# Aakash1312/Fluid-Simulation

Hardware: AMD Instinct MI355X
Metric: simulated substeps/sec (higher is better)
Workload: dtype f64

## Files before the change

fluid-simulation_amd/csrc/common.h:

```cpp
#pragma once
#include <hip/hip_runtime.h>
#include <stdint.h>

namespace fl {

constexpr uint8_t F_SOLID = 1;
constexpr uint8_t F_FLUID = 2;
constexpr int F_CNT_SHIFT = 2;

struct Grid {
    int N;
    int lo;
    int hi;
    int nx, ny, nz;
    int ox, oy, oz;
    __host__ __device__ inline size_t idx(int ix, int iy, int iz) const
    {
        return ((size_t)ix * ny + (size_t)iy) * nz + (size_t)iz;
    }
    __host__ __device__ inline size_t cells() const { return (size_t)nx * ny * nz; }
    __host__ __device__ inline long sx() const { return (long)ny * nz; }
    __host__ __device__ inline int cx0() const { return lo + ox; }
    __host__ __device__ inline int cy0() const { return lo + oy; }
    __host__ __device__ inline int cz0() const { return lo + oz; }
    __host__ __device__ inline int cx1() const { return lo + ox + nx - 1; }
    __host__ __device__ inline int cy1() const { return lo + oy + ny - 1; }
    __host__ __device__ inline int cz1() const { return lo + oz + nz - 1; }
};

struct Box {
    int x0, y0, z0, x1, y1, z1;
    __host__ __device__ inline int nx() const { return x1 - x0 + 1; }
    __host__ __device__ inline int ny() const { return y1 - y0 + 1; }
    __host__ __device__ inline int nz() const { return z1 - z0 + 1; }
    __host__ __device__ inline long long cells() const { return (long long)nx() * ny() * nz(); }
};

template <typename T>
struct Coef {
    T diag[7];
    T inv[7];
    T off;
};

constexpr int LBOX_K0 = 16;
struct LBox {
    int x0, y0, z0, nx, ny, nz, Lx, Ly, Lz;
    __host__ __device__ inline size_t cells() const { return (size_t)Lx * Ly * Lz; }
};

struct MLevel {
    int dx, dy, dz;
    long sx, sy;
    int ox, oy, oz;
    size_t cells;
    __host__ __device__ inline size_t at(int i, int j, int k) const
    {
        return (size_t)((long)(i + ox) * sx + (long)(j + oy) * sy + (k + oz));
    }
};
template <typename T>
struct MgCoef {
    T diag[7];
    T inv[7];
    T off;
};

struct PcgState {
    double bb;
    double thr;
    double rr;
    int done;
    int iters;
    int breakdown;
    int pad;
};

struct StepState {
    int bbox_min[3];
    int bbox_max[3];
    int num_active;
    int n_out;
    int max_cell;
    int n_drop;
    int n_tl_mg, n_tl_sq;
    int n_rows, n_l1_old;
    int n_tl_int, n_tl_bnd;
    int n_l1_gal, n_drop_fail;
    unsigned long long max_speed_bits;
    double dt;
    double err_num;
    double err_den;
};

constexpr size_t STATE_PS_OFF = 256;
constexpr int MAX_PARTIALS = 8192;

__device__ __forceinline__ double spline(double x)
{
    if (x < 0) x *= -1.0;
    if (x < 0.5) return 1.5 * (4.0 * x * x * x - 4.0 * x * x + 2.0 / 3.0);
    if (x < 1.0) return 1.5 * ((-8.0 * (x * x * x) / 6.0) + 4.0 * x * x - 4.0 * x + 4.0 / 3.0);
    return 0;
}

__device__ __forceinline__ double spline_at(double p, int c, int d)
{
    double x = p - (double)c;
    if (d == 1) return spline(x);
    if (x < 0) x *= -1.0;
    if (x < 1.0) return 1.5 * ((-8.0 * (x * x * x) / 6.0) + 4.0 * x * x - 4.0 * x + 4.0 / 3.0);
    return 0;
}

template <typename T>
__device__ __forceinline__ T wave_sum(T v)
{
#pragma unroll
    for (int o = 32; o > 0; o >>= 1) v += __shfl_down(v, o, 64);
    return v;
}
template <typename T>
__device__ __forceinline__ T wave_max(T v)
{
#pragma unroll
    for (int o = 32; o > 0; o >>= 1) {
        T w = __shfl_down(v, o, 64);
        v = w > v ? w : v;
    }
    return v;
}
template <typename T, int NW>
__device__ __forceinline__ T block_sum(T v, T* sm)
{
    v = wave_sum(v);
    const int lane = threadIdx.x & 63, w = threadIdx.x >> 6;
    __syncthreads();
    if (lane == 0) sm[w] = v;
    __syncthreads();
    T r = 0;
    if (threadIdx.x == 0) {
#pragma unroll
        for (int i = 0; i < NW; ++i) r += sm[i];
    }
    return r;
}
template <int NW>
__device__ __forceinline__ double block_sum_array(const double* __restrict__ a, int n, double* sm)
{
    double v = 0;
    for (int i = threadIdx.x; i < n; i += NW * 64) v += a[i];
    v = wave_sum(v);
    const int lane = threadIdx.x & 63, w = threadIdx.x >> 6;
    __syncthreads();
    if (lane == 0) sm[w] = v;
    __syncthreads();
    if (threadIdx.x == 0) {
        double r = 0;
#pragma unroll
        for (int i = 0; i < NW; ++i) r += sm[i];
        sm[NW] = r;
    }
    __syncthreads();
    return sm[NW];
}

__device__ __forceinline__ int xcd_remap(int b, int nb)
{
    const int q = nb >> 3, r = nb & 7, xcd = b & 7;
    return (xcd < r ? xcd * (q + 1) : r * (q + 1) + (xcd - r) * q) + (b >> 3);
}

__device__ __forceinline__ void block_sum3(const double* __restrict__ a, int na, const double* __restrict__ b, int nb,
                                           const double* __restrict__ c, int nc, double* sm, double& ra, double& rb, double& rc)
{
    double va = 0, vb = 0, vc = 0;
    for (int i = threadIdx.x; i < na; i += 256) va += a[i];
    for (int i = threadIdx.x; i < nb; i += 256) vb += b[i];
    for (int i = threadIdx.x; i < nc; i += 256) vc += c[i];
    va = wave_sum(va); vb = wave_sum(vb); vc = wave_sum(vc);
    const int lane = threadIdx.x & 63, w = threadIdx.x >> 6;
    if (lane == 0) { sm[w] = va; sm[4 + w] = vb; sm[8 + w] = vc; }
    __syncthreads();
    ra = ((sm[0] + sm[1]) + sm[2]) + sm[3];
    rb = ((sm[4] + sm[5]) + sm[6]) + sm[7];
    rc = ((sm[8] + sm[9]) + sm[10]) + sm[11];
}

struct Particles {
    double *px, *py, *pz, *vx, *vy, *vz;
    uint32_t* pid;
    __host__ __device__ inline Particles shifted(long o) const
    {
        Particles q = *this;
        q.px += o; q.py += o; q.pz += o; q.vx += o; q.vy += o; q.vz += o; q.pid += o;
        return q;
    }
};
constexpr uint32_t PID_DEAD = 0xFFFFFFFFu;

void launch_bin_count(hipStream_t st, Grid g, long n, Particles p, int* key, int* slot, int* cell_count, int* part, StepState* ss);
void launch_bin_scatter(hipStream_t st, long n, const int* key, const int* slot, const int* cell_start, const uint32_t* pid, int* order,
                         uint32_t* spid);
void launch_bin_rank(hipStream_t st, long n_pos, long pos0, const int* key, const int* cell_start, const int* order, const uint32_t* spid,
                     int* order2);
void launch_reorder(hipStream_t st, long n, const int* order, Particles src, Particles dst, double* w = nullptr, long wstride = 0);
void launch_weights(hipStream_t st, long n, Particles p, double* w, long stride);
void launch_axpby_box(hipStream_t st, Grid g, Box box, double a, const double* x, double b, const double* y, double* out, const PcgState* gate = nullptr);
long p2g_max_items(Box box);
size_t p2g_part_doubles(Box box);
constexpr int P2G_PILED = 256;
void launch_p2g(hipStream_t st, Grid g, Box box, Particles p, const double* pw, long wstride, const int* cell_start, const uint8_t* flags,
                double* part, int* items, float* container, double* u, double* v, double* w, double* ub, double* vb, double* wb, int2* crowd_list = nullptr,
                Particles park = Particles{});
void launch_p2g_tiles(hipStream_t st, Grid g, Box box, Particles p, const double* pw, long wstride, const int* cell_start, const uint8_t* flags,
                      float* container, double* u, double* v, double* w, double* ub, double* vb, double* wb);
void launch_g2p_tiled(hipStream_t st, Grid g, Box pb, Particles p, const int* cell_start, const double* dcx, const double* dcy, const double* dcz,
                      const double* pcx, const double* pcy, const double* pcz, double blend, StepState* ss);
void launch_g2p(hipStream_t st, Grid g, long n, Particles p, const double* dcx, const double* dcy, const double* dcz, const double* pcx,
                const double* pcy, const double* pcz, double blend, StepState* ss);
void launch_advect(hipStream_t st, Grid g, long n, Particles p, const uint8_t* flags, double max_dt, double dx, StepState* ss);
void launch_advect_bin(hipStream_t st, Grid g, long n, Particles p, const uint8_t* flags, double max_dt, double dx, StepState* ss, int* key,
                       int* slot, int* cell_count, int* part);
void launch_pack_particles(hipStream_t st, long n, Particles p, double* pos_aos, double* vel_aos);
void launch_unpack_records(hipStream_t st, long n, const double* rec, Particles p, long off);
void launch_pack_records(hipStream_t st, long n, Particles p, long off, double* rec);
void launch_unpack_ids(hipStream_t st, long n, const double* pos, const double* vel, const uint32_t* ids, Particles p);
void launch_pack_ids(hipStream_t st, long n, Particles p, long off, double* pos, double* vel, uint32_t* ids);
void launch_unpack_particles(hipStream_t st, long n, const double* pos_aos, const double* vel_aos, Particles p);

void launch_out_mark(hipStream_t st, const float* f, int N, int off, int nl, int* flags);
void launch_out_pack(hipStream_t st, const float* f, int N, int lo, int off, int nl, const int* flags, const int* slot, float* values,
                     int* origin);
struct OutWin {
    int ny, nz;
    int ox, oy, oz;
    int olo[3], ohi[3];
    int lo, off;
    int l0[3], nl[3];
    __host__ __device__ inline long leaves() const { return (long)nl[0] * nl[1] * nl[2]; }
};
void launch_out_mark_win(hipStream_t st, const float* f, const OutWin& w, int* flags);
void launch_out_pack_win(hipStream_t st, const float* f, const OutWin& w, const int* flags, const int* slot, float* values, int* origin);
void launch_exclusive_scan(hipStream_t st, const int* in, int* out, long n, int* block_sums, int* total);
void launch_sort_tail(hipStream_t st, const int* cell_count, int* cell_start, long c1, long ncell);
void launch_index_scan(hipStream_t st, Grid g, const uint8_t* flags, int* indices, int* block_sums, int* total);
void launch_index_scan_flat(hipStream_t st, const uint8_t* flags, int* indices, long n, int* block_sums, int* total);
void launch_flags(hipStream_t st, Grid g, const uint8_t* solid, const float* container, uint8_t* flags, int x0, int x1);
void launch_index_scan_range(hipStream_t st, Grid g, const uint8_t* flags, int* indices, int* block_sums, int* total, int x0, int x1);
void launch_rhs_div(hipStream_t st, Grid g, Box box, const uint8_t* flags, const double* u, const double* v, const double* w,
                    float* rhs, float* diver, double dx, double gdt0, double gdt1, double gdt2, bool rows = false, const PcgState* gate = nullptr);
void launch_vel_update(hipStream_t st, Grid g, Box box, const uint8_t* flags, const double* p, double* u, double* v, double* w,
                       double k, double g0, double g1, double g2, bool rows = false, const PcgState* gate = nullptr);
void launch_flip_delta(hipStream_t st, Grid g, Box box, const double* u, const double* v, const double* w,
                       const double* ub, const double* vb, const double* wb, double* dcx, double* dcy, double* dcz, double* pcx, double* pcy, double* pcz);
void launch_err_norm(hipStream_t st, Grid g, Box box, const uint8_t* flags, const float* b, const float* b2, double* part, StepState* ss,
                     const PcgState* gate = nullptr);
void launch_zero_step_state(hipStream_t st, StepState* ss, int N);
struct ZeroList { float* f4[4]; double* f8[7]; };
void launch_zero_fields(hipStream_t st, const ZeroList& z, Grid g, Box box, bool rows = false);
void launch_unpack_box(hipStream_t st, Grid g, Box box, const double* buf, float* container, double* u, double* v, double* w, double* ub, double* vb,
                       double* wb);

void launch_extrap_init(hipStream_t st, Grid g, const uint8_t* solid, const float* container, int* layer);
void launch_extrap_layer(hipStream_t st, Grid g, int pass, int* layer, double* u, double* v, double* w, int* n_new);
void launch_resample(hipStream_t st, Grid g, long n, Particles p, const int* cell_start, int per_cell, int xlim, double far_, int* n_parked);

struct SinkSet { int n; Box box[8]; };
void launch_src_count(hipStream_t st, Grid g, long n, Particles p, Box box, int* hist);
void launch_src_plan(hipStream_t st, Grid g, Box box, uint64_t h0, int per_cell, bool fill, const uint8_t* solid, const int* hist, int* cnt);
void launch_src_emit(hipStream_t st, Grid g, Box box, uint64_t h0, int per_cell, bool fill, const uint8_t* solid, const int* hist, const int* off,
                     Particles p, uint32_t pid0, const double vel[3]);
void launch_src_append(hipStream_t st, long n, const double* pos, const double* vel, Particles p, uint32_t pid0);
void launch_interp_from_grid(hipStream_t st, Grid g, long n, Particles p, const double* u, const double* v, const double* w);
void launch_sink_mark(hipStream_t st, Grid g, long n, Particles p, const SinkSet& sk, int* keep_dev, int* keep_pid, int* removed);
void launch_sink_compact(hipStream_t st, long n, Particles a, Particles b, const int* keep_dev, const int* dev_off, const int* pid_new);

void launch_spline_eval(hipStream_t st, int which, long n, const double* x, double* w);
void launch_dot(hipStream_t st, long n, const double* a, const double* b, double* part, int nb, double* out);

LBox make_lbox(const Box& b);
size_t lbox_max_cells(int N);
int pcg_sq_blocks(const LBox& L);
int pcg_xr_blocks(const LBox& L);
void launch_cnt_local(hipStream_t st, Grid g, LBox L, const uint8_t* flags, uint8_t* cnt);
template <typename T>
void launch_pcg_init(hipStream_t st, Grid g, LBox L, const uint8_t* cnt, const float* b, T* x, T* r, Coef<T> cf, double* part_bb,
                     double* part_rz0, PcgState* ps);
template <typename T>
void launch_pcg_sq(hipStream_t st, LBox L, const uint8_t* cnt, const T* r, const T* s_in, T* s_out, T* q, Coef<T> cf,
                   const double* part_rr, const double* part_rz_new, const double* part_rz_old, double* part_pq, PcgState* ps, int first,
                   double tol, int n_rz = -1, int zmode = 0, int sparse = 0, int n_prev = -1);
template <typename T>
void launch_pcg_xr(hipStream_t st, LBox L, const uint8_t* cnt, T* x, T* r, const T* s, const T* q, Coef<T> cf, const double* part_rz_cur,
                   const double* part_pq, double* part_rr, double* part_rz_next, PcgState* ps, int n_rz = -1, int sparse = 0);
void launch_pcg_sq_zf(hipStream_t st, LBox L, const uint8_t* cnt, const float* z, const double* s_in, double* s_out, double* q, Coef<double> cf,
                      const double* part_rr, int n_prev, const double* part_rz_new, const double* part_rz_old, double* part_pq, PcgState* ps, int first,
                      double tol, int n_rz, int sparse, const int* tlist, int nlist);
int pcg_list_blocks(int nlist);
template <typename T>
void launch_pcg_sq_list(hipStream_t st, LBox L, const uint8_t* cnt, const T* r, const T* s_in, T* s_out, T* q, Coef<T> cf,
                        const double* part_rr, int n_prev, const double* part_rz_new, const double* part_rz_old, double* part_pq, PcgState* ps,
                        int first, double tol, int n_rz, int zmode, const int* tlist, int nlist);
template <typename T>
void launch_pcg_xr_list(hipStream_t st, LBox L, const uint8_t* cnt, T* x, T* r, const T* s, const T* q, Coef<T> cf, const double* part_rz_cur,
                        int n_rz, const double* part_pq, double* part_rr, double* part_rz_next, PcgState* ps, const int* tlist, int nlist);
int pcg_row_count(const LBox& L);
int pcg_rows_blocks(int nrows);
void launch_row_list(hipStream_t st, LBox L, const uint8_t* cnt, int* flags, int* pos, int* list, int* block_sums, int* count);
constexpr int DROP_CAP = 65536;
constexpr int DROP_NCTR = 64;
void launch_drop_find(hipStream_t st, LBox L, uint8_t* cnt, int* ctr, int* pre, int* total, int* comp_n, int* comp_cells, const Box* own = nullptr);
void launch_drop_solve(hipStream_t st, Grid g, LBox L, int n_comp, const int* pre, const int* comp_n, const int* comp_cells, const uint8_t* flags,
                       const float* b, Coef<double> cf, double tol, double* pressure, double* keep, int* n_fail = nullptr, const PcgState* gate = nullptr);
template <typename T>
void launch_pcg_xr_rows(hipStream_t st, LBox L, const uint8_t* cnt, T* x, T* r, const T* s, const T* q, Coef<T> cf, const double* part_rz_cur,
                        int n_rz, const double* part_pq, int n_pq, double* part_rr, double* part_rz_next, PcgState* ps, const int* rlist, int nrows);
template <typename T>
void launch_pcg_sq_dist(hipStream_t st, LBox L, const uint8_t* cnt, const T* r, const T* s_in, T* s_out, T* q, Coef<T> cf, const double* g_rr,
                        const double* g_rz_new, const double* g_rz_old, double* part_pq, PcgState* ps, int first, double tol, int zmode);
template <typename T>
void launch_pcg_xr_dist(hipStream_t st, LBox L, const uint8_t* cnt, T* x, T* r, const T* s, const T* q, Coef<T> cf, const double* g_rz_cur,
                        const double* g_pq, double* part_rr, double* part_rz_next, PcgState* ps);
void launch_sum2(hipStream_t st, const double* a, int na, const double* b, int nb, double* out_a, double* out_b);
void launch_pcg_az_dist_zf(hipStream_t st, LBox L, const uint8_t* cnt, const float* z, double* w, Coef<double> cf, double* part_zw, PcgState* ps, const int* tlist, int nlist);
void launch_pcg_cgear_upd_zf(hipStream_t st, LBox L, const uint8_t* cnt, double* x, double* r, double* s, double* q, const float* z, const double* w, const double* g,
                             double* cg, int cur, double* part_rr, PcgState* ps, int first, double tol);
void launch_pcg_poll_stage(hipStream_t st, const double* part_rr, int n, const PcgState* ps, double* out);
void launch_pcg_poll_test(hipStream_t st, const double* g, PcgState* ps);
void launch_sum4(hipStream_t st, const double* a, int na, const double* b, int nb, const double* c, int nc, const double* e, int ne, double* out);
template <typename T>
void launch_pcg_az_dist(hipStream_t st, LBox L, const uint8_t* cnt, const T* z, T* w, Coef<T> cf, double* part_zw, PcgState* ps, const int* tlist = nullptr,
                        int nlist = 0);
template <typename T>
void launch_pcg_cgear_upd(hipStream_t st, LBox L, const uint8_t* cnt, T* x, T* r, T* s, T* q, const T* z, const T* w, const double* g, double* cg, int cur,
                          double* part_rr, PcgState* ps, int first, double tol);
template <typename T>
void launch_stencil_apply(hipStream_t st, Grid g, Box box, const uint8_t* flags, const T* s, T* q, Coef<T> cf);
template <typename T>
bool launch_stencil_march(hipStream_t st, Grid g, const uint8_t* flags, const T* s, T* q, Coef<T> cf, int variant, int cxcode);
template <typename T>
void launch_store_pressure(hipStream_t st, Grid g, LBox L, const uint8_t* cnt, const T* x, double* pressure, double* keep = nullptr,
                           const PcgState* ps = nullptr, bool gated = false);
template <typename T>
void launch_pcg_init_guess(hipStream_t st, Grid g, LBox L, const uint8_t* cnt, const float* b, const double* guess, const double* guess2, double ca,
                           double cb, T* x, T* r, Coef<T> cf, double* part_bb, double* part_rr0, PcgState* ps);

MLevel mg_level0(const LBox& L);
MLevel mg_coarser(const MLevel& f);
void launch_mg_type0(hipStream_t st, Grid g, LBox L, MLevel m, const uint8_t* flags, const uint8_t* cnt, uint8_t* typ);
void launch_mg_coarsen(hipStream_t st, MLevel mf, const uint8_t* tf, MLevel mc, uint8_t* tc, uint8_t* cnt_c);
void launch_mg_coarsen_types(hipStream_t st, MLevel mf, const uint8_t* tf, MLevel mc, uint8_t* tc);
void launch_mg_counts(hipStream_t st, MLevel m, const uint8_t* typ, uint8_t* cnt);
template <typename T>
void launch_mg_restrict(hipStream_t st, MLevel mf, const T* rf, MLevel mc, const uint8_t* cnt_c, T* fc, const PcgState* ps);
constexpr int MG_TAIL_MAX = 4;
constexpr size_t MG_TAIL_LDS = 144 * 1024;
size_t mg_tail_lds_bytes(int nl, const MLevel* lv, size_t elem);
int mg_up_blocks(const MLevel& m);
template <typename T, typename F>
void launch_mg_down(hipStream_t st, MLevel m, const uint8_t* cnt, const F* f, T* u, T* r, MLevel mc, const uint8_t* cnt_c, T* fc, MgCoef<T> cf,
                    const PcgState* ps, const int* tlist = nullptr, int nlist = 0, bool pcr = false);
template <typename T, typename F, typename O>
void launch_mg_up(hipStream_t st, MLevel m, const uint8_t* cnt, const F* f, const T* u, O* out, MLevel mc, const T* ec, MgCoef<T> cf,
                  double* part_dot, const PcgState* ps, double wc, const int* tlist = nullptr, int nlist = 0, const uint8_t* own = nullptr,
                  int pconst = 0);
bool gal_fits_coarsest(const MLevel& m);
void launch_gal_level1(hipStream_t st, MLevel m0, const uint8_t* cnt0, MgCoef<float> cf0, MLevel m1, float* gd, float* gx, float* gy, float* gz, uint8_t* cnt1);
void launch_gal_coarsen(hipStream_t st, MLevel mf, const float* fd, const float* fx, const float* fy, const float* fz, const uint8_t* cntf, MLevel mc,
                        float* gd, float* gx, float* gy, float* gz, uint8_t* cntc);
int gal_tile_count(const MLevel& m);
void launch_gal_tile_flags(hipStream_t st, MLevel m, const uint8_t* cnt, uint8_t* flags);
void launch_gal_down(hipStream_t st, MLevel m, const uint8_t* cnt, const float* gd, const float* gx, const float* gy, const float* gz, const float* f, float* u,
                     MLevel mc, float* fc, const PcgState* ps);
void launch_gal_up(hipStream_t st, MLevel m, const uint8_t* cnt, const float* gd, const float* gx, const float* gy, const float* gz, const float* f, const float* u,
                   float* out, MLevel mc, const float* ec, float wc, const PcgState* ps);
void launch_gal_coarsest(hipStream_t st, MLevel m, const float* gd, const float* gx, const float* gy, const float* gz, const float* f, float* u, int sweeps,
                         const PcgState* ps);
void launch_mg_tile_flags(hipStream_t st, MLevel m, const uint8_t* cnt, uint8_t* flags);
void launch_sq_tile_flags(hipStream_t st, LBox L, const uint8_t* cnt, uint8_t* flags);
int sq_tile_count(const LBox& L);
void launch_compact_flags(hipStream_t st, const uint8_t* flags, int n, int* list, int* count);
template <typename T>
void launch_mg_tail(hipStream_t st, int nl, const T* f0, const MLevel* lv, uint8_t* const* cnt, T* u0, const T* off, int sweeps, const PcgState* ps,
                    double wc);

}
```

fluid-simulation_amd/csrc/fluid_api.hip:

```cpp
#include "sim.h"
#include <algorithm>

using namespace fl;

static thread_local std::string g_err;
int fluid_fail(int code, const std::string& msg)
{
    g_err = msg;
    return code;
}
#define fail fluid_fail

Box fl::clip_dilate(const Box& b, int d, const Grid& g)
{
    Box r;
    r.x0 = b.x0 - d < 0 ? 0 : b.x0 - d;
    r.y0 = b.y0 - d < 0 ? 0 : b.y0 - d;
    r.z0 = b.z0 - d < 0 ? 0 : b.z0 - d;
    r.x1 = b.x1 + d > g.nx - 1 ? g.nx - 1 : b.x1 + d;
    r.y1 = b.y1 + d > g.ny - 1 ? g.ny - 1 : b.y1 + d;
    r.z1 = b.z1 + d > g.nz - 1 ? g.nz - 1 : b.z1 + d;
    return r;
}

int fl::prof_begin(fluid_sim* s, int k, double cells)
{
    ProfClass& p = s->prof[k];
    p.launches++;
    const bool per_iter = k == FLUID_PROF_PCG_SQ || k == FLUID_PROF_PCG_XR || k == FLUID_PROF_MG_UP0;
    const int every = per_iter ? s->prof_every : (s->prof_every >= 8 ? s->prof_every / 8 : (s->prof_every > 0 ? 1 : 0));
    if (every <= 0 || (p.launches - 1) % every) return -1;
    hipEvent_t a, b;
    if (hipEventCreate(&a) != hipSuccess || hipEventCreate(&b) != hipSuccess) return -1;
    hipEventRecord(a, s->st);
    p.e0.push_back(a);
    p.e1.push_back(b);
    p.pc.push_back(cells);
    return (int)p.e1.size() - 1;
}
void fl::prof_end(fluid_sim* s, int k, int tok)
{
    if (tok >= 0) hipEventRecord(s->prof[k].e1[tok], s->st);
}
static void prof_resolve(fluid_sim* s)
{
    for (int k = 0; k < FLUID_PROF_COUNT; ++k) {
        ProfClass& p = s->prof[k];
        for (size_t i = 0; i < p.e0.size(); ++i) {
            float ms = 0;
            hipEventSynchronize(p.e1[i]);
            if (hipEventElapsedTime(&ms, p.e0[i], p.e1[i]) == hipSuccess) {
                p.sampled++;
                p.ms += ms;
                p.cells += p.pc[i];
            }
            hipEventDestroy(p.e0[i]);
            hipEventDestroy(p.e1[i]);
        }
        p.e0.clear();
        p.e1.clear();
        p.pc.clear();
    }
}


static void free_particles(fluid_sim* s)
{
    for (Particles* p : {&s->pa, &s->pb}) {
        hipFree(p->px); hipFree(p->py); hipFree(p->pz); hipFree(p->vx); hipFree(p->vy); hipFree(p->vz); hipFree(p->pid);
        *p = Particles{};
    }
    hipFree(s->key); hipFree(s->slot); hipFree(s->order); hipFree(s->order2); hipFree(s->spid); hipFree(s->stage_pos); hipFree(s->stage_vel);
    s->order2 = nullptr; s->spid = nullptr; hipFree(s->pw);
    s->pw = nullptr;
    s->key = s->slot = s->order = nullptr;
    s->binned = false;
    s->stage_pos = s->stage_vel = nullptr;
    s->cap = 0;
}

int fl::alloc_particles(fluid_sim* s, long n)
{
    if (n <= s->cap) return FLUID_OK;
    n = (n + 1) & ~1L;
    free_particles(s);
    for (Particles* p : {&s->pa, &s->pb}) {
        HIPCHK(dalloc(&p->px, n)); HIPCHK(dalloc(&p->py, n)); HIPCHK(dalloc(&p->pz, n));
        HIPCHK(dalloc(&p->vx, n)); HIPCHK(dalloc(&p->vy, n)); HIPCHK(dalloc(&p->vz, n));
        HIPCHK(dalloc(&p->pid, n));
    }
    HIPCHK(dalloc(&s->key, n)); HIPCHK(dalloc(&s->slot, n)); HIPCHK(dalloc(&s->order, n)); HIPCHK(dalloc(&s->order2, n)); HIPCHK(dalloc(&s->spid, n));
    HIPCHK(dalloc(&s->stage_pos, 3 * n)); HIPCHK(dalloc(&s->stage_vel, 3 * n));
    HIPCHK(dalloc(&s->pw, 9 * n));
    HIPCHK(hipDeviceSynchronize());
    s->cap = n;
    return FLUID_OK;
}

int fl::grow_particles(fluid_sim* s, long need)
{
    if (need <= s->cap) return FLUID_OK;
    HIPCHK(hipStreamSynchronize(s->st));
    const long keep = s->p_off + s->np;
    Particles old = s->pa;
    s->pa = Particles{};
    const long ncap = ((need + need / 2) + 1) & ~1L;
    Particles nw{};
    HIPCHK(dalloc(&nw.px, ncap)); HIPCHK(dalloc(&nw.py, ncap)); HIPCHK(dalloc(&nw.pz, ncap));
    HIPCHK(dalloc(&nw.vx, ncap)); HIPCHK(dalloc(&nw.vy, ncap)); HIPCHK(dalloc(&nw.vz, ncap));
    HIPCHK(dalloc(&nw.pid, ncap));
    if (keep > 0) {
        HIPCHK(hipMemcpy(nw.px, old.px, keep * 8, hipMemcpyDeviceToDevice)); HIPCHK(hipMemcpy(nw.py, old.py, keep * 8, hipMemcpyDeviceToDevice));
        HIPCHK(hipMemcpy(nw.pz, old.pz, keep * 8, hipMemcpyDeviceToDevice)); HIPCHK(hipMemcpy(nw.vx, old.vx, keep * 8, hipMemcpyDeviceToDevice));
        HIPCHK(hipMemcpy(nw.vy, old.vy, keep * 8, hipMemcpyDeviceToDevice)); HIPCHK(hipMemcpy(nw.vz, old.vz, keep * 8, hipMemcpyDeviceToDevice));
        HIPCHK(hipMemcpy(nw.pid, old.pid, keep * 4, hipMemcpyDeviceToDevice));
    }
    hipFree(old.px); hipFree(old.py); hipFree(old.pz); hipFree(old.vx); hipFree(old.vy); hipFree(old.vz); hipFree(old.pid);
    free_particles(s);
    s->pa = nw;
    Particles* p = &s->pb;
    HIPCHK(dalloc(&p->px, ncap)); HIPCHK(dalloc(&p->py, ncap)); HIPCHK(dalloc(&p->pz, ncap));
    HIPCHK(dalloc(&p->vx, ncap)); HIPCHK(dalloc(&p->vy, ncap)); HIPCHK(dalloc(&p->vz, ncap));
    HIPCHK(dalloc(&p->pid, ncap));
    HIPCHK(dalloc(&s->key, ncap)); HIPCHK(dalloc(&s->slot, ncap)); HIPCHK(dalloc(&s->order, ncap)); HIPCHK(dalloc(&s->order2, ncap)); HIPCHK(dalloc(&s->spid, ncap));
    HIPCHK(dalloc(&s->stage_pos, 3 * ncap)); HIPCHK(dalloc(&s->stage_vel, 3 * ncap));
    HIPCHK(dalloc(&s->pw, 9 * ncap));
    HIPCHK(hipDeviceSynchronize());
    s->cap = ncap;
    return FLUID_OK;
}

extern "C" {

const char* fluid_last_error(void) { return g_err.c_str(); }
const char* fluid_version(void) { return "libfluid_hip 0.1 gfx950"; }

int fluid_default_params(fluid_params_t* p)
{
    if (!p) return fail(FLUID_ERR_ARG, "null params");
    memset(p, 0, sizeof(*p));
    p->n = 121;
    p->device = 0;
    p->dx = 1.0;
    p->rho = 1.0;
    p->gravity[0] = 0; p->gravity[1] = -10; p->gravity[2] = 0;
    p->max_dt = 0.1;
    p->outer_tol = 0.1;
    p->update_frac = 0.1;
    p->cg_tol = 2.220446049250313e-16;
    p->cg_max_iters = 0;
    p->max_outer_passes = 0;
    p->precision = FLUID_PRECISION_FP64;
    p->preconditioner = FLUID_PRECOND_MG;
    p->flip_blend = 1.0;
    p->solve_start = FLUID_START_WARM;
    p->mg_precision = FLUID_MG_FP32;
    p->dist_solve = FLUID_DIST_AUTO;
    return FLUID_OK;
}

int fluid_destroy(fluid_sim_t* s)
{
    if (!s) return FLUID_OK;
    if (s->st) hipStreamSynchronize(s->st);
    if (s->ds) dist_destroy(s);
    prof_resolve(s);
    free_particles(s);
    sources_free(s);
    output_free(s);
    void* ptrs[] = {s->solid, s->flags, s->container, s->rhs, s->diver, s->diver2, s->u, s->v, s->w, s->ub, s->vb, s->wb, s->dcx, s->dcy,
                    s->dcz, s->pressure, s->p_guess, s->p_guess2, s->p_q, s->indices, s->scan_sums, s->ipart, s->R, s->S[0], s->Q, s->X, s->mg_slab, s->mg_part, s->cntL, s->part_bb, s->part_rr,
                    s->part_rz[0], s->part_rz[1], s->part_pq, s->part_err, s->cell_count, s->cell_start, s->ss,
                    s->pcx, s->pcy, s->pcz, s->p2g_part, s->p2g_items, s->p2g_crowd, s->tl_flags, s->tl_mg, s->tl_sq, s->d_small, s->row_flags, s->row_pos, s->row_list, s->drop_n, s->drop_cells, s->drop_ctr, s->gal_slab};
    for (void* p : ptrs) if (p) hipFree(p);
    for (int i = 0; i < 2; ++i) if (s->ev_poll[i]) hipEventDestroy(s->ev_poll[i]);
    if (s->h_ss) hipHostFree(s->h_ss);
    if (s->h_small) hipHostFree(s->h_small);
    if (s->st) hipStreamDestroy(s->st);
    delete s;
    return FLUID_OK;
}

int fluid_create(const fluid_params_t* p, fluid_sim_t** out)
{
    if (!p || !out) return fail(FLUID_ERR_ARG, "null argument");
    Grid g;
    g.N = p->n;
    g.lo = -(p->n / 2);
    g.hi = g.lo + p->n - 1;
    g.nx = g.ny = g.nz = p->n;
    g.ox = g.oy = g.oz = 0;
    return fluid_create_window(p, g, out);
}

}

int fl::fluid_create_window(const fluid_params_t* p, const Grid& g, fluid_sim_t** out)
{
    if (!p || !out) return fail(FLUID_ERR_ARG, "null argument");
    if (p->n < 8 || p->n > 1024) return fail(FLUID_ERR_ARG, "n must be in [8,1024]");
    if (!(p->dx > 0) || !(p->rho > 0) || !(p->max_dt > 0)) return fail(FLUID_ERR_ARG, "dx, rho, max_dt must be > 0");
    if (p->precision != FLUID_PRECISION_FP64 && p->precision != FLUID_PRECISION_FP32) return fail(FLUID_ERR_ARG, "bad precision");
    if (!(p->flip_blend >= 0.0 && p->flip_blend <= 1.0)) return fail(FLUID_ERR_ARG, "flip_blend must be in [0,1] (1 = the reference's pure FLIP)");
    if (p->preconditioner != FLUID_PRECOND_MG && p->preconditioner != FLUID_PRECOND_JACOBI) return fail(FLUID_ERR_ARG, "bad preconditioner");
    if (p->solve_start != FLUID_START_WARM && p->solve_start != FLUID_START_ZERO) return fail(FLUID_ERR_ARG, "bad solve_start");
    if (p->mg_precision != FLUID_MG_FP32 && p->mg_precision != FLUID_MG_FP64) return fail(FLUID_ERR_ARG, "bad mg_precision");
    if (p->dist_solve < FLUID_DIST_AUTO || p->dist_solve > FLUID_DIST_REPLICATED || p->pad_ != 0) return fail(FLUID_ERR_ARG, "bad dist_solve / pad_");
    int ndev = 0;
    if (hipGetDeviceCount(&ndev) != hipSuccess || ndev <= 0)
        return fail(FLUID_ERR_HIP, "no HIP device visible: libfluid_hip has no CPU path");
    if (p->device < 0 || p->device >= ndev) return fail(FLUID_ERR_ARG, "device ordinal out of range");
    HIPCHK(hipSetDevice(p->device));
    fluid_sim* s = new fluid_sim();
    s->prm = *p;
    s->g = g;
    s->ncell = g.cells();
    s->dt = p->max_dt;
    s->mg_fp32 = p->mg_precision == FLUID_MG_FP32;
    s->warm = p->solve_start == FLUID_START_WARM;
    if (const char* e = getenv("FLUID_MG_CSWEEPS")) s->mg_csweeps = atoi(e);
    if (const char* e = getenv("FLUID_TILE_LISTS")) s->lists_force = atoi(e) != 0;
    if (const char* e = getenv("FLUID_P2G_FORM")) s->p2g_force = !strcmp(e, "rows") ? 1 : (!strcmp(e, "tiles") ? 2 : (!strcmp(e, "crowd") ? 3 : 0));
    if (const char* e = getenv("FLUID_MG_GALERKIN")) s->gal_mode = atoi(e);
    if (const char* e = getenv("FLUID_DROPLETS")) s->drops_on = atoi(e) != 0;
    if (const char* e = getenv("FLUID_ROW_SWEEPS")) s->row_sweeps = atoi(e) != 0;
    if (const char* e = getenv("FLUID_DROPLETS_MIN")) s->drop_min = atoi(e);
    if (const char* e = getenv("FLUID_ADVECT_BIN")) s->advect_bin = atoi(e) != 0;
    if (const char* e = getenv("FLUID_SOLVE_TAIL")) s->solve_tail = atoi(e) != 0;
    *out = nullptr;
    auto bail = [&](int rc) { fluid_destroy(s); return rc; };
#define A(expr) do { hipError_t e_ = (expr); if (e_ != hipSuccess) return bail(fail(FLUID_ERR_HIP, std::string(#expr) + ": " + hipGetErrorString(e_))); } while (0)
    A(hipStreamCreateWithFlags(&s->st, hipStreamNonBlocking));
    const size_t n = s->ncell;
    A(dalloc(&s->solid, n)); A(dalloc(&s->flags, n));
    A(dalloc(&s->container, n)); A(dalloc(&s->rhs, n)); A(dalloc(&s->diver, n)); A(dalloc(&s->diver2, n));
    A(dalloc(&s->u, n)); A(dalloc(&s->v, n)); A(dalloc(&s->w, n));
    A(dalloc(&s->ub, n)); A(dalloc(&s->vb, n)); A(dalloc(&s->wb, n));
    A(dalloc(&s->dcx, n)); A(dalloc(&s->dcy, n)); A(dalloc(&s->dcz, n));
    A(dalloc(&s->pressure, n));
    if (s->warm) {
        A(dalloc(&s->p_guess, n)); A(dalloc(&s->p_guess2, n));
        if (hipMemset(s->p_guess, 0, n * sizeof(double)) != hipSuccess || hipMemset(s->p_guess2, 0, n * sizeof(double)) != hipSuccess) return bail(FLUID_ERR_HIP);
        if (const char* e = getenv("FLUID_EXTRAPOLATE")) s->extrapolate = atoi(e) != 0;
        if (s->extrapolate) { A(dalloc(&s->p_q, n)); if (hipMemset(s->p_q, 0, n * sizeof(double)) != hipSuccess) return bail(FLUID_ERR_HIP); }
    }
    A(dalloc(&s->indices, n));
    A(dalloc(&s->scan_sums, (n + 2) / 2048 + 16));
    A(dalloc(&s->ipart, (size_t)1024 * 8));
    const size_t se = solver_elem(s);
    s->lmax = lbox_max_cells(std::max(g.nx, std::max(g.ny, g.nz)));
    const size_t ln = s->lmax;
    A(dalloc((char**)&s->R, ln * se)); A(dalloc((char**)&s->S[0], 2 * ln * se + 256));
    s->S[1] = (char*)s->S[0] + ln * se;
    A(dalloc((char**)&s->Q, ln * se)); A(dalloc((char**)&s->X, ln * se)); A(dalloc(&s->cntL, ln + 64));
    A(dalloc(&s->mg_part, ln / 256 + 64));
    A(dalloc(&s->part_bb, (size_t)MAX_PARTIALS)); A(dalloc(&s->part_rr, (size_t)MAX_PARTIALS));
    A(dalloc(&s->part_rz[0], (size_t)MAX_PARTIALS)); A(dalloc(&s->part_rz[1], (size_t)MAX_PARTIALS));
    A(dalloc(&s->part_pq, (size_t)MAX_PARTIALS)); A(dalloc(&s->part_err, (size_t)2 * MAX_PARTIALS));
    static_assert(sizeof(StepState) <= STATE_PS_OFF, "PcgState overlaps StepState");
    A(dalloc((char**)&s->ss, STATE_PS_OFF + sizeof(PcgState)));
    s->ps = (PcgState*)((char*)s->ss + STATE_PS_OFF);
    A(dalloc(&s->cell_count, n + 4)); A(dalloc(&s->cell_start, n + 4));
    A(dalloc(&s->d_small, (size_t)32));
    A(hipHostMalloc((void**)&s->h_small, 32 * sizeof(int)));
    A(hipEventCreateWithFlags(&s->ev_poll[0], hipEventDisableTiming));
    A(hipEventCreateWithFlags(&s->ev_poll[1], hipEventDisableTiming));
    A(hipHostMalloc((void**)&s->h_ss, STATE_PS_OFF + 2 * sizeof(PcgState)));
    s->h_ps = (PcgState*)((char*)s->h_ss + STATE_PS_OFF);
#undef A
    std::vector<uint8_t> sol(n, 0);
    const int N = p->n;
    for (int x = 0; x < g.nx; ++x)
        for (int y = 0; y < g.ny; ++y)
            for (int z = 0; z < g.nz; ++z) {
                const int X = x + g.ox, Y = y + g.oy, Z = z + g.oz;
                if (X < 2 || X > N - 3 || Y < 2 || Y > N - 3 || Z < 2 || Z > N - 3) sol[g.idx(x, y, z)] = 1;
            }
    hipError_t e = hipMemcpy(s->solid, sol.data(), n, hipMemcpyHostToDevice);
    if (e == hipSuccess) e = hipMemcpy(s->flags, sol.data(), n, hipMemcpyHostToDevice);
    if (e == hipSuccess) e = hipDeviceSynchronize();
    if (e != hipSuccess) return bail(fail(FLUID_ERR_HIP, std::string("solid upload: ") + hipGetErrorString(e)));
    *out = s;
    return FLUID_OK;
}

extern "C" {

int fluid_set_solid(fluid_sim_t* s, const uint8_t* solid)
{
    if (!s || !solid) return fail(FLUID_ERR_ARG, "null argument");
    const int N = s->g.N;
    const Grid g = s->g;
    for (int x = 0; x < N; ++x)
        for (int y = 0; y < N; ++y)
            for (int z = 0; z < N; ++z) {
                size_t c = ((size_t)x * N + y) * N + z;
                bool outsideW = x < 2 || x > N - 3 || y < 2 || y > N - 3 || z < 2 || z > N - 3;
                if (outsideW && !solid[c]) return fail(FLUID_ERR_ARG, "cells outside W=[lo+2,hi-2]^3 must be solid");
            }
    std::vector<uint8_t> sol(s->ncell);
    for (int x = 0; x < g.nx; ++x)
        for (int y = 0; y < g.ny; ++y)
            for (int z = 0; z < g.nz; ++z)
                sol[g.idx(x, y, z)] = solid[((size_t)(x + g.ox) * N + (y + g.oy)) * N + (z + g.oz)] ? 1 : 0;
    dist_keep_solid(s, solid);
    HIPCHK(hipStreamSynchronize(s->st));
    HIPCHK(hipMemcpy(s->solid, sol.data(), s->ncell, hipMemcpyHostToDevice));
    HIPCHK(hipMemcpy(s->flags, sol.data(), s->ncell, hipMemcpyHostToDevice));
    s->have_p2g = s->have_flags = false;
    s->flags_valid = false;
    s->have_guess = false;
    return FLUID_OK;
}

int fluid_upload_particles(fluid_sim_t* s, int64_t n, const double* pos, const double* vel)
{
    if (!s || n < 0 || (n > 0 && !pos)) return fail(FLUID_ERR_ARG, "bad particle arguments");
    if (s->dist) return fail(FLUID_ERR_STATE, "decomposed run: use fluid_upload_particles_ids (global ids must be unique across ranks)");
    if (n > 0x7fffffffL) return fail(FLUID_ERR_ARG, "too many particles");
    HIPCHK(hipSetDevice(s->prm.device));
    int rc = alloc_particles(s, (long)n);
    if (rc) return rc;
    s->np = (long)n;
    s->p_off = 0;
    if (n > 0) {
        HIPCHK(hipMemcpyAsync(s->stage_pos, pos, 3 * n * sizeof(double), hipMemcpyHostToDevice, s->st));
        if (vel) HIPCHK(hipMemcpyAsync(s->stage_vel, vel, 3 * n * sizeof(double), hipMemcpyHostToDevice, s->st));
        launch_unpack_particles(s->st, s->np, s->stage_pos, vel ? s->stage_vel : nullptr, s->pa);
        HIPCHK(hipGetLastError());
        HIPCHK(hipStreamSynchronize(s->st));
    }
    s->sorted = s->have_p2g = s->have_flags = false;
    s->have_guess = false;
    s->sort_hint = false;
    s->binned = false;
    s->vel_ok = false;
    return FLUID_OK;
}

int fluid_download_particles(fluid_sim_t* s, double* pos, double* vel)
{
    if (!s || !pos || !vel) return fail(FLUID_ERR_ARG, "null argument");
    if (s->dist) return fail(FLUID_ERR_STATE, "decomposed run: use fluid_download_particles_ids");
    if (s->np == 0) return FLUID_OK;
    HIPCHK(hipSetDevice(s->prm.device));
    launch_pack_particles(s->st, s->np, s->pa.shifted(s->p_off), s->stage_pos, s->stage_vel);
    HIPCHK(hipGetLastError());
    HIPCHK(hipMemcpyAsync(pos, s->stage_pos, 3 * s->np * sizeof(double), hipMemcpyDeviceToHost, s->st));
    HIPCHK(hipMemcpyAsync(vel, s->stage_vel, 3 * s->np * sizeof(double), hipMemcpyDeviceToHost, s->st));
    HIPCHK(hipStreamSynchronize(s->st));
    return FLUID_OK;
}

int64_t fluid_num_particles(fluid_sim_t* s) { return s ? s->np : -1; }
int fluid_set_dt(fluid_sim_t* s, double dt)
{
    if (!s || !(dt > 0)) return fail(FLUID_ERR_ARG, "dt must be > 0");
    s->dt = dt;
    return FLUID_OK;
}
int fluid_get_dt(fluid_sim_t* s, double* dt)
{
    if (!s || !dt) return fail(FLUID_ERR_ARG, "null argument");
    *dt = s->dt;
    return FLUID_OK;
}

static inline double u01(uint64_t seed, uint64_t ctr)
{
    uint64_t z = seed * 0x9E3779B97F4A7C15ull + ctr * 0xBF58476D1CE4E5B9ull + 0x94D049BB133111EBull;
    z ^= z >> 30; z *= 0xBF58476D1CE4E5B9ull;
    z ^= z >> 27; z *= 0x94D049BB133111EBull;
    z ^= z >> 31;
    return (double)(z >> 11) * (1.0 / 9007199254740992.0);
}

int64_t fluid_scene_water_cube_drop(int32_t n, int32_t ppc, uint64_t seed, double* pos)
{
    if (n < 8 || ppc < 1) return -1;
    const int m = (int)std::lround((double)n * 41.0 / 121.0);
    const int c0 = -(m / 2), c1 = c0 + m - 1;
    const int lo = -(n / 2), hi = lo + n - 1;
    int64_t cnt = 0;
    uint64_t ctr = 0;
    for (int x = c0; x <= c1; ++x)
        for (int y = c0; y <= c1; ++y)
            for (int z = c0; z <= c1; ++z)
                for (int k = 0; k < ppc; ++k) {
                    const double px = x - 0.5 + u01(seed, ctr), py = y - 0.5 + u01(seed, ctr + 1), pz = z - 0.5 + u01(seed, ctr + 2);
                    ctr += 3;
                    if (px > lo + 2 && px < hi - 2 && py > lo + 2 && py < hi - 2 && pz > lo + 2 && pz < hi - 2) {
                        if (pos) { pos[3 * cnt] = px; pos[3 * cnt + 1] = py; pos[3 * cnt + 2] = pz; }
                        cnt++;
                    }
                }
    return cnt;
}

}

int fl::read_ss(fluid_sim* s)
{
    HIPCHK(hipMemcpyAsync(s->h_ss, s->ss, sizeof(StepState), hipMemcpyDeviceToHost, s->st));
    HIPCHK(hipStreamSynchronize(s->st));
    return FLUID_OK;
}

int fl::clear_dirty(fluid_sim* s)
{
    if (box_empty(s->dirty)) return FLUID_OK;
    const ZeroList z = {{s->container, s->rhs, s->diver, s->diver2}, {s->u, s->v, s->w, s->ub, s->vb, s->wb, s->pressure}};
    launch_zero_fields(s->st, z, s->g, s->dirty, !s->dist && s->row_sweeps);
    HIPCHK(hipGetLastError());
    s->dirty = Box{0, 0, 0, -1, -1, -1};
    return FLUID_OK;
}

int fl::sort_pass(fluid_sim* s, int ax0, int ax1, int* h_tail)
{
    const Grid g = s->g;
    const long ncell = (long)s->ncell, n2 = g.sx();
    const long c0 = (long)ax0 * n2, c1 = (long)(ax1 + 1) * n2;
    launch_zero_step_state(s->st, s->ss, g.N);
    HIPCHK(hipMemsetAsync(s->cell_count + c0, 0, (c1 - c0) * sizeof(int), s->st));
    HIPCHK(hipMemsetAsync(s->cell_count + ncell, 0, 4 * sizeof(int), s->st));
    launch_bin_count(s->st, g, s->np, s->pa.shifted(s->p_off), s->key, s->slot, s->cell_count, s->ipart, s->ss);
    launch_exclusive_scan(s->st, s->cell_count + c0, s->cell_start + c0, c1 - c0, s->scan_sums, s->cell_start + c1);
    launch_sort_tail(s->st, s->cell_count, s->cell_start, c1, ncell);
    launch_bin_scatter(s->st, s->np, s->key, s->slot, s->cell_start, s->pa.shifted(s->p_off).pid, s->order, s->spid);
    launch_bin_rank(s->st, s->np, 0, s->key, s->cell_start, s->order, s->spid, s->order2);
    HIPCHK(hipGetLastError());
    if (h_tail) HIPCHK(hipMemcpyAsync(h_tail, s->cell_start + ncell, 3 * sizeof(int), hipMemcpyDeviceToHost, s->st));
    return read_ss(s);
}

static int sort_binned(fluid_sim* s)
{
    const Grid g = s->g;
    const long ncell = (long)s->ncell, n2 = g.sx();
    const long c0 = (long)s->bin_x0 * n2, c1 = (long)(s->bin_x1 + 1) * n2;
    launch_zero_step_state(s->st, s->ss, g.N);
    launch_exclusive_scan(s->st, s->cell_count + c0, s->cell_start + c0, c1 - c0, s->scan_sums, s->cell_start + c1);
    launch_sort_tail(s->st, s->cell_count, s->cell_start, c1, ncell);
    launch_bin_scatter(s->st, s->np, s->key, s->slot, s->cell_start, s->pa.shifted(s->p_off).pid, s->order, s->spid);
    launch_bin_rank(s->st, s->np, 0, s->key, s->cell_start, s->order, s->spid, s->order2);
    HIPCHK(hipGetLastError());
    StepState& h = *s->h_ss;
    for (int a = 0; a < 3; ++a) h.bbox_min[a] = s->bin_min[a], h.bbox_max[a] = s->bin_max[a];
    h.n_out = s->bin_n_out;
    h.max_cell = s->bin_max_cell;
    return FLUID_OK;
}

static int phase_sort(fluid_sim* s)
{
    const Grid g = s->g;
    int tok = prof_begin(s, FLUID_PROF_SORT, (double)s->np);
    int ax0 = 0, ax1 = g.nx - 1;
    const bool guess = s->sort_hint && !box_empty(s->Pb);
    if (guess) {
        ax0 = std::max(0, s->Pb.x0 - 3);
        ax1 = std::min(g.nx - 1, s->Pb.x1 + 3);
    }
    const bool binned = s->binned && guess && ax0 == s->bin_x0 && ax1 == s->bin_x1 && s->np > 0;
    s->binned = false;
    const auto missed = [&](const int* bmin, const int* bmax) {
        return guess && bmax[0] >= 0 && (bmin[0] < std::min(ax0 + 2, s->Pb.x0) || bmax[0] > std::max(ax1 - 2, s->Pb.x1));
    };
    int rc;
    if (binned && !missed(s->bin_min, s->bin_max)) {
        if ((rc = sort_binned(s))) return rc;
    } else {
        rc = binned ? FLUID_OK : sort_pass(s, ax0, ax1);
        if (rc) return rc;
        if (binned || missed(s->h_ss->bbox_min, s->h_ss->bbox_max)) {
            if ((rc = sort_pass(s, 0, g.nx - 1))) return rc;
        }
    }
    s->sort_hint = true;
    s->n_out = s->h_ss->n_out;
    s->max_cell = s->h_ss->max_cell;
    const StepState& h = *s->h_ss;
    if (h.bbox_max[0] < 0) {
        s->Pb = Box{0, 0, 0, -1, -1, -1};
    } else {
        s->Pb = Box{h.bbox_min[0], h.bbox_min[1], h.bbox_min[2], h.bbox_max[0], h.bbox_max[1], h.bbox_max[2]};
    }
    if (!box_empty(s->Pb)) {
        s->Rb = clip_dilate(s->Pb, 1, g);
        s->Sb = clip_dilate(s->Pb, 2, g);
    } else {
        s->Rb = s->Sb = s->Pb;
    }
    launch_reorder(s->st, s->np, s->order2, s->pa.shifted(s->p_off), s->pb, s->pw, s->cap);
    HIPCHK(hipGetLastError());
    std::swap(s->pa, s->pb);
    s->p_off = 0;
    prof_end(s, FLUID_PROF_SORT, tok);
    s->sorted = true;
    return FLUID_OK;
}

int fl::run_p2g(fluid_sim* s, const Box& box)
{
    const long ref_cells = s->p2g_ref_cells > 0 ? s->p2g_ref_cells : s->Rb.cells();
    const bool airy = s->last_num_active > 0 && (double)s->last_num_active < 0.3 * (double)ref_cells;
    const bool huge = (size_t)12 * sizeof(double) * (size_t)box.cells() > ((size_t)16 << 30);
    const bool piled = s->max_cell > P2G_PILED || airy;
    if (s->p2g_force ? s->p2g_force == 2 : huge) {
        s->stats.paths |= FLUID_PATH_P2G_TILES;
        launch_p2g_tiles(s->st, s->g, box, s->pa, s->pw, s->cap, s->cell_start, s->flags, s->container, s->u, s->v, s->w, s->ub, s->vb, s->wb);
        return FLUID_OK;
    }
    const bool crowd = s->p2g_force ? s->p2g_force == 3 : piled;
    if (crowd) {
        s->stats.paths |= FLUID_PATH_P2G_CROWD;
        const size_t nl = (size_t)s->cap / 16 + 64;
        if (nl > s->p2g_crowd_cap) {
            if (s->p2g_crowd) { HIPCHK(hipStreamSynchronize(s->st)); hipFree(s->p2g_crowd); s->p2g_crowd = nullptr; }
            HIPCHK(hipMalloc((void**)&s->p2g_crowd, nl * sizeof(int2)));
            s->p2g_crowd_cap = nl;
        }
    }
    const size_t need = p2g_part_doubles(box);
    if (need > s->p2g_part_cap) {
        if (s->p2g_part) { HIPCHK(hipStreamSynchronize(s->st)); hipFree(s->p2g_part); s->p2g_part = nullptr; }
        HIPCHK(hipMalloc((void**)&s->p2g_part, (need + need / 4) * sizeof(double)));
        s->p2g_part_cap = need + need / 4;
    }
    const size_t ni = 4 + 4 * (size_t)p2g_max_items(box);
    if (ni > s->p2g_items_cap) {
        if (s->p2g_items) { HIPCHK(hipStreamSynchronize(s->st)); hipFree(s->p2g_items); s->p2g_items = nullptr; }
        HIPCHK(hipMalloc((void**)&s->p2g_items, (ni + ni / 4) * sizeof(int)));
        HIPCHK(hipMemsetAsync(s->p2g_items, 0, 4 * sizeof(int), s->st));
        s->p2g_items_cap = ni + ni / 4;
    }
    launch_p2g(s->st, s->g, box, s->pa, s->pw, s->cap, s->cell_start, s->flags, s->p2g_part, s->p2g_items, s->container, s->u, s->v, s->w, s->ub,
               s->vb, s->wb, crowd ? s->p2g_crowd : nullptr, s->pb);
    return FLUID_OK;
}

static int phase_p2g(fluid_sim* s)
{
    HIPCHK(hipSetDevice(s->prm.device));
    int rc = phase_sort(s);
    if (rc) return rc;
    rc = clear_dirty(s);
    if (rc) return rc;
    memset(&s->stats, 0, sizeof(s->stats));
    s->stats.dt_in = s->dt;
    s->stats.dt_out = s->dt;
    for (int a = 0; a < 3; ++a) {
        s->stats.box_lo[a] = (&s->Rb.x0)[a];
        s->stats.box_hi[a] = (&s->Rb.x1)[a];
    }
    if (!box_empty(s->Rb)) {
        int tok = prof_begin(s, FLUID_PROF_P2G, (double)s->Rb.cells());
        rc = run_p2g(s, s->Rb);
        prof_end(s, FLUID_PROF_P2G, tok);
        if (rc) return rc;
        HIPCHK(hipGetLastError());
        s->dirty = s->Sb;
    }
    s->have_p2g = true;
    s->step_counter++;
    s->have_flags = false;
    return FLUID_OK;
}

template <typename T>
Coef<T> fl::make_coef(const fluid_sim* s)
{
    const double scale = s->dt / (s->prm.rho * s->prm.dx * s->prm.dx);
    Coef<T> c;
    float acc = 0.0f;
    c.diag[0] = 0;
    c.inv[0] = 0;
    for (int k = 1; k <= 6; ++k) {
        acc = (float)((double)acc + scale);
        c.diag[k] = (T)acc;
        c.inv[k] = (T)1 / c.diag[k];
    }
    c.off = (T)(float)(-1 * scale);
    return c;
}
template Coef<double> fl::make_coef<double>(const fluid_sim*);
template Coef<float> fl::make_coef<float>(const fluid_sim*);

hipError_t fl::zero_search(fluid_sim* s, size_t lb)
{
    const size_t step = (lb + 255) / 256 * 256;
    s->S[1] = (char*)s->S[0] + step;
    return hipMemsetAsync(s->S[0], 0, step + lb, s->st);
}


static int gal_build(fluid_sim* s);
static int mg_setup(fluid_sim* s)
{
    s->mgl[0] = mg_level0(s->L);
    int nl = 1;
    while (nl < fluid_sim::MG_MAXL && (nl < 2 || s->mgl[nl - 1].dx > 8 || s->mgl[nl - 1].dy > 8 || s->mgl[nl - 1].dz > 8)) {
        s->mgl[nl] = mg_coarser(s->mgl[nl - 1]);
        ++nl;
    }
    if (s->mgl[nl - 1].dx > 8 || s->mgl[nl - 1].dy > 8 || s->mgl[nl - 1].dz > 8) return fail(FLUID_ERR_STATE, "multigrid: too many levels");
    s->mg_nl = nl;
    int tail = nl - 1;
    const size_t es = s->mg_fp32 ? sizeof(float) : sizeof(double);
    auto fits = [&](int t) {
        const size_t b = nl - t <= MG_TAIL_MAX ? mg_tail_lds_bytes(nl - t, s->mgl + t, es) : 0;
        return b > 0 && b <= MG_TAIL_LDS;
    };
    while (tail > 1 && fits(tail - 1)) --tail;
    if (!fits(tail)) return fail(FLUID_ERR_STATE, "multigrid: coarsest level does not fit the tail kernel");
    s->mg_tail = tail;
    size_t total = 0;
    auto take = [&](size_t bytes) { const size_t o = total; total += (bytes + 255) / 256 * 256; return o; };
    size_t o_typ[fluid_sim::MG_MAXL], o_cnt[fluid_sim::MG_MAXL], o_u[fluid_sim::MG_MAXL], o_v[fluid_sim::MG_MAXL], o_f[fluid_sim::MG_MAXL],
        o_r[fluid_sim::MG_MAXL];
    for (int l = 0; l < nl; ++l) {
        const size_t c = s->mgl[l].cells + 64;
        o_typ[l] = take(c); o_cnt[l] = take(c);
        o_u[l] = take(c * es); o_v[l] = take(c * es); o_f[l] = take(c * es); o_r[l] = take(c * es);
    }
    const size_t o_z = take((s->mgl[0].cells + 64) * 8);
    if (total > s->mg_slab_cap) {
        if (s->mg_slab) { HIPCHK(hipStreamSynchronize(s->st)); hipFree(s->mg_slab); s->mg_slab = nullptr; }
        const size_t cap = total + total / 4;
        HIPCHK(hipMalloc((void**)&s->mg_slab, cap));
        s->mg_slab_cap = cap;
    }
    for (int l = 0; l < nl; ++l) {
        s->mg_typ[l] = (uint8_t*)(s->mg_slab + o_typ[l]);
        s->mg_cnt[l] = l ? (uint8_t*)(s->mg_slab + o_cnt[l]) : nullptr;
        s->mg_u[l] = s->mg_slab + o_u[l]; s->mg_v[l] = s->mg_slab + o_v[l];
        s->mg_f[l] = l ? s->mg_slab + o_f[l] : nullptr;
        s->mg_r[l] = s->mg_slab + o_r[l];
    }
    s->Zmg = s->mg_slab + o_z;
    HIPCHK(hipMemsetAsync(s->mg_slab, 0, total, s->st));
    launch_mg_type0(s->st, s->g, s->L, s->mgl[0], s->flags, s->cntL, s->mg_typ[0]);
    for (int l = 1; l < nl; ++l) launch_mg_coarsen(s->st, s->mgl[l - 1], s->mg_typ[l - 1], s->mgl[l], s->mg_typ[l], s->mg_cnt[l]);
    { int rcg = gal_build(s); if (rcg) return rcg; }
    HIPCHK(hipGetLastError());
    return FLUID_OK;
}

MgCoef<double> fl::mg_coef(const fluid_sim* s, int level)
{
    MgCoef<double> c;
    if (level == 0) {
        const Coef<double> f = make_coef<double>(s);
        for (int k = 0; k < 7; ++k) { c.diag[k] = f.diag[k]; c.inv[k] = f.inv[k]; }
        c.off = f.off;
        return c;
    }
    const double scale = s->dt / (s->prm.rho * s->prm.dx * s->prm.dx) / std::pow(4.0, level);
    c.off = -scale;
    c.diag[0] = 0; c.inv[0] = 0;
    for (int k = 1; k < 7; ++k) { c.diag[k] = scale * k; c.inv[k] = 1.0 / c.diag[k]; }
    return c;
}

static int mg_rz_blocks(const fluid_sim* s) { return s->lists_on ? s->n_tl_mg : mg_up_blocks(s->mgl[0]); }

template <typename V>
static MgCoef<V> mg_coef_as(const fluid_sim* s, int level)
{
    const MgCoef<double> d = mg_coef(s, level);
    MgCoef<V> c;
    for (int k = 0; k < 7; ++k) { c.diag[k] = (V)d.diag[k]; c.inv[k] = (V)d.inv[k]; }
    c.off = (V)d.off;
    return c;
}
static int gal_build(fluid_sim* s)
{
    s->gal = false;
    s->gal_eligible = false;
    const int nl = s->mg_nl;
    int lc = 1;
    while (lc < nl - 1 && !gal_fits_coarsest(s->mgl[lc])) ++lc;
    if (!(s->gal_mode && s->lists_on && s->mg_fp32 && !s->dist && (long)s->mgl[0].dx * s->mgl[0].dy * s->mgl[0].dz > 200000 &&
          gal_fits_coarsest(s->mgl[lc]) && lc >= 2)) {
        s->gal_it[0] = s->gal_it[1] = -1;
        return FLUID_OK;
    }
    s->gal_eligible = true;
    bool use = s->gal_mode >= 2;
    if (s->gal_mode == 1) {
        if (s->gal_it[0] < 0) use = false;
        else if (s->gal_it[1] < 0) use = true;
        else {
            use = 21 * s->gal_it[1] < 20 * s->gal_it[0];
            if (++s->gal_since_probe >= 32) { use = !use; s->gal_since_probe = 0; }
        }
    }
    if (!use) return FLUID_OK;
    size_t total = 0, off[fluid_sim::MG_MAXL][6];
    for (int l = 1; l <= lc; ++l)
        for (int q = 0; q < 6; ++q) {
            off[l][q] = total;
            total += (q < 5 ? ((q < 4 ? sizeof(float) : 1) * (s->mgl[l].cells + 64) + 255) / 256 * 256 : ((size_t)gal_tile_count(s->mgl[l]) + 255) / 256 * 256);
        }
    if (total > s->gal_slab_cap) {
        if (s->gal_slab) { HIPCHK(hipStreamSynchronize(s->st)); hipFree(s->gal_slab); s->gal_slab = nullptr; }
        HIPCHK(hipMalloc((void**)&s->gal_slab, total + total / 4));
        s->gal_slab_cap = total + total / 4;
    }
    HIPCHK(hipMemsetAsync(s->gal_slab, 0, total, s->st));
    for (int l = 1; l <= lc; ++l) {
        for (int q = 0; q < 4; ++q) s->gal_c[l][q] = (float*)(s->gal_slab + off[l][q]);
        s->gal_cnt[l] = (uint8_t*)(s->gal_slab + off[l][4]);
        s->gal_tfl[l] = (uint8_t*)(s->gal_slab + off[l][5]);
    }
    launch_gal_level1(s->st, s->mgl[0], s->cntL, mg_coef_as<float>(s, 0), s->mgl[1], s->gal_c[1][0], s->gal_c[1][1], s->gal_c[1][2], s->gal_c[1][3], s->gal_cnt[1]);
    for (int l = 2; l <= lc; ++l)
        launch_gal_coarsen(s->st, s->mgl[l - 1], s->gal_c[l - 1][0], s->gal_c[l - 1][1], s->gal_c[l - 1][2], s->gal_c[l - 1][3], s->gal_cnt[l - 1], s->mgl[l],
                           s->gal_c[l][0], s->gal_c[l][1], s->gal_c[l][2], s->gal_c[l][3], s->gal_cnt[l]);
    for (int l = 1; l < lc; ++l) launch_gal_tile_flags(s->st, s->mgl[l], s->gal_cnt[l], s->gal_tfl[l]);
    s->gal = true;
    s->gal_lc = lc;
    s->gal_dt = s->dt;
    HIPCHK(hipGetLastError());
    return FLUID_OK;
}
static int mg_vcycle_gal(fluid_sim* s, const double* rhs0, float* z0, double* part_rz)
{
    typedef float V;
    const PcgState* ps = s->ps;
    const int lc = s->gal_lc;
    auto U = [&](int l) { return (V*)s->mg_u[l]; };
    auto W = [&](int l) { return (V*)s->mg_v[l]; };
    auto F = [&](int l) { return (V*)s->mg_f[l]; };
    auto C = [&](int l, int q) { return (const float*)s->gal_c[l][q]; };
    const MLevel& m0 = s->mgl[0];
    launch_mg_down<V, double>(s->st, m0, s->cntL, rhs0, U(0), (V*)s->mg_r[0], s->mgl[1], nullptr, F(1), mg_coef_as<V>(s, 0), ps, s->tl_mg, s->n_tl_mg, true);
    for (int l = 1; l < lc; ++l) launch_gal_down(s->st, s->mgl[l], s->gal_tfl[l], C(l, 0), C(l, 1), C(l, 2), C(l, 3), F(l), U(l), s->mgl[l + 1], F(l + 1), ps);
    launch_gal_coarsest(s->st, s->mgl[lc], C(lc, 0), C(lc, 1), C(lc, 2), C(lc, 3), F(lc), U(lc), s->gal_sweeps, ps);
    for (int l = lc - 1; l >= 1; --l)
        launch_gal_up(s->st, s->mgl[l], s->gal_tfl[l], C(l, 0), C(l, 1), C(l, 2), C(l, 3), F(l), U(l), W(l), s->mgl[l + 1], l + 1 == lc ? U(l + 1) : W(l + 1),
                      (float)s->gal_wc, ps);
    const int tok = prof_begin(s, FLUID_PROF_MG_UP0, (double)s->Rb.cells());
    launch_mg_up<V, double, float>(s->st, m0, s->cntL, rhs0, (const V*)U(0), z0, s->mgl[1], W(1), mg_coef_as<V>(s, 0), part_rz, ps, s->gal_wc, s->tl_mg, s->n_tl_mg,
                                   nullptr, 1);
    prof_end(s, FLUID_PROF_MG_UP0, tok);
    HIPCHK(hipGetLastError());
    return FLUID_OK;
}

template <typename V>
static int mg_vcycle_t(fluid_sim* s, const double* rhs0, V* z0, double* part_rz)
{
    const int nl = s->mg_nl, tail = s->mg_tail;
    const PcgState* ps = s->ps;
    auto U = [&](int l) { return (V*)s->mg_u[l]; };
    auto W = [&](int l) { return (V*)s->mg_v[l]; };
    auto F = [&](int l) { return (V*)s->mg_f[l]; };
    auto R = [&](int l) { return (V*)s->mg_r[l]; };
    for (int l = 0; l < tail; ++l) {
        const MLevel& m = s->mgl[l];
        const bool fold = l > 0 || (long)m.dx * m.dy * m.dz <= 200000;
        V* fc = fold ? F(l + 1) : nullptr;
        const uint8_t* cc = fold ? s->mg_cnt[l + 1] : nullptr;
        const bool lst = s->lists_on && !fold;
        if (l == 0) launch_mg_down<V, double>(s->st, m, s->cntL, rhs0, U(0), R(0), s->mgl[1], cc, fc, mg_coef_as<V>(s, 0), ps, lst ? s->tl_mg : nullptr, s->n_tl_mg);
        else launch_mg_down<V, V>(s->st, m, s->mg_cnt[l], (const V*)F(l), U(l), R(l), s->mgl[l + 1], cc, fc, mg_coef_as<V>(s, l), ps);
        if (!fold) launch_mg_restrict<V>(s->st, m, (const V*)R(l), s->mgl[l + 1], s->mg_cnt[l + 1], F(l + 1), ps);
    }
    {
        V off[fluid_sim::MG_MAXL];
        for (int l = tail; l < nl; ++l) off[l] = (V)mg_coef(s, l).off;
        launch_mg_tail<V>(s->st, nl - tail, (const V*)F(tail), s->mgl + tail, s->mg_cnt + tail, U(tail), off + tail, s->mg_csweeps, ps, s->mg_wc[3]);
    }
    for (int l = tail - 1; l >= 0; --l) {
        const MLevel& m = s->mgl[l];
        const V* ec = l + 1 == tail ? U(l + 1) : W(l + 1);
        if (l == 0) {
            const int tok = prof_begin(s, FLUID_PROF_MG_UP0, (double)s->Rb.cells());
            launch_mg_up<V, double, V>(s->st, m, s->cntL, rhs0, (const V*)U(0), z0, s->mgl[1], ec, mg_coef_as<V>(s, 0), part_rz, ps, s->mg_wc[0],
                                       s->lists_on ? s->tl_mg : nullptr, s->n_tl_mg);
            prof_end(s, FLUID_PROF_MG_UP0, tok);
        } else {
            launch_mg_up<V, V, V>(s->st, m, s->mg_cnt[l], (const V*)F(l), (const V*)U(l), W(l), s->mgl[l + 1], ec, mg_coef_as<V>(s, l), nullptr, ps, s->mg_wc[l == 1 ? 1 : 2]);
        }
    }
    HIPCHK(hipGetLastError());
    return FLUID_OK;
}
static int mg_vcycle(fluid_sim* s, const double* rhs0, void* z0, double* part_rz)
{
    if (s->gal && s->lists_on) return mg_vcycle_gal(s, rhs0, (float*)z0, part_rz);
    return s->mg_fp32 ? mg_vcycle_t<float>(s, rhs0, (float*)z0, part_rz) : mg_vcycle_t<double>(s, rhs0, (double*)z0, part_rz);
}

static int phase_vel_update(fluid_sim* s, const PcgState* gate = nullptr);
static int phase_rhs_div(fluid_sim* s, int which, const PcgState* gate = nullptr);
static int solve_mg(fluid_sim* s, bool with_tail)
{
    typedef double T;
    const Grid g = s->g;
    const LBox L = s->L;
    T* X = (T*)s->X;
    T* R = (T*)s->R;
    T* Q = (T*)s->Q;
    T* Sx[2] = {(T*)s->S[0], (T*)s->S[1]};
    T* Z = (T*)s->Zmg;
    const uint8_t* cnt = s->cntL;
    const Coef<T> cf = make_coef<T>(s);
    const double tol = s->prm.cg_tol;
    long max_it = s->prm.cg_max_iters > 0 ? s->prm.cg_max_iters : 2 * (long)s->stats.num_active;
    if (max_it < 1) max_it = 1;
    const double cells = (double)s->Rb.cells();
    const int sparse = (double)s->stats.num_active < 0.4 * (double)L.cells();
    const bool lists = s->lists_on;
    const bool rows = lists && s->rows_on && s->n_rows > 0;
    const int n_init = pcg_xr_blocks(L), n_list = rows ? pcg_rows_blocks(s->n_rows) : pcg_list_blocks(s->n_tl_sq);
    const int n_rz_raw = mg_rz_blocks(s);
    const bool fold = n_rz_raw > 1024;
    const int n_rz = fold ? 1 : n_rz_raw;
    int rc;
    int tsolve = prof_begin(s, FLUID_PROF_SOLVE, cells);
    if (s->gal && s->gal_dt != s->dt) {
        const int keep = s->gal_mode; s->gal_mode = 2; rc = gal_build(s); s->gal_mode = keep;
        if (rc) return rc;
    }
    if (s->gal) s->stats.paths |= FLUID_PATH_MG_GALERKIN;
    const bool guess = s->warm && s->have_guess;
    const double *g1, *g2;
    double gca, gcb;
    s->start_guess(g1, g2, gca, gcb);
    if (guess) launch_pcg_init_guess<T>(s->st, g, L, cnt, s->diver, g1, g2, gca, gcb, X, R, cf, s->part_bb, s->part_rz[1], s->ps);
    else launch_pcg_init<T>(s->st, g, L, cnt, s->diver, X, R, cf, s->part_bb, s->part_rr, s->ps);
    long it = 0;
    const int pclass = s->pass_class();
    long batch = s->mg_last_iters_k[pclass] > 5 ? s->mg_last_iters_k[pclass] + 1 : 4;
    bool done = false;
    const bool zf = s->mg_fp32 || (s->gal && s->lists_on);
    auto sq = [&](int cur, const double* part_rr, int n_prev, const double* rz_new, const double* rz_old, int first, int sp) {
        const int prv = cur ^ 1;
        if (zf)
            launch_pcg_sq_zf(s->st, L, cnt, (const float*)s->Zmg, Sx[prv], Sx[cur], Q, cf, part_rr, n_prev, rz_new, rz_old, s->part_pq, s->ps, first, tol, n_rz, sp,
                             lists ? s->tl_sq : nullptr, s->n_tl_sq);
        else if (lists)
            launch_pcg_sq_list<T>(s->st, L, cnt, Z, Sx[prv], Sx[cur], Q, cf, part_rr, n_prev, rz_new, rz_old, s->part_pq, s->ps, first, tol, n_rz, 1, s->tl_sq, s->n_tl_sq);
        else
            launch_pcg_sq<T>(s->st, L, cnt, Z, Sx[prv], Sx[cur], Q, cf, part_rr, rz_new, rz_old, s->part_pq, s->ps, first, tol, n_rz, 1, sp, n_prev);
    };
    const bool will_make_q = s->warm && s->p_q && s->stats.outer_passes == 1 && s->guess_step == s->step_counter && s->guess_pass == 0;
    auto solution_out = [&](const PcgState* gate) {
        launch_store_pressure<T>(s->st, g, L, cnt, X, s->pressure, s->warm ? s->p_guess2 : nullptr, s->ps, gate != nullptr);
        launch_drop_solve(s->st, g, L, s->n_drop, s->drop_ctr + 64 * DROP_NCTR, s->drop_n, s->drop_cells, s->flags, s->diver, make_coef<double>(s), tol,
                          s->pressure, s->warm ? s->p_guess2 : nullptr, &s->ss->n_drop_fail, gate);
        if (will_make_q) launch_axpby_box(s->st, g, s->Rb, 1.0, s->p_guess2, -(1.0 - s->prm.update_frac), s->p_guess, s->p_q, gate);
    };
    bool first_poll = true;
    s->tail_ran = false;
    while (!done) {
        for (long k = 0; k < batch && it < max_it; ++k, ++it) {
            const int cur = (int)(it & 1), prv = cur ^ 1;
            if ((rc = mg_vcycle(s, R, s->Zmg, fold ? s->mg_part : s->part_rz[cur]))) return rc;
            if (fold) launch_sum2(s->st, s->mg_part, n_rz_raw, s->mg_part, 0, s->part_rz[cur], nullptr);
            int tok = prof_begin(s, FLUID_PROF_PCG_SQ, cells);
            sq(cur, it == 0 ? s->part_bb : s->part_rr, it == 0 ? n_init : (lists ? n_list : n_init), s->part_rz[cur], s->part_rz[prv], it == 0 ? (guess ? 2 : 1) : 0,
               sparse);
            prof_end(s, FLUID_PROF_PCG_SQ, tok);
            tok = prof_begin(s, FLUID_PROF_PCG_XR, cells);
            if (rows)
                launch_pcg_xr_rows<T>(s->st, L, cnt, X, R, Sx[cur], Q, cf, s->part_rz[cur], n_rz, s->part_pq, pcg_list_blocks(s->n_tl_sq), s->part_rr,
                                      s->part_err, s->ps, s->row_list, s->n_rows);
            else if (lists)
                launch_pcg_xr_list<T>(s->st, L, cnt, X, R, Sx[cur], Q, cf, s->part_rz[cur], n_rz, s->part_pq, s->part_rr, s->part_err, s->ps,
                                      s->tl_sq, s->n_tl_sq);
            else
                launch_pcg_xr<T>(s->st, L, cnt, X, R, Sx[cur], Q, cf, s->part_rz[cur], s->part_pq, s->part_rr, s->part_err, s->ps, n_rz, sparse);
            prof_end(s, FLUID_PROF_PCG_XR, tok);
        }
        HIPCHK(hipGetLastError());
        if (it < max_it) {
            const int cur = (int)(it & 1), prv = cur ^ 1;
            sq(cur, s->part_rr, lists ? n_list : n_init, s->part_rz[prv], s->part_rz[prv], 0, 0);
        }
        const bool spec = with_tail && s->solve_tail && !s->dist && first_poll && it < max_it;
        first_poll = false;
        if (spec) {
            int rc2;
            solution_out(s->ps);
            if ((rc2 = phase_vel_update(s, s->ps))) return rc2;
            if ((rc2 = phase_rhs_div(s, 1, s->ps))) return rc2;
            launch_err_norm(s->st, s->g, s->Rb, s->flags, s->diver, s->diver2, s->part_err, s->ss, s->ps);
            HIPCHK(hipGetLastError());
            HIPCHK(hipMemcpyAsync(s->h_ss, s->ss, STATE_PS_OFF + sizeof(PcgState), hipMemcpyDeviceToHost, s->st));
        } else {
            HIPCHK(hipMemcpyAsync(&s->h_ps[0], s->ps, sizeof(PcgState), hipMemcpyDeviceToHost, s->st));
        }
        HIPCHK(hipStreamSynchronize(s->st));
        done = s->h_ps[0].done || it >= max_it;
        if (spec && s->h_ps[0].done) s->tail_ran = true;
        if (!done) {
            s->h_ps[1] = s->h_ps[0];
            s->h_ps[1].iters -= 1;
            HIPCHK(hipMemcpyAsync(s->ps, &s->h_ps[1], sizeof(PcgState), hipMemcpyHostToDevice, s->st));
        }
        batch = 1;
    }
    int iters = s->h_ps->iters;
    const double rr = s->h_ps->rr;
    if (!s->h_ps->done) iters = (int)max_it;
    if (!s->tail_ran) solution_out(nullptr);
    if (s->warm) s->rotate_guess();
    s->have_guess = s->warm;
    if (s->make_q() != will_make_q) return fail(FLUID_ERR_STATE, "solve_mg: q formed for the wrong pass");
    if (will_make_q) s->q_step = s->step_counter;
    HIPCHK(hipGetLastError());
    prof_end(s, FLUID_PROF_SOLVE, tsolve);
    s->stats.cg_iters_last = iters;
    s->stats.cg_iters += iters;
    s->mg_last_iters_k[pclass] = iters;
    if (s->gal_eligible && s->stats.outer_passes == 0) s->gal_it[s->gal ? 1 : 0] = iters;
    s->stats.relres = s->h_ps->bb > 0 ? std::sqrt(rr / s->h_ps->bb) : 0.0;
    if (s->h_ps->breakdown) return fail(FLUID_ERR_SOLVER, "PCG breakdown: s.As <= 0 or NaN");
    return FLUID_OK;
}

int fl::phase_flags(fluid_sim* s)
{
    HIPCHK(hipSetDevice(s->prm.device));
    int x0 = 0, x1 = s->g.nx - 1;
    const bool none = box_empty(s->Sb);
    if (s->flags_valid) {
        x0 = none ? s->flag_x0 : (s->flag_x1 < s->flag_x0 ? s->Sb.x0 : std::min(s->Sb.x0, s->flag_x0));
        x1 = none ? s->flag_x1 : (s->flag_x1 < s->flag_x0 ? s->Sb.x1 : std::max(s->Sb.x1, s->flag_x1));
    }
    if (x1 >= x0) {
        launch_flags(s->st, s->g, s->solid, s->container, s->flags, x0, x1);
        launch_index_scan_range(s->st, s->g, s->flags, s->indices, s->scan_sums, &s->ss->num_active, x0, x1);
    } else {
        HIPCHK(hipMemsetAsync(&s->ss->num_active, 0, sizeof(int), s->st));
    }
    s->flag_x0 = none ? 0 : s->Sb.x0;
    s->flag_x1 = none ? -1 : s->Sb.x1;
    s->flags_valid = true;
    HIPCHK(hipGetLastError());
    bool built = false, drops = false;
    s->n_drop = 0;
    if (!box_empty(s->Rb)) {
        s->L = make_lbox(s->Rb);
        launch_cnt_local(s->st, s->g, s->L, s->flags, s->cntL);
        if (use_mg(s) && (s->lists_force >= 0 ? s->lists_force == 1 : s->lists_hint)) {
            const MLevel m0 = mg_level0(s->L);
            const int n_mg = mg_up_blocks(m0), n_sq = sq_tile_count(s->L);
            const size_t need = (size_t)n_mg + n_sq;
            if (need > s->tl_cap) {
                HIPCHK(hipStreamSynchronize(s->st));
                hipFree(s->tl_flags); hipFree(s->tl_mg); hipFree(s->tl_sq);
                s->tl_flags = nullptr; s->tl_mg = s->tl_sq = nullptr;
                const size_t cap = need + need / 4;
                HIPCHK(hipMalloc((void**)&s->tl_flags, cap));
                HIPCHK(hipMalloc((void**)&s->tl_mg, cap * sizeof(int)));
                HIPCHK(hipMalloc((void**)&s->tl_sq, cap * sizeof(int)));
                s->tl_cap = cap;
            }
            if (s->drops_on && !s->dist && (s->drop_last < 0 || s->drop_last >= s->drop_min || ++s->drop_skipped >= 8)) {
                s->drop_skipped = 0;
                if (!s->drop_cells) {
                    HIPCHK(hipMalloc((void**)&s->drop_ctr, (size_t)(64 * DROP_NCTR + DROP_NCTR + 1) * sizeof(int)));
                    HIPCHK(hipMalloc((void**)&s->drop_n, (size_t)DROP_CAP * sizeof(int)));
                    HIPCHK(hipMalloc((void**)&s->drop_cells, (size_t)DROP_CAP * 64 * sizeof(int)));
                }
                launch_drop_find(s->st, s->L, s->cntL, s->drop_ctr, s->drop_ctr + 64 * DROP_NCTR, &s->ss->n_drop, s->drop_n, s->drop_cells);
                drops = true;
            }
            launch_mg_tile_flags(s->st, m0, s->cntL, s->tl_flags);
            launch_compact_flags(s->st, s->tl_flags, n_mg, s->tl_mg, &s->ss->n_tl_mg);
            launch_sq_tile_flags(s->st, s->L, s->cntL, s->tl_flags + n_mg);
            launch_compact_flags(s->st, s->tl_flags + n_mg, n_sq, s->tl_sq, &s->ss->n_tl_sq);
            if (s->rows_on) {
                const size_t nr = (size_t)pcg_row_count(s->L);
                if (nr > s->row_cap) {
                    HIPCHK(hipStreamSynchronize(s->st));
                    hipFree(s->row_flags); hipFree(s->row_pos); hipFree(s->row_list);
                    s->row_flags = s->row_pos = s->row_list = nullptr;
                    const size_t cap = nr + nr / 4 + 1024;
                    HIPCHK(hipMalloc((void**)&s->row_flags, cap * sizeof(int)));
                    HIPCHK(hipMalloc((void**)&s->row_pos, cap * sizeof(int)));
                    HIPCHK(hipMalloc((void**)&s->row_list, cap * sizeof(int)));
                    s->row_cap = cap;
                }
                launch_row_list(s->st, s->L, s->cntL, s->row_flags, s->row_pos, s->row_list, s->scan_sums, &s->ss->n_rows);
            }
            built = true;
        }
        HIPCHK(hipGetLastError());
    }
    int rc = read_ss(s);
    if (rc) return rc;
    s->stats.num_active = s->h_ss->num_active;
    s->last_num_active = s->stats.num_active;
    s->lists_on = false;
    s->lists_hint = false;
    if (!box_empty(s->Rb)) {
        const bool airy = (double)s->stats.num_active < 0.45 * (double)s->L.cells() && s->L.cells() > (size_t)1500000;
        s->lists_hint = airy;
        s->n_tl_mg = s->h_ss->n_tl_mg; s->n_tl_sq = s->h_ss->n_tl_sq; s->n_rows = s->h_ss->n_rows;
        s->n_drop = drops ? std::min(s->h_ss->n_drop, DROP_CAP) : 0;
        if (drops) s->drop_last = s->n_drop;
        if (s->n_drop > 0) s->stats.paths |= FLUID_PATH_DROPLETS;
        s->lists_on = built && s->n_tl_mg > 0 && s->n_tl_sq > 0 && (s->lists_force == 1 || airy);
        if (s->lists_on) s->stats.paths |= FLUID_PATH_TILE_LISTS;
        const size_t lb = (s->L.cells() + 2 * (size_t)s->L.Lz) * solver_elem(s);
        HIPCHK(zero_search(s, lb));
        HIPCHK(hipGetLastError());
        if (use_mg(s)) {
            int rc2 = mg_setup(s);
            if (rc2) return rc2;
        }
    }
    s->have_flags = true;
    return FLUID_OK;
}

static int phase_rhs_div(fluid_sim* s, int which, const PcgState* gate)
{
    if (!s->have_flags) return fail(FLUID_ERR_STATE, "rhs_div before flags_index");
    if (box_empty(s->Rb)) return FLUID_OK;
    const double dt = s->dt;
    launch_rhs_div(s->st, s->g, s->Rb, s->flags, s->u, s->v, s->w, s->rhs, which ? s->diver2 : s->diver, s->prm.dx,
                   s->prm.gravity[0] * dt, s->prm.gravity[1] * dt, s->prm.gravity[2] * dt, !s->dist && s->row_sweeps, gate);
    HIPCHK(hipGetLastError());
    return FLUID_OK;
}

template <typename T>
static int solve_impl(fluid_sim* s)
{
    const Grid g = s->g;
    const LBox L = s->L;
    T* X = (T*)s->X;
    T* R = (T*)s->R;
    T* Q = (T*)s->Q;
    T* Sx[2] = {(T*)s->S[0], (T*)s->S[1]};
    const uint8_t* cnt = s->cntL;
    const Coef<T> cf = make_coef<T>(s);
    const double tol = s->prm.cg_tol;
    long max_it = s->prm.cg_max_iters > 0 ? s->prm.cg_max_iters : 2 * (long)s->stats.num_active;
    if (max_it < 1) max_it = 1;
    const double cells = (double)s->Rb.cells();
    int tsolve = prof_begin(s, FLUID_PROF_SOLVE, cells);
    launch_pcg_init<T>(s->st, g, L, cnt, s->diver, X, R, cf, s->part_bb, s->part_rz[0], s->ps);
    int tok = prof_begin(s, FLUID_PROF_PCG_SQ, cells);
    launch_pcg_sq<T>(s->st, L, cnt, R, (const T*)nullptr, Sx[0], Q, cf, s->part_bb, nullptr, nullptr, s->part_pq, s->ps, 1, tol);
    prof_end(s, FLUID_PROF_PCG_SQ, tok);
    tok = prof_begin(s, FLUID_PROF_PCG_XR, cells);
    launch_pcg_xr<T>(s->st, L, cnt, X, R, Sx[0], Q, cf, s->part_rz[0], s->part_pq, s->part_rr, s->part_rz[1], s->ps);
    prof_end(s, FLUID_PROF_PCG_XR, tok);
    long it = 1;
    const int CHECK = 16;
    bool done = false;
    int nb = 0;
    while (!done) {
        for (int k = 0; k < CHECK && it < max_it; ++k, ++it) {
            const int cur = (int)(it & 1), prv = cur ^ 1;
            tok = prof_begin(s, FLUID_PROF_PCG_SQ, cells);
            launch_pcg_sq<T>(s->st, L, cnt, R, Sx[prv], Sx[cur], Q, cf, s->part_rr, s->part_rz[cur], s->part_rz[prv], s->part_pq, s->ps, 0, tol);
            prof_end(s, FLUID_PROF_PCG_SQ, tok);
            tok = prof_begin(s, FLUID_PROF_PCG_XR, cells);
            launch_pcg_xr<T>(s->st, L, cnt, X, R, Sx[cur], Q, cf, s->part_rz[cur], s->part_pq, s->part_rr, s->part_rz[prv], s->ps);
            prof_end(s, FLUID_PROF_PCG_XR, tok);
        }
        HIPCHK(hipGetLastError());
        HIPCHK(hipMemcpyAsync(&s->h_ps[nb & 1], s->ps, sizeof(PcgState), hipMemcpyDeviceToHost, s->st));
        HIPCHK(hipEventRecord(s->ev_poll[nb & 1], s->st));
        if (nb >= 1) {
            HIPCHK(hipEventSynchronize(s->ev_poll[(nb - 1) & 1]));
            if (s->h_ps[(nb - 1) & 1].done) done = true;
        }
        if (it >= max_it) done = true;
        ++nb;
    }
    HIPCHK(hipMemcpyAsync(&s->h_ps[0], s->ps, sizeof(PcgState), hipMemcpyDeviceToHost, s->st));
    HIPCHK(hipStreamSynchronize(s->st));
    int iters = s->h_ps->iters;
    const double rr = s->h_ps->rr;
    if (!s->h_ps->done) {
        iters = (int)max_it;
    }
    launch_store_pressure<T>(s->st, g, L, cnt, X, s->pressure);
    launch_drop_solve(s->st, g, L, s->n_drop, s->drop_ctr + 64 * DROP_NCTR, s->drop_n, s->drop_cells, s->flags, s->diver, make_coef<double>(s), tol,
                      s->pressure, nullptr, &s->ss->n_drop_fail);
    HIPCHK(hipGetLastError());
    prof_end(s, FLUID_PROF_SOLVE, tsolve);
    s->stats.cg_iters_last = iters;
    s->stats.cg_iters += iters;
    s->stats.relres = s->h_ps->bb > 0 ? std::sqrt(rr / s->h_ps->bb) : 0.0;
    if (s->h_ps->breakdown) return fail(FLUID_ERR_SOLVER, "PCG breakdown: s.As <= 0 or NaN (matrix not SPD for these flags)");
    return FLUID_OK;
}

static int phase_solve(fluid_sim* s, bool with_tail = false)
{
    s->tail_ran = false;
    if (!s->have_flags) return fail(FLUID_ERR_STATE, "solve before flags_index");
    if (box_empty(s->Rb)) return FLUID_OK;
    if (use_mg(s) && s->mg_nl >= 2) return solve_mg(s, with_tail);
    return s->prm.precision == FLUID_PRECISION_FP32 ? solve_impl<float>(s) : solve_impl<double>(s);
}

static int phase_vel_update(fluid_sim* s, const PcgState* gate)
{
    if (!s->have_flags) return fail(FLUID_ERR_STATE, "vel_update before flags_index");
    if (box_empty(s->Sb)) return FLUID_OK;
    const double dtp = s->dt * s->prm.update_frac;
    const double k = dtp / (s->prm.rho * s->prm.dx);
    launch_vel_update(s->st, s->g, s->Sb, s->flags, s->pressure, s->u, s->v, s->w, k, s->prm.gravity[0] * dtp, s->prm.gravity[1] * dtp,
                      s->prm.gravity[2] * dtp, !s->dist && s->row_sweeps, gate);
    HIPCHK(hipGetLastError());
    return FLUID_OK;
}

int fl::phase_pressure_pass(fluid_sim* s, double* error)
{
    int rc;
    if ((rc = phase_rhs_div(s, 0))) return rc;
    if ((rc = phase_solve(s, true))) return rc;
    const bool tail_ran = s->tail_ran;
    s->tail_ran = false;
    if (!tail_ran) {
        if ((rc = phase_vel_update(s))) return rc;
        if ((rc = phase_rhs_div(s, 1))) return rc;
    }
    double err = NAN;
    if (!box_empty(s->Rb)) {
        if (!tail_ran) {
            launch_err_norm(s->st, s->g, s->Rb, s->flags, s->diver, s->diver2, s->part_err, s->ss);
            HIPCHK(hipGetLastError());
            if ((rc = read_ss(s))) return rc;
        }
        if (s->h_ss->n_drop_fail > 0) s->stats.paths |= FLUID_PATH_DROPLETS_SHORT;
        err = std::sqrt(s->h_ss->err_num) / std::sqrt(s->h_ss->err_den);
    }
    s->stats.error = err;
    s->stats.outer_passes++;
    if (error) *error = err;
    return FLUID_OK;
}

int fl::pic_fields(fluid_sim* s)
{
    if (s->prm.flip_blend >= 1.0 || s->pcx) return FLUID_OK;
    double** f[3] = {&s->pcx, &s->pcy, &s->pcz};
    for (double** q : f) {
        HIPCHK(hipMalloc((void**)q, s->ncell * sizeof(double)));
        HIPCHK(hipMemsetAsync(*q, 0, s->ncell * sizeof(double), s->st));
    }
    return FLUID_OK;
}

static int phase_flip_advect(fluid_sim* s)
{
    if (!s->have_p2g) return fail(FLUID_ERR_STATE, "flip_advect before p2g");
    HIPCHK(hipSetDevice(s->prm.device));
    int rcp = pic_fields(s);
    if (rcp) return rcp;
    if (!box_empty(s->Rb)) launch_flip_delta(s->st, s->g, s->Rb, s->u, s->v, s->w, s->ub, s->vb, s->wb, s->dcx, s->dcy, s->dcz, s->pcx, s->pcy, s->pcz);
    int tok = prof_begin(s, FLUID_PROF_G2P, (double)s->np);
    if (s->sorted && s->p_off == 0 && (double)s->np >= 4.0 * (double)s->Pb.cells()) {
        launch_g2p_tiled(s->st, s->g, s->Pb, s->pa, s->cell_start, s->dcx, s->dcy, s->dcz, s->pcx, s->pcy, s->pcz, s->prm.flip_blend, s->ss);
        if (!box_empty(s->Pb)) s->stats.paths |= FLUID_PATH_G2P_TILES;
        if (s->n_out > 0)
            launch_g2p(s->st, s->g, s->n_out, s->pa.shifted(s->np - s->n_out), s->dcx, s->dcy, s->dcz, s->pcx, s->pcy, s->pcz, s->prm.flip_blend, s->ss);
    } else {
        launch_g2p(s->st, s->g, s->np, s->pa.shifted(s->p_off), s->dcx, s->dcy, s->dcz, s->pcx, s->pcy, s->pcz, s->prm.flip_blend, s->ss);
    }
    prof_end(s, FLUID_PROF_G2P, tok);
    const bool bin = s->advect_bin && !s->dist && s->np > 0 && s->sorted && s->sort_hint && !box_empty(s->Pb);
    s->binned = false;
    if (bin) {
        const Grid g = s->g;
        s->bin_x0 = std::max(0, s->Pb.x0 - 3);
        s->bin_x1 = std::min(g.nx - 1, s->Pb.x1 + 3);
        const long n2 = g.sx(), c0 = (long)s->bin_x0 * n2, c1 = (long)(s->bin_x1 + 1) * n2;
        HIPCHK(hipMemsetAsync(s->cell_count + c0, 0, (c1 - c0) * sizeof(int), s->st));
        HIPCHK(hipMemsetAsync(s->cell_count + s->ncell, 0, 4 * sizeof(int), s->st));
        launch_advect_bin(s->st, g, s->np, s->pa.shifted(s->p_off), s->flags, s->prm.max_dt, s->prm.dx, s->ss, s->key, s->slot, s->cell_count, s->ipart);
    } else {
        launch_advect(s->st, s->g, s->np, s->pa.shifted(s->p_off), s->flags, s->prm.max_dt, s->prm.dx, s->ss);
    }
    HIPCHK(hipGetLastError());
    int rc = read_ss(s);
    if (rc) return rc;
    if (bin) {
        const StepState& h = *s->h_ss;
        for (int a = 0; a < 3; ++a) s->bin_min[a] = h.bbox_min[a], s->bin_max[a] = h.bbox_max[a];
        s->bin_n_out = h.n_out;
        s->bin_max_cell = h.max_cell;
        s->binned = true;
    }
    s->dt = s->h_ss->dt;
    double ms;
    memcpy(&ms, &s->h_ss->max_speed_bits, sizeof(double));
    s->stats.max_speed = ms;
    s->stats.dt_out = s->dt;
    s->sorted = false;
    s->have_p2g = false;
    s->vel_ok = true;
    return FLUID_OK;
}

extern "C" {

#define PHASE_GUARD(s)                                                                                        \
    if (!(s)) return fail(FLUID_ERR_ARG, "null handle");                                                      \
    if ((s)->dist) return fail(FLUID_ERR_STATE, "per-phase entry points are single-GPU only; a decomposed run steps with fluid_step")
int fluid_p2g(fluid_sim_t* s) { PHASE_GUARD(s); return phase_p2g(s); }
int fluid_flags_index(fluid_sim_t* s) { PHASE_GUARD(s); return phase_flags(s); }
int fluid_rhs_div(fluid_sim_t* s, int which) { PHASE_GUARD(s); return phase_rhs_div(s, which, nullptr); }
int fluid_solve(fluid_sim_t* s) { PHASE_GUARD(s); return phase_solve(s, false); }
int fluid_vel_update(fluid_sim_t* s) { PHASE_GUARD(s); return phase_vel_update(s, nullptr); }
int fluid_pressure_pass(fluid_sim_t* s, double* error) { PHASE_GUARD(s); return phase_pressure_pass(s, error); }
int fluid_flip_advect(fluid_sim_t* s) { PHASE_GUARD(s); return phase_flip_advect(s); }

int fluid_extrapolate(fluid_sim_t* s, int32_t* n_layers)
{
    PHASE_GUARD(s);
    if (!s->have_p2g) return fail(FLUID_ERR_STATE, "extrapolate before p2g");
    HIPCHK(hipSetDevice(s->prm.device));
    const Grid g = s->g;
    int* layer = s->indices;
    int* n_new = s->d_small;
    launch_extrap_init(s->st, g, s->solid, s->container, layer);
    int pass = 0;
    for (bool more = true; more;) {
        HIPCHK(hipMemsetAsync(n_new, 0, sizeof(int), s->st));
        for (int k = 0; k < 8; ++k) launch_extrap_layer(s->st, g, ++pass, layer, s->u, s->v, s->w, n_new);
        HIPCHK(hipGetLastError());
        HIPCHK(hipMemcpyAsync(s->h_small, n_new, sizeof(int), hipMemcpyDeviceToHost, s->st));
        HIPCHK(hipStreamSynchronize(s->st));
        more = s->h_small[0] != 0 && pass < 3 * g.N + 8;
    }
    const size_t bytes = s->ncell * sizeof(double);
    HIPCHK(hipMemcpyAsync(s->ub, s->u, bytes, hipMemcpyDeviceToDevice, s->st));
    HIPCHK(hipMemcpyAsync(s->vb, s->v, bytes, hipMemcpyDeviceToDevice, s->st));
    HIPCHK(hipMemcpyAsync(s->wb, s->w, bytes, hipMemcpyDeviceToDevice, s->st));
    s->flags_valid = false;
    s->have_flags = false;
    s->dirty = Box{0, 0, 0, g.nx - 1, g.ny - 1, g.nz - 1};
    HIPCHK(hipStreamSynchronize(s->st));
    if (n_layers) *n_layers = pass;
    return FLUID_OK;
}

int fluid_get_droplets(fluid_sim_t* s, int32_t* n_components, int64_t* cells, int32_t cap_components)
{
    if (!s) return fail(FLUID_ERR_ARG, "null handle");
    if (n_components) *n_components = s->n_drop;
    if (!cells || s->n_drop <= 0 || cap_components <= 0) return FLUID_OK;
    HIPCHK(hipSetDevice(s->prm.device));
    const int n = std::min(s->n_drop, (int)cap_components);
    std::vector<int> pre(DROP_NCTR + 1), an(DROP_CAP), ac((size_t)DROP_CAP * 64), hn(n), hc((size_t)n * 64);
    HIPCHK(hipStreamSynchronize(s->st));
    HIPCHK(hipMemcpy(pre.data(), s->drop_ctr + 64 * DROP_NCTR, pre.size() * sizeof(int), hipMemcpyDeviceToHost));
    HIPCHK(hipMemcpy(an.data(), s->drop_n, an.size() * sizeof(int), hipMemcpyDeviceToHost));
    HIPCHK(hipMemcpy(ac.data(), s->drop_cells, ac.size() * sizeof(int), hipMemcpyDeviceToHost));
    for (int d = 0, c = 0; d < n; ++d) {
        while (c + 1 < DROP_NCTR && pre[c + 1] <= d) ++c;
        const size_t slot = (size_t)c * (DROP_CAP / DROP_NCTR) + (size_t)(d - pre[c]);
        hn[d] = an[slot];
        std::copy(ac.begin() + slot * 64, ac.begin() + slot * 64 + 64, hc.begin() + (size_t)d * 64);
    }
    const LBox L = s->L;
    for (int c = 0; c < n; ++c) {
        int64_t* o = cells + (size_t)c * 64;
        const int m = std::min(std::max(hn[c], 0), 64);
        for (int q = 0; q < m; ++q) {
            const long t = hc[(size_t)c * 64 + q];
            const int k = (int)(t % L.Lz), j = (int)((t / L.Lz) % L.Ly), i = (int)(t / ((long)L.Lz * L.Ly));
            o[q] = (int64_t)s->g.idx(L.x0 + i - 1, L.y0 + j - 1, L.z0 + k - LBOX_K0);
        }
        std::sort(o, o + m);
        for (int q = m; q < 64; ++q) o[q] = -1;
    }
    return FLUID_OK;
}

int fluid_resample(fluid_sim_t* s, int32_t per_cell, int64_t* n_parked)
{
    PHASE_GUARD(s);
    if (per_cell < 0) return fail(FLUID_ERR_ARG, "per_cell must be >= 0");
    if (s->np == 0) { if (n_parked) *n_parked = 0; return FLUID_OK; }
    HIPCHK(hipSetDevice(s->prm.device));
    int rc = phase_sort(s);
    if (rc) return rc;
    HIPCHK(hipMemsetAsync(s->d_small, 0, sizeof(int), s->st));
    launch_resample(s->st, s->g, s->np - s->n_out, s->pa, s->cell_start, per_cell, s->g.hi - 10, (double)(s->g.hi + 40), s->d_small);
    HIPCHK(hipGetLastError());
    HIPCHK(hipMemcpyAsync(s->h_small, s->d_small, sizeof(int), hipMemcpyDeviceToHost, s->st));
    HIPCHK(hipStreamSynchronize(s->st));
    if (n_parked) *n_parked = s->h_small[0];
    s->sorted = s->have_p2g = s->have_flags = false;
    s->sort_hint = false;
    s->binned = false;
    return FLUID_OK;
}

int fluid_get_stats(fluid_sim_t* s, fluid_step_stats_t* st)
{
    if (!s || !st) return fail(FLUID_ERR_ARG, "null argument");
    *st = s->stats;
    return FLUID_OK;
}


int fluid_step(fluid_sim_t* s, fluid_step_stats_t* stats)
{
    if (!s) return fail(FLUID_ERR_ARG, "null handle");
    int rc;
    if ((rc = output_auto_check(s))) return rc;
    if (s->dist) return dist_step(s, stats);
    if ((rc = phase_p2g(s))) return rc;
    if ((rc = phase_flags(s))) return rc;
    double error = NAN;
    do {
        if ((rc = phase_pressure_pass(s, &error))) return rc;
        if (s->prm.max_outer_passes > 0 && s->stats.outer_passes >= s->prm.max_outer_passes) break;
    } while (error > s->prm.outer_tol);
    if ((rc = phase_flip_advect(s))) return rc;
    if ((rc = sources_apply(s))) return rc;
    if ((rc = output_auto(s))) return rc;
    s->n_steps++;
    if (stats) *stats = s->stats;
    return FLUID_OK;
}

static int field_info(fluid_sim* s, int field, void** ptr, size_t* bytes)
{
    const size_t n = s->ncell, se = solver_elem(s);
    switch (field) {
    case FLUID_FIELD_CONTAINER: case FLUID_FIELD_WEIGHTS: case FLUID_FIELD_OUTPUT: *ptr = s->container; *bytes = n * 4; return 0;
    case FLUID_FIELD_INDICES: *ptr = s->indices; *bytes = n * 4; return 0;
    case FLUID_FIELD_RHS: *ptr = s->rhs; *bytes = n * 4; return 0;
    case FLUID_FIELD_DIVER: *ptr = s->diver; *bytes = n * 4; return 0;
    case FLUID_FIELD_DIVER2: *ptr = s->diver2; *bytes = n * 4; return 0;
    case FLUID_FIELD_PRESSURE: *ptr = s->pressure; *bytes = n * 8; return 0;
    case FLUID_FIELD_SOLID: *ptr = s->solid; *bytes = n; return 0;
    case FLUID_FIELD_FLAGS: *ptr = s->flags; *bytes = n; return 0;
    case FLUID_FIELD_SEARCH: *ptr = s->S[0]; *bytes = n * se; return 0;
    case FLUID_FIELD_Q: *ptr = s->Q; *bytes = n * se; return 0;
    case FLUID_FIELD_VEL: case FLUID_FIELD_VEL_BEFORE: *ptr = nullptr; *bytes = 3 * n * 8; return 0;
    }
    return -1;
}

int fluid_download_field(fluid_sim_t* s, int field, void* dst, size_t bytes)
{
    if (!s || !dst) return fail(FLUID_ERR_ARG, "null argument");
    void* p;
    size_t nb;
    if (field_info(s, field, &p, &nb)) return fail(FLUID_ERR_ARG, "unknown field id");
    if (bytes != nb) return fail(FLUID_ERR_ARG, "byte count does not match the field size");
    HIPCHK(hipSetDevice(s->prm.device));
    HIPCHK(hipStreamSynchronize(s->st));
    if (field == FLUID_FIELD_VEL || field == FLUID_FIELD_VEL_BEFORE) {
        double* src[3] = {field == FLUID_FIELD_VEL ? s->u : s->ub, field == FLUID_FIELD_VEL ? s->v : s->vb, field == FLUID_FIELD_VEL ? s->w : s->wb};
        for (int a = 0; a < 3; ++a) HIPCHK(hipMemcpy((char*)dst + a * s->ncell * 8, src[a], s->ncell * 8, hipMemcpyDeviceToHost));
        return FLUID_OK;
    }
    HIPCHK(hipMemcpy(dst, p, nb, hipMemcpyDeviceToHost));
    return FLUID_OK;
}

int fluid_upload_field(fluid_sim_t* s, int field, const void* src, size_t bytes)
{
    if (!s || !src) return fail(FLUID_ERR_ARG, "null argument");
    void* p;
    size_t nb;
    if (field_info(s, field, &p, &nb)) return fail(FLUID_ERR_ARG, "unknown field id");
    if (bytes != nb) return fail(FLUID_ERR_ARG, "byte count does not match the field size");
    if (field == FLUID_FIELD_SOLID || field == FLUID_FIELD_FLAGS || field == FLUID_FIELD_INDICES || field == FLUID_FIELD_Q)
        return fail(FLUID_ERR_ARG, "field is not uploadable (use fluid_set_solid / fluid_flags_index)");
    HIPCHK(hipSetDevice(s->prm.device));
    HIPCHK(hipStreamSynchronize(s->st));
    if (field == FLUID_FIELD_VEL || field == FLUID_FIELD_VEL_BEFORE) {
        double* d[3] = {field == FLUID_FIELD_VEL ? s->u : s->ub, field == FLUID_FIELD_VEL ? s->v : s->vb, field == FLUID_FIELD_VEL ? s->w : s->wb};
        for (int a = 0; a < 3; ++a) HIPCHK(hipMemcpy(d[a], (const char*)src + a * s->ncell * 8, s->ncell * 8, hipMemcpyHostToDevice));
    } else {
        HIPCHK(hipMemcpy(p, src, nb, hipMemcpyHostToDevice));
    }
    s->Rb = s->Sb = Box{0, 0, 0, s->g.nx - 1, s->g.ny - 1, s->g.nz - 1};
    s->dirty = s->Rb;
    if (field == FLUID_FIELD_CONTAINER) { s->have_p2g = true; s->have_flags = false; }
    return FLUID_OK;
}

static int stencil_run(fluid_sim* s, int reps, int box_mode, int nsets, void* const (*sets)[3], float* avg_ms)
{
    const int N = s->g.N;
    const Box box = box_mode == 1 ? s->Rb : Box{0, 0, 0, N - 1, N - 1, N - 1};
    if (box_empty(box)) return fail(FLUID_ERR_STATE, "empty active box");
    const char* ev = getenv("FLUID_MARCH_VARIANT");
    const char* ec = getenv("FLUID_MARCH_CX");
    const int mv = ev ? atoi(ev) : 0, mc = ec ? atoi(ec) : 0;
    hipEvent_t e0, e1;
    HIPCHK(hipEventCreate(&e0));
    HIPCHK(hipEventCreate(&e1));
    HIPCHK(hipEventRecord(e0, s->st));
    for (int i = 0; i < reps; ++i) {
        const void* S = nsets > 1 ? sets[i % nsets][0] : s->S[0];
        void* Q = nsets > 1 ? sets[i % nsets][1] : s->Q;
        const uint8_t* fl = nsets > 1 ? (const uint8_t*)sets[i % nsets][2] : s->flags;
        if (s->prm.precision == FLUID_PRECISION_FP32) {
            if (!(box_mode == 0 && (N >= 64 || mv) && launch_stencil_march<float>(s->st, s->g, fl, (const float*)S, (float*)Q, make_coef<float>(s), mv, mc)))
                launch_stencil_apply<float>(s->st, s->g, box, fl, (const float*)S, (float*)Q, make_coef<float>(s));
        } else {
            if (!(box_mode == 0 && (N >= 64 || mv) && launch_stencil_march<double>(s->st, s->g, fl, (const double*)S, (double*)Q, make_coef<double>(s), mv, mc)))
                launch_stencil_apply<double>(s->st, s->g, box, fl, (const double*)S, (double*)Q, make_coef<double>(s));
        }
    }
    HIPCHK(hipEventRecord(e1, s->st));
    HIPCHK(hipGetLastError());
    HIPCHK(hipEventSynchronize(e1));
    float ms = 0;
    HIPCHK(hipEventElapsedTime(&ms, e0, e1));
    hipEventDestroy(e0);
    hipEventDestroy(e1);
    if (avg_ms) *avg_ms = ms / reps;
    return FLUID_OK;
}

int fluid_stencil_apply(fluid_sim_t* s, int reps, int box_mode, float* avg_ms)
{
    if (!s || reps < 1) return fail(FLUID_ERR_ARG, "bad argument");
    if (!s->have_flags) return fail(FLUID_ERR_STATE, "stencil_apply before flags_index");
    HIPCHK(hipSetDevice(s->prm.device));
    return stencil_run(s, reps, box_mode, 1, nullptr, avg_ms);
}

int fluid_stencil_apply_hbm(fluid_sim_t* s, int reps, int box_mode, int64_t footprint_bytes, int32_t* nsets_out, float* avg_ms)
{
    if (!s || reps < 1 || footprint_bytes < 0) return fail(FLUID_ERR_ARG, "bad argument");
    if (!s->have_flags) return fail(FLUID_ERR_STATE, "stencil_apply before flags_index");
    HIPCHK(hipSetDevice(s->prm.device));
    const size_t se = solver_elem(s), n = s->ncell;
    const size_t set_bytes = 2 * n * se + n;
    int nsets = (int)((footprint_bytes + (int64_t)set_bytes - 1) / (int64_t)set_bytes);
    nsets = std::max(2, std::min(nsets, 256));
    std::vector<void*> mem((size_t)3 * nsets, nullptr);
    std::vector<void*> flat(mem.size());
    auto release = [&]() { for (void* p : mem) if (p) hipFree(p); };
    for (int i = 0; i < nsets; ++i) {
        hipError_t e = hipMalloc(&mem[3 * i], n * se);
        if (e == hipSuccess) e = hipMalloc(&mem[3 * i + 1], n * se);
        if (e == hipSuccess) e = hipMalloc(&mem[3 * i + 2], n);
        if (e == hipSuccess) e = hipMemcpyAsync(mem[3 * i], s->S[0], n * se, hipMemcpyDeviceToDevice, s->st);
        if (e == hipSuccess) e = hipMemsetAsync(mem[3 * i + 1], 0, n * se, s->st);
        if (e == hipSuccess) e = hipMemcpyAsync(mem[3 * i + 2], s->flags, n, hipMemcpyDeviceToDevice, s->st);
        if (e != hipSuccess) { release(); return fail(FLUID_ERR_HIP, std::string("stencil_apply_hbm: ") + hipGetErrorString(e)); }
    }
    int rc = stencil_run(s, 3 * nsets, box_mode, nsets, (void* const (*)[3])mem.data(), nullptr);
    if (!rc) rc = stencil_run(s, reps, box_mode, nsets, (void* const (*)[3])mem.data(), avg_ms);
    if (!rc && hipMemcpyAsync(s->Q, mem[3 * ((reps - 1) % nsets) + 1], n * se, hipMemcpyDeviceToDevice, s->st) != hipSuccess) rc = fail(FLUID_ERR_HIP, "stencil_apply_hbm: copy back");
    hipStreamSynchronize(s->st);
    release();
    if (nsets_out) *nsets_out = nsets;
    return rc;
}

static int hook_device(int32_t device)
{
    int ndev = 0;
    if (hipGetDeviceCount(&ndev) != hipSuccess || ndev <= 0) return fail(FLUID_ERR_HIP, "no HIP device visible: libfluid_hip has no CPU path");
    if (device < 0 || device >= ndev) return fail(FLUID_ERR_ARG, "device ordinal out of range");
    HIPCHK(hipSetDevice(device));
    return FLUID_OK;
}

int fluid_spline_eval(int32_t device, int32_t which, int64_t n, const double* x, double* w)
{
    if (n < 0 || which < 0 || which > 3 || (n > 0 && (!x || !w))) return fail(FLUID_ERR_ARG, "bad argument");
    int rc = hook_device(device);
    if (rc || n == 0) return rc;
    double *dx = nullptr, *dw = nullptr;
    HIPCHK(hipMalloc((void**)&dx, n * sizeof(double)));
    HIPCHK(hipMalloc((void**)&dw, n * sizeof(double)));
    HIPCHK(hipMemcpy(dx, x, n * sizeof(double), hipMemcpyHostToDevice));
    launch_spline_eval(nullptr, which, (long)n, dx, dw);
    HIPCHK(hipGetLastError());
    HIPCHK(hipMemcpy(w, dw, n * sizeof(double), hipMemcpyDeviceToHost));
    hipFree(dx); hipFree(dw);
    return FLUID_OK;
}

int fluid_dot_eval(int32_t device, int64_t n, const double* a, const double* b, double* out)
{
    if (n < 0 || !out || (n > 0 && (!a || !b))) return fail(FLUID_ERR_ARG, "bad argument");
    int rc = hook_device(device);
    if (rc) return rc;
    double *da = nullptr, *db = nullptr, *dp = nullptr;
    const int nb = 1024;
    HIPCHK(hipMalloc((void**)&da, (n + 1) * sizeof(double)));
    HIPCHK(hipMalloc((void**)&db, (n + 1) * sizeof(double)));
    HIPCHK(hipMalloc((void**)&dp, (nb + 1) * sizeof(double)));
    if (n) {
        HIPCHK(hipMemcpy(da, a, n * sizeof(double), hipMemcpyHostToDevice));
        HIPCHK(hipMemcpy(db, b, n * sizeof(double), hipMemcpyHostToDevice));
    }
    launch_dot(nullptr, (long)n, da, db, dp, nb, dp + nb);
    HIPCHK(hipGetLastError());
    HIPCHK(hipMemcpy(out, dp + nb, sizeof(double), hipMemcpyDeviceToHost));
    hipFree(da); hipFree(db); hipFree(dp);
    return FLUID_OK;
}

int fluid_scan_eval(int32_t device, int32_t mode, int64_t n, int32_t in_offset, int32_t out_offset, const void* in, int32_t* out, int32_t* total)
{
    if (n <= 0 || n > 0x7fffffffL || mode < 0 || mode > 1 || in_offset < 0 || in_offset > 64 || out_offset < 0 || out_offset > 64 || !in || !out || !total)
        return fail(FLUID_ERR_ARG, "bad argument");
    int rc = hook_device(device);
    if (rc) return rc;
    const size_t ie = mode == 0 ? sizeof(int) : 1, guard = 16;
    const int fill = 0x5a5a5a5a;
    char* din = nullptr;
    int *dout = nullptr, *dsums = nullptr;
    HIPCHK(hipMalloc((void**)&din, ((size_t)n + in_offset + 64) * ie));
    HIPCHK(hipMalloc((void**)&dout, ((size_t)n + out_offset + 2 * guard + 1) * sizeof(int)));
    HIPCHK(hipMalloc((void**)&dsums, ((size_t)n / 2048 + 16) * sizeof(int)));
    HIPCHK(hipMemset(dout, 0x5a, ((size_t)n + out_offset + 2 * guard + 1) * sizeof(int)));
    HIPCHK(hipMemcpy(din + (size_t)in_offset * ie, in, (size_t)n * ie, hipMemcpyHostToDevice));
    int* o = dout + guard + out_offset;
    if (mode == 0) launch_exclusive_scan(nullptr, (const int*)din + in_offset, o, (long)n, dsums, o + n + guard);
    else launch_index_scan_flat(nullptr, (const uint8_t*)din + in_offset, o, (long)n, dsums, o + n + guard);
    HIPCHK(hipGetLastError());
    std::vector<int> h((size_t)n + 2 * guard + 1);
    HIPCHK(hipMemcpy(h.data(), o - guard, h.size() * sizeof(int), hipMemcpyDeviceToHost));
    hipFree(din); hipFree(dout); hipFree(dsums);
    for (size_t i = 0; i < guard; ++i)
        if (h[i] != fill || h[guard + (size_t)n + i] != fill) return fail(FLUID_ERR_STATE, "scan wrote outside out[0, n)");
    memcpy(out, h.data() + guard, (size_t)n * sizeof(int));
    *total = h[2 * guard + (size_t)n];
    return FLUID_OK;
}

int fluid_profile_enable(fluid_sim_t* s, int sample_every)
{
    if (!s || sample_every < 0) return fail(FLUID_ERR_ARG, "bad argument");
    s->prof_every = sample_every;
    return FLUID_OK;
}
int fluid_profile_read(fluid_sim_t* s, int klass, int64_t* n_launches, int64_t* n_sampled, double* total_ms, double* cells)
{
    if (!s || klass < 0 || klass >= FLUID_PROF_COUNT) return fail(FLUID_ERR_ARG, "bad argument");
    prof_resolve(s);
    const ProfClass& p = s->prof[klass];
    if (n_launches) *n_launches = p.launches;
    if (n_sampled) *n_sampled = p.sampled;
    if (total_ms) *total_ms = p.ms;
    if (cells) *cells = p.cells;
    return FLUID_OK;
}
int fluid_profile_reset(fluid_sim_t* s)
{
    if (!s) return fail(FLUID_ERR_ARG, "null handle");
    prof_resolve(s);
    for (int k = 0; k < FLUID_PROF_COUNT; ++k) {
        s->prof[k].launches = s->prof[k].sampled = 0;
        s->prof[k].ms = s->prof[k].cells = 0;
    }
    return FLUID_OK;
}

}
```

fluid-simulation_amd/csrc/fluid_sources.hip:

```cpp
#include "sim.h"
#include <algorithm>

using namespace fl;
#define fail fluid_fail

static uint64_t sm64_host(uint64_t x)
{
    uint64_t z = x + 0x9E3779B97F4A7C15ull;
    z = (z ^ (z >> 30)) * 0xBF58476D1CE4E5B9ull;
    z = (z ^ (z >> 27)) * 0x94D049BB133111EBull;
    return z ^ (z >> 31);
}

#define SRC_GUARD(s)                                                                                                     \
    if (!(s)) return fail(FLUID_ERR_ARG, "null handle");                                                                 \
    if ((s)->dist) return fail(FLUID_ERR_STATE, "these entry points are single-GPU only (they renumber the pids): a decomposed handle uses fluid_dist_set_source, fluid_dist_set_sink, fluid_dist_get_source_stats, fluid_dist_add_particles")

static bool box_from(const fluid_sim* s, const int32_t lo[3], const int32_t hi[3], Box& b)
{
    const int N = s->g.N;
    for (int a = 0; a < 3; ++a)
        if (lo[a] < 0 || hi[a] > N - 1 || lo[a] > hi[a]) return false;
    b = Box{lo[0], lo[1], lo[2], hi[0], hi[1], hi[2]};
    return true;
}

static int ensure_sums(fluid_sim* s)
{
    if (s->src_sums) return FLUID_OK;
    HIPCHK(hipMalloc((void**)&s->src_sums, ((size_t)INT32_MAX / 2048 + 16) * sizeof(int)));
    return FLUID_OK;
}

void fl::sources_free(fluid_sim* s)
{
    for (auto& q : s->src) {
        if (q.buf) hipFree(q.buf);
        q.buf = nullptr;
    }
    if (s->src_sums) hipFree(s->src_sums);
    s->src_sums = nullptr;
}

static int read_small(fluid_sim* s, int i)
{
    HIPCHK(hipMemcpyAsync(s->h_small + i, s->d_small + i, sizeof(int), hipMemcpyDeviceToHost, s->st));
    HIPCHK(hipStreamSynchronize(s->st));
    return FLUID_OK;
}

static int apply_sinks(fluid_sim* s, long* removed)
{
    *removed = 0;
    SinkSet sk{};
    for (int i = 0; i < FLUID_MAX_SINKS; ++i)
        if (s->sink_on[i]) sk.box[sk.n++] = s->sink[i];
    if (sk.n == 0 || s->np == 0) return FLUID_OK;
    const long n = s->np;
    const Particles a = s->pa.shifted(s->p_off);
    HIPCHK(hipMemsetAsync(s->d_small, 0, sizeof(int), s->st));
    launch_sink_mark(s->st, s->g, n, a, sk, nullptr, nullptr, s->d_small);
    HIPCHK(hipGetLastError());
    int rc = read_small(s, 0);
    if (rc) return rc;
    const long r = s->h_small[0];
    if (r == 0) return FLUID_OK;
    launch_sink_mark(s->st, s->g, n, a, sk, s->key, s->order, nullptr);
    launch_exclusive_scan(s->st, s->key, s->slot, n, s->src_sums, s->d_small + 2);
    launch_exclusive_scan(s->st, s->order, s->order2, n, s->src_sums, s->d_small + 3);
    launch_sink_compact(s->st, n, a, s->pb, s->key, s->slot, s->order2);
    HIPCHK(hipGetLastError());
    std::swap(s->pa, s->pb);
    s->p_off = 0;
    s->np = n - r;
    *removed = r;
    return FLUID_OK;
}

static int apply_source(fluid_sim* s, fluid_sim::SrcSlot& q, long t, long* emitted)
{
    *emitted = 0;
    const fluid_source_t& c = q.src;
    const Box b = q.box;
    const long B = b.cells();
    int *hist = q.buf, *cnt = q.buf + B, *off = q.buf + 2 * B;
    const bool fill = c.mode == FLUID_SOURCE_FILL;
    const uint64_t h0 = sm64_host(sm64_host(c.seed) ^ (uint64_t)t);
    if (fill) {
        HIPCHK(hipMemsetAsync(hist, 0, B * sizeof(int), s->st));
        launch_src_count(s->st, s->g, s->np, s->pa.shifted(s->p_off), b, hist);
    }
    launch_src_plan(s->st, s->g, b, h0, c.per_cell, fill, s->solid, hist, cnt);
    launch_exclusive_scan(s->st, cnt, off, B, s->src_sums, s->d_small + 1);
    HIPCHK(hipGetLastError());
    int rc = read_small(s, 1);
    if (rc) return rc;
    const long m = s->h_small[1];
    if (m == 0) return FLUID_OK;
    if (s->np + m > (long)INT32_MAX) return fail(FLUID_ERR_STATE, "a source would take the particle count past INT32_MAX");
    if ((rc = grow_particles(s, s->p_off + s->np + m))) return rc;
    const Particles p = s->pa.shifted(s->p_off + s->np);
    const double zero[3] = {0, 0, 0};
    launch_src_emit(s->st, s->g, b, h0, c.per_cell, fill, s->solid, hist, off, p, (uint32_t)s->np, c.vel_mode == FLUID_SOURCE_VEL_FIXED ? c.vel : zero);
    if (c.vel_mode == FLUID_SOURCE_VEL_GRID) launch_interp_from_grid(s->st, s->g, m, p, s->u, s->v, s->w);
    HIPCHK(hipGetLastError());
    s->np += m;
    *emitted = m;
    return FLUID_OK;
}

int fl::sources_apply(fluid_sim* s)
{
    s->src_emit_last = s->src_rm_last = 0;
    bool any = false;
    for (int i = 0; i < FLUID_MAX_SINKS; ++i) any = any || s->sink_on[i];
    for (const auto& q : s->src) any = any || q.on;
    if (!any) return FLUID_OK;
    s->binned = false;
    const long t = s->n_steps;
    long removed = 0, emitted = 0;
    int rc = apply_sinks(s, &removed);
    if (rc) return rc;
    for (auto& q : s->src) {
        if (!q.on || t % q.src.every != 0) continue;
        long m = 0;
        if ((rc = apply_source(s, q, t, &m))) return rc;
        emitted += m;
        if (m > 0 && !box_empty(s->Pb)) {
            Box& P = s->Pb;
            P = Box{std::min(P.x0, q.box.x0), std::min(P.y0, q.box.y0), std::min(P.z0, q.box.z0),
                    std::max(P.x1, q.box.x1), std::max(P.y1, q.box.y1), std::max(P.z1, q.box.z1)};
        }
    }
    s->src_emit_last = emitted, s->src_rm_last = removed;
    s->src_emit_total += emitted, s->src_rm_total += removed;
    if (emitted || removed) s->stats.paths |= FLUID_PATH_SOURCES;
    return FLUID_OK;
}

extern "C" {

int fluid_add_particles(fluid_sim_t* s, int64_t n, const double* pos, const double* vel)
{
    SRC_GUARD(s);
    if (n < 0 || (n > 0 && !pos)) return fail(FLUID_ERR_ARG, "bad particle arguments");
    if (!vel && !s->vel_ok) return fail(FLUID_ERR_STATE, "add_particles with vel == NULL needs the grid velocities of a completed step");
    if (s->np + (long)n > (long)INT32_MAX) return fail(FLUID_ERR_STATE, "more than INT32_MAX particles");
    if (n == 0) return FLUID_OK;
    HIPCHK(hipSetDevice(s->prm.device));
    int rc = grow_particles(s, s->p_off + s->np + (long)n);
    if (rc) return rc;
    HIPCHK(hipMemcpyAsync(s->stage_pos, pos, 3 * n * sizeof(double), hipMemcpyHostToDevice, s->st));
    if (vel) HIPCHK(hipMemcpyAsync(s->stage_vel, vel, 3 * n * sizeof(double), hipMemcpyHostToDevice, s->st));
    const Particles p = s->pa.shifted(s->p_off + s->np);
    launch_src_append(s->st, (long)n, s->stage_pos, vel ? s->stage_vel : nullptr, p, (uint32_t)s->np);
    if (!vel) launch_interp_from_grid(s->st, s->g, (long)n, p, s->u, s->v, s->w);
    HIPCHK(hipGetLastError());
    HIPCHK(hipStreamSynchronize(s->st));
    s->np += (long)n;
    s->sorted = s->have_p2g = s->have_flags = false;
    s->sort_hint = false;
    s->binned = false;
    return FLUID_OK;
}

int fluid_set_source(fluid_sim_t* s, int32_t slot, const fluid_source_t* src)
{
    SRC_GUARD(s);
    if (slot < 0 || slot >= FLUID_MAX_SOURCES) return fail(FLUID_ERR_ARG, "source slot out of range");
    auto& q = s->src[slot];
    HIPCHK(hipSetDevice(s->prm.device));
    if (!src) {
        HIPCHK(hipStreamSynchronize(s->st));
        if (q.buf) hipFree(q.buf);
        q = fluid_sim::SrcSlot{};
        return FLUID_OK;
    }
    Box b;
    if (!box_from(s, src->lo, src->hi, b)) return fail(FLUID_ERR_ARG, "source box empty or off the grid");
    if (src->per_cell < 1 || src->per_cell > 64) return fail(FLUID_ERR_ARG, "per_cell must be in 1..64");
    if (src->mode != FLUID_SOURCE_ADD && src->mode != FLUID_SOURCE_FILL) return fail(FLUID_ERR_ARG, "bad source mode");
    if (src->vel_mode != FLUID_SOURCE_VEL_FIXED && src->vel_mode != FLUID_SOURCE_VEL_GRID) return fail(FLUID_ERR_ARG, "bad source vel_mode");
    if (src->every < 1) return fail(FLUID_ERR_ARG, "every must be >= 1");
    if ((double)b.cells() * src->per_cell > (double)INT32_MAX) return fail(FLUID_ERR_ARG, "source box x per_cell exceeds INT32_MAX points");
    int rc = ensure_sums(s);
    if (rc) return rc;
    HIPCHK(hipStreamSynchronize(s->st));
    if (q.buf) hipFree(q.buf);
    q.buf = nullptr;
    q.on = false;
    HIPCHK(hipMalloc((void**)&q.buf, 3 * (size_t)b.cells() * sizeof(int)));
    q.src = *src;
    q.box = b;
    q.on = true;
    return FLUID_OK;
}

int fluid_set_sink(fluid_sim_t* s, int32_t slot, const int32_t lo[3], const int32_t hi[3])
{
    SRC_GUARD(s);
    if (slot < 0 || slot >= FLUID_MAX_SINKS) return fail(FLUID_ERR_ARG, "sink slot out of range");
    if (!lo) {
        s->sink_on[slot] = false;
        return FLUID_OK;
    }
    Box b;
    if (!hi || !box_from(s, lo, hi, b)) return fail(FLUID_ERR_ARG, "sink box empty or off the grid");
    HIPCHK(hipSetDevice(s->prm.device));
    int rc = ensure_sums(s);
    if (rc) return rc;
    s->sink[slot] = b;
    s->sink_on[slot] = true;
    return FLUID_OK;
}

int fluid_get_source_stats(fluid_sim_t* s, int64_t* emitted_last, int64_t* removed_last, int64_t* emitted_total, int64_t* removed_total)
{
    SRC_GUARD(s);
    if (emitted_last) *emitted_last = s->src_emit_last;
    if (removed_last) *removed_last = s->src_rm_last;
    if (emitted_total) *emitted_total = s->src_emit_total;
    if (removed_total) *removed_total = s->src_rm_total;
    return FLUID_OK;
}

}
```

fluid-simulation_amd/csrc/kernels_particles.hip:

```cpp
#include "common.h"

namespace fl {

struct BinAcc {
    int mn[3] = {0x7fffffff, 0x7fffffff, 0x7fffffff}, mx[3] = {-1, -1, -1};
    int nout = 0, cmax = 0;
};
__device__ __forceinline__ void bin_one(const Grid& g, long ncell, long i, double px, double py, double pz, bool dead, int* __restrict__ key,
                                        int* __restrict__ slot, int* __restrict__ cell_count, BinAcc& acc)
{
    int bx = (int)round(px) - g.cx0(), by = (int)round(py) - g.cy0(), bz = (int)round(pz) - g.cz0();
    bool in = bx >= 0 && bx < g.nx && by >= 0 && by < g.ny && bz >= 0 && bz < g.nz;
    int k = in ? (int)g.idx(bx, by, bz) : (int)ncell;
    if (dead) { k = (int)ncell + 1; in = false; }
    key[i] = k;
    {
        const int lane = threadIdx.x & 63;
        const int kp = __shfl_up(k, 1, 64);
        const bool head = lane == 0 || kp != k;
        const unsigned long long hm = __ballot(head);
        const unsigned long long below = hm & ((2ull << lane) - 1ull);
        const int start = 63 - __clzll((long long)below);
        const unsigned long long above = (lane == 63) ? 0ull : (hm >> (lane + 1)) << (lane + 1);
        const unsigned long long act = __ballot(true);
        const int stop = above ? __ffsll((long long)above) - 1 : 64 - __clzll((long long)act) + 0;
        int base = 0;
        if (head) {
            base = atomicAdd(&cell_count[k], stop - start);
            if (in && base + stop - start > acc.cmax) acc.cmax = base + stop - start;
        }
        base = __shfl(base, start, 64);
        slot[i] = base + (lane - start);
    }
    if (in) {
        acc.mn[0] = bx < acc.mn[0] ? bx : acc.mn[0]; acc.mx[0] = bx > acc.mx[0] ? bx : acc.mx[0];
        acc.mn[1] = by < acc.mn[1] ? by : acc.mn[1]; acc.mx[1] = by > acc.mx[1] ? by : acc.mx[1];
        acc.mn[2] = bz < acc.mn[2] ? bz : acc.mn[2]; acc.mx[2] = bz > acc.mx[2] ? bz : acc.mx[2];
    } else if (!dead) {
        acc.nout++;
    }
}
__device__ __forceinline__ void bin_block_partials(const BinAcc& acc, int (*sm)[8], int* __restrict__ part)
{
    const int lane = threadIdx.x & 63, w = threadIdx.x >> 6;
#pragma unroll
    for (int a = 0; a < 3; ++a) {
        int lo = acc.mn[a], hi = acc.mx[a];
#pragma unroll
        for (int o = 32; o > 0; o >>= 1) {
            int l2 = __shfl_down(lo, o, 64), h2 = __shfl_down(hi, o, 64);
            lo = l2 < lo ? l2 : lo;
            hi = h2 > hi ? h2 : hi;
        }
        if (lane == 0) { sm[w][a] = lo; sm[w][3 + a] = hi; }
    }
    const int nout = wave_sum(acc.nout);
    const int cmax = wave_max(acc.cmax);
    if (lane == 0) { sm[w][6] = nout; sm[w][7] = cmax; }
    __syncthreads();
    if (threadIdx.x < 8) {
        const int a = threadIdx.x;
        int v = sm[0][a];
        for (int k = 1; k < 4; ++k) {
            int t = sm[k][a];
            v = a < 3 ? (t < v ? t : v) : (a == 6 ? v + t : (t > v ? t : v));
        }
        part[blockIdx.x * 8 + a] = v;
    }
}

__global__ __launch_bounds__(256) void k_bin_count(Grid g, long n, Particles p, int* __restrict__ key, int* __restrict__ slot,
                                                   int* __restrict__ cell_count, int* __restrict__ part)
{
    __shared__ int sm[4][8];
    BinAcc acc;
    const long ncell = (long)g.cells();
    for (long i = (long)blockIdx.x * 256 + threadIdx.x; i < n; i += (long)gridDim.x * 256)
        bin_one(g, ncell, i, p.px[i], p.py[i], p.pz[i], p.pid[i] == PID_DEAD, key, slot, cell_count, acc);
    bin_block_partials(acc, sm, part);
}

__device__ __forceinline__ void bin_reduce(const int* __restrict__ part, int nb, StepState* ss, int (*sm)[8])
{
    int mn[3] = {0x7fffffff, 0x7fffffff, 0x7fffffff}, mx[3] = {-1, -1, -1}, nout = 0, cmax = 0;
    for (int b = threadIdx.x; b < nb; b += 256) {
#pragma unroll
        for (int a = 0; a < 3; ++a) {
            int l = part[b * 8 + a], h = part[b * 8 + 3 + a];
            mn[a] = l < mn[a] ? l : mn[a];
            mx[a] = h > mx[a] ? h : mx[a];
        }
        nout += part[b * 8 + 6];
        cmax = part[b * 8 + 7] > cmax ? part[b * 8 + 7] : cmax;
    }
    const int lane = threadIdx.x & 63, w = threadIdx.x >> 6;
#pragma unroll
    for (int a = 0; a < 3; ++a) {
        int lo = mn[a], hi = mx[a];
#pragma unroll
        for (int o = 32; o > 0; o >>= 1) {
            int l2 = __shfl_down(lo, o, 64), h2 = __shfl_down(hi, o, 64);
            lo = l2 < lo ? l2 : lo;
            hi = h2 > hi ? h2 : hi;
        }
        if (lane == 0) { sm[w][a] = lo; sm[w][3 + a] = hi; }
    }
    nout = wave_sum(nout);
    cmax = wave_max(cmax);
    if (lane == 0) { sm[w][6] = nout; sm[w][7] = cmax; }
    __syncthreads();
    if (threadIdx.x == 0) {
        for (int a = 0; a < 3; ++a) {
            int lo = sm[0][a], hi = sm[0][3 + a];
            for (int k = 1; k < 4; ++k) {
                lo = sm[k][a] < lo ? sm[k][a] : lo;
                hi = sm[k][3 + a] > hi ? sm[k][3 + a] : hi;
            }
            ss->bbox_min[a] = lo;
            ss->bbox_max[a] = hi;
        }
        ss->n_out = sm[0][6] + sm[1][6] + sm[2][6] + sm[3][6];
        int cm = sm[0][7];
        for (int k = 1; k < 4; ++k) cm = sm[k][7] > cm ? sm[k][7] : cm;
        ss->max_cell = cm;
    }
}

__global__ __launch_bounds__(256) void k_bin_bbox(const int* __restrict__ part, int nb, StepState* ss)
{
    __shared__ int sm[4][8];
    bin_reduce(part, nb, ss, sm);
}

__global__ __launch_bounds__(256) void k_bin_scatter(long n, const int* __restrict__ key, const int* __restrict__ slot,
                                                     const int* __restrict__ cell_start, const uint32_t* __restrict__ pid,
                                                     int* __restrict__ order, uint32_t* __restrict__ spid)
{
    long i = (long)blockIdx.x * 256 + threadIdx.x;
    if (i >= n) return;
    const int d = cell_start[key[i]] + slot[i];
    order[d] = (int)i;
    spid[d] = pid[i];
}

constexpr int RANK_CH = 2048;
__global__ __launch_bounds__(256) void k_bin_rank(long n_pos, long pos0, const int* __restrict__ key, const int* __restrict__ cell_start,
                                                  const int* __restrict__ order, const uint32_t* __restrict__ spid, int* __restrict__ order2)
{
    __shared__ uint32_t sid[RANK_CH];
    __shared__ int sAB[2];
    const long j = pos0 + (long)blockIdx.x * 256 + threadIdx.x;
    const long end = pos0 + n_pos;
    const bool act = j < end;
    int src = 0, a = 0, b = 0;
    uint32_t mine = 0;
    if (act) {
        src = order[j];
        const int k = key[src];
        a = cell_start[k];
        b = cell_start[k + 1];
        mine = spid[j];
    }
    if (threadIdx.x == 0) sAB[0] = a;
    if (act && (j + 1 == end || threadIdx.x == 255)) sAB[1] = b;
    __syncthreads();
    const int A = sAB[0], B = sAB[1];
    int rank = 0;
    for (int c0 = A; c0 < B; c0 += RANK_CH) {
        const int c1 = c0 + RANK_CH < B ? c0 + RANK_CH : B;
        if (c0 != A) __syncthreads();
        for (int t = c0 + threadIdx.x; t < c1; t += 256) sid[t - c0] = spid[t];
        __syncthreads();
        const int lo = a > c0 ? a : c0, hi = b < c1 ? b : c1;
        for (int t = lo; t < hi; ++t) rank += sid[t - c0] < mine;
    }
    if (act) order2[a + rank] = src;
}

__device__ __forceinline__ void axis_weights(double px, double py, double pz, double* __restrict__ w, long stride, long j)
{
    const double q[3] = {px, py, pz};
#pragma unroll
    for (int a = 0; a < 3; ++a) {
        const int b = (int)round(q[a]);
#pragma unroll
        for (int d = 0; d < 3; ++d) w[(a * 3 + d) * stride + j] = spline_at(q[a], b - 1 + d, d);
    }
}

__global__ __launch_bounds__(256) void k_reorder(long n, const int* __restrict__ order, Particles s, Particles d, double* __restrict__ w,
                                                 long wstride)
{
    long j = (long)blockIdx.x * 256 + threadIdx.x;
    if (j >= n) return;
    int i = order[j];
    const double px = s.px[i], py = s.py[i], pz = s.pz[i];
    d.px[j] = px; d.py[j] = py; d.pz[j] = pz;
    d.vx[j] = s.vx[i]; d.vy[j] = s.vy[i]; d.vz[j] = s.vz[i];
    d.pid[j] = s.pid[i];
    if (w) axis_weights(px, py, pz, w, wstride, j);
}

__global__ __launch_bounds__(256) void k_weights(long n, Particles p, double* __restrict__ w, long stride)
{
    long j = (long)blockIdx.x * 256 + threadIdx.x;
    if (j >= n) return;
    axis_weights(p.px[j], p.py[j], p.pz[j], w, stride, j);
}

constexpr int P2G_SLOTS = 256 * 4;
constexpr int P2G_THREADS = 192;
constexpr int P2G_CH = 384;
constexpr int P2G_SEG = P2G_CH / 8 + 1;
__device__ __forceinline__ int p2g_slot(int k) { return (k & 7) * P2G_SEG + (k >> 3); }
constexpr int P2G_LDS = 8 * P2G_SEG;
constexpr int P2G_HEAVY = 48;
constexpr int P2G_CROWD = 18;
constexpr int P2G_PIECE = 512;
constexpr int P2G_BUDGET = 8192;
constexpr int P2G_ZT = 62;

template <bool VEC, bool CROWD>
__global__ __launch_bounds__(P2G_THREADS, 3) void k_p2g_rows(Grid g, Box box, Particles p, const double* __restrict__ pw, long wstride,
                                                          const int* __restrict__ cell_start, double* __restrict__ part, long cells, int zt, const int* __restrict__ items,
                                                          Particles crowd, uint8_t* __restrict__ colflag, int ntz)
{
    __shared__ double sr[12][P2G_LDS];
    const int tid = threadIdx.x, e = tid >> 6, lane = tid & 63;
    for (int item = blockIdx.x; item < items[0]; item += gridDim.x) {
    const int4 wi = reinterpret_cast<const int4*>(items)[1 + item];
    const int rx = box.x0 - 1 + wi.x, Y0 = wi.y, Y1 = wi.z, tz0 = box.z0 + wi.w * zt;
    const int X = rx - 1 + e, zc = tz0 - 1 + lane;
    const bool colx = X >= box.x0 && X <= box.x1;
    const bool src = colx && zc >= 0 && zc < g.nz;
    const bool tgt = colx && lane >= 1 && lane <= zt && zc <= box.z1;
    const bool rowx = rx >= 0 && rx < g.nx;
    const int zlo = tz0 > 0 ? tz0 - 1 : 0, zhi = tz0 + zt < g.nz - 1 ? tz0 + zt : g.nz - 1;
    const double* swx = sr[e];
    double* const out = part + (long)(2 - e) * 4 * cells + (long)(X - box.x0) * box.ny() * box.nz() + (zc - box.z0);
    double C[3][4];
#pragma unroll
    for (int a = 0; a < 3; ++a)
#pragma unroll
        for (int q = 0; q < 4; ++q) C[a][q] = 0;
    int pjb = 0, pje = 0, nca = 0, ncz = 0;
    bool have = false;
    uint8_t* const cflag = colflag + ((long)(2 - e) * box.nx() + (X - box.x0)) * box.ny() * ntz + wi.w;
    for (int ry = Y0 - 1; ry <= Y1 + 1; ++ry) {
        const int ri = ry - (Y0 - 1);
        if ((ri & 63) == 0) {
            const int y = ry + lane;
            pjb = pje = 0;
            if (rowx && y >= 0 && y < g.ny && y <= Y1 + 1) {
                pjb = cell_start[g.idx(rx, y, zlo)];
                pje = cell_start[g.idx(rx, y, zhi) + 1];
            }
        }
        double T[3][3][4];
#pragma unroll
        for (int a = 0; a < 3; ++a)
#pragma unroll
            for (int d = 0; d < 3; ++d)
#pragma unroll
                for (int q = 0; q < 4; ++q) T[a][d][q] = 0;
        const int jb = __shfl(pjb, ri & 63, 64), je = __shfl(pje, ri & 63, 64);
        int ca = nca, cz = ncz;
        if (je > jb && !have && src) {
            const size_t r0 = g.idx(rx, ry, zc);
            ca = cell_start[r0];
            cz = cell_start[r0 + 1];
        }
        have = false;
        if (((ri + 1) & 63) != 0 && ry < Y1 + 1 && __shfl(pje, (ri + 1) & 63, 64) > __shfl(pjb, (ri + 1) & 63, 64)) {
            have = true;
            nca = ncz = 0;
            if (src) {
                const size_t r1 = g.idx(rx, ry + 1, zc);
                nca = cell_start[r1];
                ncz = cell_start[r1 + 1];
            }
        }
        if (je > jb) {
            const int ca_all = ca, n_all = cz - ca;
            if (CROWD && n_all >= P2G_CROWD) cz = ca;
            for (int cb = VEC ? (jb & ~1) : jb; cb < je; cb += P2G_CH) {
                const int ce = cb + P2G_CH < je ? cb + P2G_CH : je;
                if (CROWD) {
                    if (!__syncthreads_or((ca > cb ? ca : cb) < (cz < ce ? cz : ce))) continue;
                } else
                    __syncthreads();
                if (VEC) {
                    for (int j = cb + 2 * tid; j < ce; j += 2 * P2G_THREADS) {
                        const int k0 = p2g_slot(j - cb), k1 = p2g_slot(j + 1 - cb);
                        double2 t[6];
#pragma unroll
                        for (int q = 0; q < 6; ++q) t[q] = *reinterpret_cast<const double2*>(pw + q * wstride + j);
#pragma unroll
                        for (int q = 0; q < 6; ++q) { sr[q][k0] = t[q].x; sr[q][k1] = t[q].y; }
#pragma unroll
                        for (int q = 0; q < 3; ++q) t[q] = *reinterpret_cast<const double2*>(pw + (6 + q) * wstride + j);
                        t[3] = *reinterpret_cast<const double2*>(p.vx + j);
                        t[4] = *reinterpret_cast<const double2*>(p.vy + j);
                        t[5] = *reinterpret_cast<const double2*>(p.vz + j);
#pragma unroll
                        for (int q = 0; q < 6; ++q) { sr[6 + q][k0] = t[q].x; sr[6 + q][k1] = t[q].y; }
                    }
                } else {
                    for (int j = cb + tid; j < ce; j += P2G_THREADS) {
                        const int k = p2g_slot(j - cb);
#pragma unroll
                        for (int q = 0; q < 9; ++q) sr[q][k] = pw[q * wstride + j];
                        sr[9][k] = p.vx[j]; sr[10][k] = p.vy[j]; sr[11][k] = p.vz[j];
                    }
                }
                __syncthreads();
                int lo = ca > cb ? ca : cb, hi = cz < ce ? cz : ce;
                if (hi < lo) hi = lo;
                const bool heavy = !CROWD && hi - lo > P2G_HEAVY;
                if (!heavy) {
                    for (int j = lo; j < hi; ++j) {
                        const int k = p2g_slot(j - cb);
                        const double wx = swx[k];
                        const double vx = sr[9][k], vy = sr[10][k], vz = sr[11][k];
                        const double z0 = sr[6][k], z1 = sr[7][k], z2 = sr[8][k];
#pragma unroll
                        for (int a = 0; a < 3; ++a) {
                            const double xy = wx * sr[3 + a][k];
                            const double c0 = xy * z0, c1 = xy * z1, c2 = xy * z2;
                            T[a][0][0] += c0; T[a][0][1] = T[a][0][1] + c0 * vx; T[a][0][2] = T[a][0][2] + c0 * vy; T[a][0][3] = T[a][0][3] + c0 * vz;
                            T[a][1][0] += c1; T[a][1][1] = T[a][1][1] + c1 * vx; T[a][1][2] = T[a][1][2] + c1 * vy; T[a][1][3] = T[a][1][3] + c1 * vz;
                            T[a][2][0] += c2; T[a][2][1] = T[a][2][1] + c2 * vx; T[a][2][2] = T[a][2][2] + c2 * vy; T[a][2][3] = T[a][2][3] + c2 * vz;
                        }
                    }
                }
                unsigned long long hm = CROWD ? 0ull : __ballot(heavy);
                while (hm) {
                    const int L = __ffsll((long long)hm) - 1;
                    hm &= hm - 1;
                    const int lo_L = __shfl(lo, L, 64), hi_L = __shfl(hi, L, 64);
#pragma unroll
                    for (int a = 0; a < 3; ++a) {
                        double H[3][4];
#pragma unroll
                        for (int d = 0; d < 3; ++d)
#pragma unroll
                            for (int q = 0; q < 4; ++q) H[d][q] = 0;
                        for (int j = lo_L + lane; j < hi_L; j += 64) {
                            const int k = p2g_slot(j - cb);
                            const double xy = swx[k] * sr[3 + a][k];
                            const double vx = sr[9][k], vy = sr[10][k], vz = sr[11][k];
                            const double zw[3] = {sr[6][k], sr[7][k], sr[8][k]};
#pragma unroll
                            for (int d = 0; d < 3; ++d) {
                                const double cw = xy * zw[d];
                                H[d][0] += cw; H[d][1] += cw * vx; H[d][2] += cw * vy; H[d][3] += cw * vz;
                            }
                        }
#pragma unroll
                        for (int d = 0; d < 3; ++d)
#pragma unroll
                            for (int q = 0; q < 4; ++q) {
                                const double t = __shfl(wave_sum(H[d][q]), 0, 64);
                                if (lane == L) T[a][d][q] += t;
                            }
                    }
                }
            }
            if (CROWD) {
                const double* c0 = e == 0 ? crowd.px : (e == 1 ? crowd.pz : crowd.vy);
                const double* c1 = e == 0 ? crowd.py : (e == 1 ? crowd.vx : crowd.vz);
                if (n_all >= P2G_CROWD) {
                    for (int at = ca_all; at < ca_all + n_all; at += P2G_PIECE) {
                        const long o18 = ca_all + 18L * ((at - ca_all) / P2G_PIECE);
#pragma unroll
                        for (int a = 0; a < 3; ++a)
#pragma unroll
                            for (int d = 0; d < 3; ++d)
#pragma unroll
                                for (int q = 0; q < 4; ++q) {
                                    const int Lr = a * 12 + d * 4 + q;
                                    T[a][d][q] += (Lr < 18 ? c0 : c1)[o18 + Lr % 18];
                                }
                    }
                }
            }
        }
#pragma unroll
        for (int a = 0; a < 3; ++a)
#pragma unroll
            for (int q = 0; q < 4; ++q) {
                const double below = __shfl_up(T[a][2][q], 1, 64), above = __shfl_down(T[a][0][q], 1, 64);
                C[a][q] = ((C[a][q] + below) + T[a][1][q]) + above;
            }
        if (ry - 1 >= Y0 && colx) {
            const bool any = __any(tgt && C[0][0] != 0);
            if (lane == 0) cflag[(long)(ry - 1 - box.y0) * ntz] = any;
            if (any && tgt) {
                double* o = out + (long)(ry - 1 - box.y0) * box.nz();
#pragma unroll
                for (int q = 0; q < 4; ++q) o[q * cells] = C[0][q];
            }
        }
#pragma unroll
        for (int q = 0; q < 4; ++q) { C[0][q] = C[1][q]; C[1][q] = C[2][q]; C[2][q] = 0; }
    }
    }
}

constexpr int PC_WAVES = 4;
typedef double pc_d4 __attribute__((ext_vector_type(4)));
__global__ __launch_bounds__(256) void k_p2g_crowd_list(Grid g, Box box, const int* __restrict__ cell_start, int2* __restrict__ list, int* __restrict__ count)
{
    __shared__ int s_w[4], s_base;
    const int nz = box.nz(), ny = box.ny(), nz4 = (nz + 3) / 4;
    const long i = (long)blockIdx.x * 256 + threadIdx.x;
    int first[5] = {0, 0, 0, 0, 0};
    int pieces = 0;
    if (i < (long)box.nx() * ny * nz4) {
        const int z = 4 * (int)(i % nz4), y = (int)((i / nz4) % ny), x = (int)(i / ((long)nz4 * ny));
        const int* cs = cell_start + g.idx(box.x0 + x, box.y0 + y, box.z0 + z);
        const int m = nz - z < 4 ? nz - z : 4;
#pragma unroll
        for (int k = 0; k < 5; ++k) first[k] = cs[k <= m ? k : m];
#pragma unroll
        for (int k = 0; k < 4; ++k) {
            const int n = first[k + 1] - first[k];
            pieces += n >= P2G_CROWD ? (n + P2G_PIECE - 1) / P2G_PIECE : 0;
        }
    }
    const int lane = threadIdx.x & 63, wv = threadIdx.x >> 6;
    int inc = pieces;
#pragma unroll
    for (int o = 1; o < 64; o <<= 1) {
        const int u = __shfl_up(inc, o, 64);
        if (lane >= o) inc += u;
    }
    if (lane == 63) s_w[wv] = inc;
    __syncthreads();
    if (threadIdx.x == 0) {
        const int tot = s_w[0] + s_w[1] + s_w[2] + s_w[3];
        s_base = tot ? atomicAdd(count, tot) : 0;
    }
    __syncthreads();
    if (!pieces) return;
    int at = s_base + inc - pieces;
    for (int w = 0; w < wv; ++w) at += s_w[w];
#pragma unroll
    for (int k = 0; k < 4; ++k) {
        const int n = first[k + 1] - first[k];
        if (n < P2G_CROWD) continue;
        for (int j = 0; j * P2G_PIECE < n; ++j) {
            const int len = n - j * P2G_PIECE < P2G_PIECE ? n - j * P2G_PIECE : P2G_PIECE;
            list[at++] = make_int2(first[k] + j * P2G_PIECE, (j << 9) | (len - 1));
        }
    }
}
__global__ __launch_bounds__(64 * PC_WAVES) void k_p2g_crowd_sum(Particles p, const double* __restrict__ pw, long wstride,
                                                                const int2* __restrict__ list, int* __restrict__ count, Particles park)
{
    __shared__ double sw[PC_WAVES][12][64];
    const int wv = threadIdx.x >> 6, lane = threadIdx.x & 63;
    const int n = lane & 15, gq = lane >> 4;
    const int total = count[0];
    double(*my)[64] = sw[wv];
    const double* ax = my[n < 9 ? n / 3 : 0];
    const double* ay = my[3 + (n < 9 ? n % 3 : 0)];
    const double* bz = my[6 + (n < 12 ? n >> 2 : 0)];
    const double* bv = my[8 + ((n & 3) ? (n & 3) : 1)];
    for (int ent = blockIdx.x * PC_WAVES + wv; ent < total; ent += gridDim.x * PC_WAVES) {
        const int2 en = list[ent];
        const int piece = en.y >> 9, lo = en.x, hi = lo + (en.y & 511) + 1, ca = lo - P2G_PIECE * piece;
        pc_d4 D = {0, 0, 0, 0};
        for (int b = lo; b < hi; b += 64) {
            const int j = b + lane;
            const bool ok = j < hi;
            double v[12];
#pragma unroll
            for (int q = 0; q < 9; ++q) v[q] = ok ? pw[q * wstride + j] : 0.0;
            v[9] = ok ? p.vx[j] : 0.0, v[10] = ok ? p.vy[j] : 0.0, v[11] = ok ? p.vz[j] : 0.0;
            __builtin_amdgcn_wave_barrier();
#pragma unroll
            for (int q = 0; q < 12; ++q) my[q][lane] = v[q];
            __builtin_amdgcn_wave_barrier();
            const int nb = hi - b < 64 ? hi - b : 64;
#pragma unroll 4
            for (int s4 = 0; s4 < 16; ++s4) {
                if (4 * s4 >= nb) break;
                const int k = 4 * s4 + gq;
                const double A = n < 9 ? ax[k] * ay[k] : 0.0;
                const double zw = bz[k], zv = zw * bv[k];
                const double B = n < 12 ? ((n & 3) ? zv : zw) : 0.0;
                D = __builtin_amdgcn_mfma_f64_16x16x4f64(A, B, D, 0, 0, 0);
            }
        }
        if (n < 12) {
// ... 138 lines not shown
                __syncthreads();
                int lo = ca > cb ? ca : cb, hi = cz < ce ? cz : ce;
                if (hi < lo) hi = lo;
                const bool heavy = hi - lo > P2G_HEAVY;
                if (!heavy) {
                    for (int j = lo; j < hi; ++j) {
                        const int k = p2gt_slot(j - cb);
                        const double a = swx[k] * swy[k];
                        const double vx = sv[0][k], vy = sv[1][k], vz = sv[2][k];
#pragma unroll
                        for (int d = 0; d < 3; ++d) {
                            const double cw = a * sw[6 + d][k];
                            S[d] += cw;
                            U[d] = U[d] + cw * vx;
                            V[d] = V[d] + cw * vy;
                            W[d] = W[d] + cw * vz;
                        }
                    }
                }
                unsigned long long hm = __ballot(heavy);
                while (hm) {
                    const int L = __ffsll((long long)hm) - 1;
                    hm &= hm - 1;
                    const int lo_L = __shfl(lo, L, 64), hi_L = __shfl(hi, L, 64);
                    double ps[3] = {0, 0, 0}, pu[3] = {0, 0, 0}, pv[3] = {0, 0, 0}, pq[3] = {0, 0, 0};
                    for (int j = lo_L + lane; j < hi_L; j += 64) {
                        const int k = p2gt_slot(j - cb);
                        const double a = swx[k] * swy[k];
                        const double vx = sv[0][k], vy = sv[1][k], vz = sv[2][k];
#pragma unroll
                        for (int d = 0; d < 3; ++d) {
                            const double cw = a * sw[6 + d][k];
                            ps[d] += cw;
                            pu[d] += cw * vx;
                            pv[d] += cw * vy;
                            pq[d] += cw * vz;
                        }
                    }
#pragma unroll
                    for (int d = 0; d < 3; ++d) {
                        double t0 = wave_sum(ps[d]), t1 = wave_sum(pu[d]), t2 = wave_sum(pv[d]), t3 = wave_sum(pq[d]);
                        t0 = __shfl(t0, 0, 64); t1 = __shfl(t1, 0, 64); t2 = __shfl(t2, 0, 64); t3 = __shfl(t3, 0, 64);
                        if (lane == L) { S[d] += t0; U[d] += t1; V[d] += t2; W[d] += t3; }
                    }
                }
            }
            const double s0 = __shfl_up(S[2], 1, 64), s2 = __shfl_down(S[0], 1, 64);
            const double u0 = __shfl_up(U[2], 1, 64), u2 = __shfl_down(U[0], 1, 64);
            const double v0 = __shfl_up(V[2], 1, 64), v2 = __shfl_down(V[0], 1, 64);
            const double w0 = __shfl_up(W[2], 1, 64), w2 = __shfl_down(W[0], 1, 64);
            if (live) {
                wf = (float)((double)wf + s0);
                wf = (float)((double)wf + S[1]);
                wf = (float)((double)wf + s2);
                su = ((su + u0) + U[1]) + u2;
                sv_ = ((sv_ + v0) + V[1]) + v2;
                sw_ = ((sw_ + w0) + W[1]) + w2;
            }
        }
    }
    if (!live) return;
    if (wf > 0) {
        const double wd = (double)wf;
        su /= wd; sv_ /= wd; sw_ /= wd;
    }
    container[c] = wf;
    u[c] = su; v[c] = sv_; w[c] = sw_;
    ub[c] = su; vb[c] = sv_; wb[c] = sw_;
}

__global__ __launch_bounds__(256) void k_g2p(Grid g, long n, Particles p, const double* __restrict__ dcx, const double* __restrict__ dcy,
                                             const double* __restrict__ dcz, const double* __restrict__ pcx, const double* __restrict__ pcy,
                                             const double* __restrict__ pcz, double blend, StepState* ss)
{
    __shared__ double sm[4];
    long i = (long)blockIdx.x * 256 + threadIdx.x;
    double len = 0;
    if (i < n && p.pid[i] != PID_DEAD) {
        const double cx = p.px[i], cy = p.py[i], cz = p.pz[i];
        const int wlo = g.lo + 2, whi = g.hi - 2;
        const int fcx = (int)round(cx), fcy = (int)round(cy), fcz = (int)round(cz);
        double wx[3], wy[3], wz[3];
        int ox[3], oy[3], oz[3];
        const int sxs = (int)g.sx();
#pragma unroll
        for (int d = 0; d < 3; ++d) {
            const int ax = fcx - 1 + d, ay = fcy - 1 + d, az = fcz - 1 + d;
            wx[d] = (ax >= wlo && ax <= whi) ? spline_at(cx, ax, d) : 0.0;
            wy[d] = (ay >= wlo && ay <= whi) ? spline_at(cy, ay, d) : 0.0;
            wz[d] = (az >= wlo && az <= whi) ? spline_at(cz, az, d) : 0.0;
            ox[d] = (min(max(ax, g.cx0()), g.cx1()) - g.cx0()) * sxs;
            oy[d] = (min(max(ay, g.cy0()), g.cy1()) - g.cy0()) * g.nz;
            oz[d] = min(max(az, g.cz0()), g.cz1()) - g.cz0();
        }
        double weight = 0, d0 = 0, d1 = 0, d2 = 0, q0 = 0, q1 = 0, q2 = 0;
#pragma unroll
        for (int xi = 0; xi < 3; ++xi)
#pragma unroll
            for (int yi = 0; yi < 3; ++yi)
#pragma unroll
                for (int zi = 0; zi < 3; ++zi) {
                    const int c = ox[xi] + oy[yi] + oz[zi];
                    const double cw = wx[xi] * wy[yi] * wz[zi];
                    weight += cw;
                    d0 += dcx[c] * cw;
                    d1 += dcy[c] * cw;
                    d2 += dcz[c] * cw;
                    if (pcx) {
                        q0 += pcx[c] * cw;
                        q1 += pcy[c] * cw;
                        q2 += pcz[c] * cw;
                    }
                }
        double vx = p.vx[i], vy = p.vy[i], vz = p.vz[i];
        if (weight != 0) {
            vx += d0 / weight;
            vy += d1 / weight;
            vz += d2 / weight;
            if (pcx) {
                vx = blend * vx + (1.0 - blend) * (q0 / weight);
                vy = blend * vy + (1.0 - blend) * (q1 / weight);
                vz = blend * vz + (1.0 - blend) * (q2 / weight);
            }
            p.vx[i] = vx; p.vy[i] = vy; p.vz[i] = vz;
        }
        len = sqrt(vx * vx + vy * vy + vz * vz);
        if (!(len == len)) len = 0;
    }
    len = wave_max(len);
    if ((threadIdx.x & 63) == 0) sm[threadIdx.x >> 6] = len;
    __syncthreads();
    if (threadIdx.x == 0) {
        double m = sm[0];
        for (int k = 1; k < 4; ++k) m = sm[k] > m ? sm[k] : m;
        if (m > 0) atomicMax(&ss->max_speed_bits, (unsigned long long)__double_as_longlong(m));
    }
}

constexpr int G2P_TX = 4, G2P_TY = 4, G2P_TZ = 30;
template <bool PIC>
__global__ __launch_bounds__(256) void k_g2p_tiled(Grid g, Box pb, Particles p, const int* __restrict__ cell_start,
                                                   const double* __restrict__ dcx, const double* __restrict__ dcy,
                                                   const double* __restrict__ dcz, const double* __restrict__ pcx,
                                                   const double* __restrict__ pcy, const double* __restrict__ pcz, double blend, StepState* ss)
{
    constexpr int LX = G2P_TX + 2, LY = G2P_TY + 2, LZ = G2P_TZ + 2, LN = LX * LY * LZ, NROW = G2P_TX * G2P_TY;
    __shared__ double sf[PIC ? 6 : 3][LN];
    __shared__ int srow[NROW][2];
    __shared__ double sm[4];
    const int tid = threadIdx.x;
    const int nty = (pb.ny() + G2P_TY - 1) / G2P_TY, ntz = (pb.nz() + G2P_TZ - 1) / G2P_TZ;
    const int tile = blockIdx.x;
    const int tz = tile % ntz, ty = (tile / ntz) % nty, tx = tile / (ntz * nty);
    const int x0 = pb.x0 + tx * G2P_TX, y0 = pb.y0 + ty * G2P_TY, z0 = pb.z0 + tz * G2P_TZ;
    const int z1 = z0 + G2P_TZ - 1 < pb.z1 ? z0 + G2P_TZ - 1 : pb.z1;
    if (tid < NROW) {
        const int cx = x0 + tid / G2P_TY, cy = y0 + tid % G2P_TY;
        int a = 0, b = 0;
        if (cx <= pb.x1 && cy <= pb.y1) {
            a = cell_start[g.idx(cx, cy, z0)];
            b = cell_start[g.idx(cx, cy, z1) + 1];
        }
        srow[tid][0] = a;
        srow[tid][1] = b;
    }
    for (int t = tid; t < LN; t += 256) {
        const int lx = t / (LY * LZ), r = t - lx * (LY * LZ), ly = r / LZ, lz = r - ly * LZ;
        const int gx = x0 - 1 + lx, gy = y0 - 1 + ly, gz = z0 - 1 + lz;
        const bool in = gx >= 0 && gx < g.nx && gy >= 0 && gy < g.ny && gz >= 0 && gz < g.nz;
        const size_t c = in ? g.idx(gx, gy, gz) : 0;
        sf[0][t] = in ? dcx[c] : 0.0;
        sf[1][t] = in ? dcy[c] : 0.0;
        sf[2][t] = in ? dcz[c] : 0.0;
        if (PIC) {
            sf[PIC ? 3 : 0][t] = in ? pcx[c] : 0.0;
            sf[PIC ? 4 : 0][t] = in ? pcy[c] : 0.0;
            sf[PIC ? 5 : 0][t] = in ? pcz[c] : 0.0;
        }
    }
    __syncthreads();
    const int wlo = g.lo + 2, whi = g.hi - 2;
    double len = 0;
    for (int row = 0; row < NROW; ++row) {
        const int a = srow[row][0], b = srow[row][1];
        for (int i = a + tid; i < b; i += 256) {
            const double cx = p.px[i], cy = p.py[i], cz = p.pz[i];
            const int fcx = (int)round(cx), fcy = (int)round(cy), fcz = (int)round(cz);
            double wx[3], wy[3], wz[3];
#pragma unroll
            for (int d = 0; d < 3; ++d) {
                const int ax = fcx - 1 + d, ay = fcy - 1 + d, az = fcz - 1 + d;
                wx[d] = (ax >= wlo && ax <= whi) ? spline_at(cx, ax, d) : 0.0;
                wy[d] = (ay >= wlo && ay <= whi) ? spline_at(cy, ay, d) : 0.0;
                wz[d] = (az >= wlo && az <= whi) ? spline_at(cz, az, d) : 0.0;
            }
            const int lb = ((fcx - g.cx0() - x0) * LY + (fcy - g.cy0() - y0)) * LZ + (fcz - g.cz0() - z0);
            double weight = 0, d0 = 0, d1 = 0, d2 = 0, q0 = 0, q1 = 0, q2 = 0;
#pragma unroll
            for (int xi = 0; xi < 3; ++xi)
#pragma unroll
                for (int yi = 0; yi < 3; ++yi)
#pragma unroll
                    for (int zi = 0; zi < 3; ++zi) {
                        const int c = lb + (xi * LY + yi) * LZ + zi;
                        const double cw = wx[xi] * wy[yi] * wz[zi];
                        weight += cw;
                        d0 += sf[0][c] * cw;
                        d1 += sf[1][c] * cw;
                        d2 += sf[2][c] * cw;
                        if (PIC) {
                            q0 += sf[PIC ? 3 : 0][c] * cw;
                            q1 += sf[PIC ? 4 : 0][c] * cw;
                            q2 += sf[PIC ? 5 : 0][c] * cw;
                        }
                    }
            double vx = p.vx[i], vy = p.vy[i], vz = p.vz[i];
            if (weight != 0) {
                vx += d0 / weight;
                vy += d1 / weight;
                vz += d2 / weight;
                if (PIC) {
                    vx = blend * vx + (1.0 - blend) * (q0 / weight);
                    vy = blend * vy + (1.0 - blend) * (q1 / weight);
                    vz = blend * vz + (1.0 - blend) * (q2 / weight);
                }
                p.vx[i] = vx; p.vy[i] = vy; p.vz[i] = vz;
            }
            double l = sqrt(vx * vx + vy * vy + vz * vz);
            if (!(l == l)) l = 0;
            len = l > len ? l : len;
        }
    }
    len = wave_max(len);
    if ((tid & 63) == 0) sm[tid >> 6] = len;
    __syncthreads();
    if (tid == 0) {
        double m = sm[0];
        for (int k = 1; k < 4; ++k) m = sm[k] > m ? sm[k] : m;
        if (m > 0) atomicMax(&ss->max_speed_bits, (unsigned long long)__double_as_longlong(m));
    }
}

__device__ __forceinline__ bool is_solid(const Grid& g, const uint8_t* flags, int x, int y, int z)
{
    if (x < g.cx0() || x > g.cx1() || y < g.cy0() || y > g.cy1() || z < g.cz0() || z > g.cz1()) return false;
    return flags[g.idx(x - g.cx0(), y - g.cy0(), z - g.cz0())] & F_SOLID;
}

__device__ __forceinline__ double advect_timestep(double max_dt, double dx, const StepState* ss)
{
    const double maxSpeed = __longlong_as_double((long long)ss->max_speed_bits);
    if (maxSpeed != 0) return max_dt < dx / maxSpeed ? max_dt : dx / maxSpeed;
    return max_dt;
}
__device__ __forceinline__ void advect_one(const Grid& g, const Particles& p, const uint8_t* __restrict__ flags, double timestep, long i, double& P0,
                                           double& P1, double& P2)
{
    const double e = 0;
    P0 = p.px[i], P1 = p.py[i], P2 = p.pz[i];
    double V0 = p.vx[i], V1 = p.vy[i], V2 = p.vz[i];
    const double q0 = P0 + timestep * V0, q1 = P1 + timestep * V1, q2 = P2 + timestep * V2;
    if (is_solid(g, flags, (int)round(q0), (int)round(q1), (int)round(q2))) {
        const double vx = V0 * timestep, vy = V1 * timestep, vz = V2 * timestep;
        if (is_solid(g, flags, (int)round(P0 + vx), (int)P1, (int)P2)) V0 *= -1.0 * e;
        if (is_solid(g, flags, (int)P0, (int)round(P1 + vy), (int)P2)) V1 *= -1.0 * e;
        if (is_solid(g, flags, (int)P0, (int)P1, (int)round(P2 + vz))) V2 *= -1.0 * e;
        P0 += V0 * timestep; P1 += V1 * timestep; P2 += V2 * timestep;
        p.vx[i] = V0; p.vy[i] = V1; p.vz[i] = V2;
    } else {
        P0 = q0; P1 = q1; P2 = q2;
    }
    p.px[i] = P0; p.py[i] = P1; p.pz[i] = P2;
}

__global__ __launch_bounds__(256) void k_advect(Grid g, long n, Particles p, const uint8_t* __restrict__ flags, double max_dt, double dx,
                                                StepState* ss)
{
    const double timestep = advect_timestep(max_dt, dx, ss);
    long i = (long)blockIdx.x * 256 + threadIdx.x;
    if (i < n && p.pid[i] != PID_DEAD) {
        double P0, P1, P2;
        advect_one(g, p, flags, timestep, i, P0, P1, P2);
    }
}

__global__ __launch_bounds__(256) void k_advect_bin(Grid g, long n, Particles p, const uint8_t* __restrict__ flags, double max_dt, double dx,
                                                    StepState* ss, int* __restrict__ key, int* __restrict__ slot, int* __restrict__ cell_count,
                                                    int* __restrict__ part)
{
    __shared__ int sm[4][8];
    const double timestep = advect_timestep(max_dt, dx, ss);
    BinAcc acc;
    const long ncell = (long)g.cells();
    for (long i = (long)blockIdx.x * 256 + threadIdx.x; i < n; i += (long)gridDim.x * 256) {
        const bool dead = p.pid[i] == PID_DEAD;
        double P0, P1, P2;
        if (!dead) advect_one(g, p, flags, timestep, i, P0, P1, P2);
        else P0 = p.px[i], P1 = p.py[i], P2 = p.pz[i];
        bin_one(g, ncell, i, P0, P1, P2, dead, key, slot, cell_count, acc);
    }
    bin_block_partials(acc, sm, part);
}

__global__ __launch_bounds__(256) void k_publish_dt(double max_dt, double dx, StepState* ss, const int* __restrict__ part, int nb)
{
    __shared__ int sm[4][8];
    if (nb > 0) bin_reduce(part, nb, ss, sm);
    if (threadIdx.x == 0) ss->dt = advect_timestep(max_dt, dx, ss);
}

__global__ __launch_bounds__(256) void k_unpack_records(long n, const double* __restrict__ rec, Particles p, long off)
{
    long j = (long)blockIdx.x * 256 + threadIdx.x;
    if (j >= n) return;
    const double* d = rec + (size_t)j * 7;
    p.px[off + j] = d[0]; p.py[off + j] = d[1]; p.pz[off + j] = d[2];
    p.vx[off + j] = d[3]; p.vy[off + j] = d[4]; p.vz[off + j] = d[5];
    p.pid[off + j] = (uint32_t)d[6];
}
__global__ __launch_bounds__(256) void k_pack_records(long n, Particles p, long off, double* __restrict__ rec)
{
    long j = (long)blockIdx.x * 256 + threadIdx.x;
    if (j >= n) return;
    double* d = rec + (size_t)j * 7;
    d[0] = p.px[off + j]; d[1] = p.py[off + j]; d[2] = p.pz[off + j];
    d[3] = p.vx[off + j]; d[4] = p.vy[off + j]; d[5] = p.vz[off + j];
    d[6] = (double)p.pid[off + j];
}
__global__ __launch_bounds__(256) void k_unpack_ids(long n, const double* __restrict__ pos, const double* __restrict__ vel,
                                                    const uint32_t* __restrict__ ids, Particles p)
{
    long j = (long)blockIdx.x * 256 + threadIdx.x;
    if (j >= n) return;
    p.px[j] = pos[3 * j]; p.py[j] = pos[3 * j + 1]; p.pz[j] = pos[3 * j + 2];
    if (vel) { p.vx[j] = vel[3 * j]; p.vy[j] = vel[3 * j + 1]; p.vz[j] = vel[3 * j + 2]; }
    else { p.vx[j] = 0; p.vy[j] = 0; p.vz[j] = 0; }
    p.pid[j] = ids[j];
}
__global__ __launch_bounds__(256) void k_pack_ids(long n, Particles p, long off, double* __restrict__ pos, double* __restrict__ vel,
                                                  uint32_t* __restrict__ ids)
{
    long j = (long)blockIdx.x * 256 + threadIdx.x;
    if (j >= n) return;
    pos[3 * j] = p.px[off + j]; pos[3 * j + 1] = p.py[off + j]; pos[3 * j + 2] = p.pz[off + j];
    vel[3 * j] = p.vx[off + j]; vel[3 * j + 1] = p.vy[off + j]; vel[3 * j + 2] = p.vz[off + j];
    ids[j] = p.pid[off + j];
}

__global__ __launch_bounds__(256) void k_pack(long n, Particles p, double* __restrict__ pos, double* __restrict__ vel)
{
    long j = (long)blockIdx.x * 256 + threadIdx.x;
    if (j >= n) return;
    const size_t o = 3 * (size_t)p.pid[j];
    pos[o] = p.px[j]; pos[o + 1] = p.py[j]; pos[o + 2] = p.pz[j];
    vel[o] = p.vx[j]; vel[o + 1] = p.vy[j]; vel[o + 2] = p.vz[j];
}
__global__ __launch_bounds__(256) void k_unpack(long n, const double* __restrict__ pos, const double* __restrict__ vel, Particles p)
{
    long j = (long)blockIdx.x * 256 + threadIdx.x;
    if (j >= n) return;
    p.px[j] = pos[3 * j]; p.py[j] = pos[3 * j + 1]; p.pz[j] = pos[3 * j + 2];
    if (vel) { p.vx[j] = vel[3 * j]; p.vy[j] = vel[3 * j + 1]; p.vz[j] = vel[3 * j + 2]; }
    else { p.vx[j] = 0; p.vy[j] = 0; p.vz[j] = 0; }
    p.pid[j] = (uint32_t)j;
}

static inline unsigned nblk(long n) { return (unsigned)((n + 255) / 256); }

void launch_bin_count(hipStream_t st, Grid g, long n, Particles p, int* key, int* slot, int* cell_count, int* part, StepState* ss)
{
    if (n <= 0) return;
    unsigned nb = nblk(n);
    if (nb > 1024) nb = 1024;
    hipLaunchKernelGGL(k_bin_count, dim3(nb), dim3(256), 0, st, g, n, p, key, slot, cell_count, part);
    hipLaunchKernelGGL(k_bin_bbox, dim3(1), dim3(256), 0, st, (const int*)part, (int)nb, ss);
}
void launch_bin_scatter(hipStream_t st, long n, const int* key, const int* slot, const int* cell_start, const uint32_t* pid, int* order,
                         uint32_t* spid)
{
    if (n > 0) hipLaunchKernelGGL(k_bin_scatter, dim3(nblk(n)), dim3(256), 0, st, n, key, slot, cell_start, pid, order, spid);
}
void launch_bin_rank(hipStream_t st, long n_pos, long pos0, const int* key, const int* cell_start, const int* order, const uint32_t* spid,
                     int* order2)
{
    if (n_pos > 0) hipLaunchKernelGGL(k_bin_rank, dim3(nblk(n_pos)), dim3(256), 0, st, n_pos, pos0, key, cell_start, order, spid, order2);
}
void launch_reorder(hipStream_t st, long n, const int* order, Particles src, Particles dst, double* w, long wstride)
{
    if (n > 0) hipLaunchKernelGGL(k_reorder, dim3(nblk(n)), dim3(256), 0, st, n, order, src, dst, w, wstride);
}
void launch_weights(hipStream_t st, long n, Particles p, double* w, long stride)
{
    if (n > 0) hipLaunchKernelGGL(k_weights, dim3(nblk(n)), dim3(256), 0, st, n, p, w, stride);
}
static void p2g_cut(const Box& box, int& ntz, int& zt, int& nseg)
{
    ntz = (box.nz() + P2G_ZT - 1) / P2G_ZT;
    zt = (box.nz() + ntz - 1) / ntz;
    nseg = 1;
    long best = -1;
    const long per = (long)(box.nx() + 2) * ntz;
    for (int k = 1; k <= box.ny(); ++k) {
        const long ys = (box.ny() + k - 1) / k, rounds = (per * k + P2G_SLOTS - 1) / P2G_SLOTS, cost = rounds * (ys + 2);
        if (best < 0 || cost < best) { best = cost; nseg = k; }
    }
}
size_t p2g_part_doubles(Box box)
{
    int ntz, zt, nseg;
    p2g_cut(box, ntz, zt, nseg);
    return (size_t)12 * box.cells() + ((size_t)3 * box.nx() * box.ny() * ntz + 7) / 8 + 8;
}
long p2g_max_items(Box box)
{
    int ntz, zt, nseg;
    p2g_cut(box, ntz, zt, nseg);
    return (long)(box.nx() + 2) * box.ny() * ntz;
}
void launch_p2g(hipStream_t st, Grid g, Box box, Particles p, const double* pw, long wstride, const int* cell_start, const uint8_t* flags,
                double* part, int* items, float* container, double* u, double* v, double* w, double* ub, double* vb, double* wb, int2* crowd_list,
                Particles park)
{
    int ntz, zt, nseg;
    p2g_cut(box, ntz, zt, nseg);
    const long cells = box.cells();
    const int budget = P2G_BUDGET;
    const unsigned nt = (unsigned)((box.nx() + 2) * nseg * ntz);
    hipLaunchKernelGGL(k_p2g_items, dim3(nblk((long)(box.nx() + 2) * nseg)), dim3(256), 0, st, g, box, cell_start, nseg, ntz, budget, items);
    const bool vec = ((((uintptr_t)pw | (uintptr_t)p.vx | (uintptr_t)p.vy | (uintptr_t)p.vz) & 15) == 0) && (wstride & 1) == 0;
    uint8_t* colflag = reinterpret_cast<uint8_t*>(part + 12 * cells);
    if (crowd_list) {
        Box sb = box;
        sb.x0 = sb.x0 > 0 ? sb.x0 - 1 : 0, sb.y0 = sb.y0 > 0 ? sb.y0 - 1 : 0, sb.z0 = sb.z0 > 0 ? sb.z0 - 1 : 0;
        sb.x1 = sb.x1 < g.nx - 1 ? sb.x1 + 1 : g.nx - 1, sb.y1 = sb.y1 < g.ny - 1 ? sb.y1 + 1 : g.ny - 1, sb.z1 = sb.z1 < g.nz - 1 ? sb.z1 + 1 : g.nz - 1;
        hipLaunchKernelGGL(k_p2g_crowd_list, dim3(nblk((long)sb.nx() * sb.ny() * ((sb.nz() + 3) / 4))), dim3(256), 0, st, g, sb, cell_start, crowd_list, items + 1);
        hipLaunchKernelGGL(k_p2g_crowd_sum, dim3(2048), dim3(64 * PC_WAVES), 0, st, p, pw, wstride, crowd_list, items + 1, park);
        if (vec) hipLaunchKernelGGL((k_p2g_rows<true, true>), dim3(nt), dim3(P2G_THREADS), 0, st, g, box, p, pw, wstride, cell_start, part, cells, zt, items, park, colflag, ntz);
        else hipLaunchKernelGGL((k_p2g_rows<false, true>), dim3(nt), dim3(P2G_THREADS), 0, st, g, box, p, pw, wstride, cell_start, part, cells, zt, items, park, colflag, ntz);
    } else if (vec) hipLaunchKernelGGL((k_p2g_rows<true, false>), dim3(nt), dim3(P2G_THREADS), 0, st, g, box, p, pw, wstride, cell_start, part, cells, zt, items, park, colflag, ntz);
    else hipLaunchKernelGGL((k_p2g_rows<false, false>), dim3(nt), dim3(P2G_THREADS), 0, st, g, box, p, pw, wstride, cell_start, part, cells, zt, items, park, colflag, ntz);
    hipLaunchKernelGGL(k_p2g_combine, dim3(nblk(cells)), dim3(256), 0, st, g, box, part, cells, flags, container, u, v, w, ub, vb, wb, items, colflag, zt, ntz);
}
void launch_p2g_tiles(hipStream_t st, Grid g, Box box, Particles p, const double* pw, long wstride, const int* cell_start, const uint8_t* flags,
                      float* container, double* u, double* v, double* w, double* ub, double* vb, double* wb)
{
    const int ntz = (box.nz() + P2G_ZT - 1) / P2G_ZT, zt = (box.nz() + ntz - 1) / ntz;
    const unsigned nt = (unsigned)(((box.nx() + P2GT_T - 1) / P2GT_T) * ((box.ny() + P2GT_T - 1) / P2GT_T) * ntz);
    hipLaunchKernelGGL(k_p2g_tiles, dim3(nt), dim3(P2GT_THREADS), 0, st, g, box, p, pw, wstride, cell_start, flags, container, u, v, w, ub, vb, wb, zt);
}
void launch_g2p_tiled(hipStream_t st, Grid g, Box pb, Particles p, const int* cell_start, const double* dcx, const double* dcy, const double* dcz,
                      const double* pcx, const double* pcy, const double* pcz, double blend, StepState* ss)
{
    if (pb.cells() <= 0) return;
    const unsigned nt = (unsigned)(((pb.nx() + G2P_TX - 1) / G2P_TX) * ((pb.ny() + G2P_TY - 1) / G2P_TY) * ((pb.nz() + G2P_TZ - 1) / G2P_TZ));
    if (pcx) hipLaunchKernelGGL(k_g2p_tiled<true>, dim3(nt), dim3(256), 0, st, g, pb, p, cell_start, dcx, dcy, dcz, pcx, pcy, pcz, blend, ss);
    else hipLaunchKernelGGL(k_g2p_tiled<false>, dim3(nt), dim3(256), 0, st, g, pb, p, cell_start, dcx, dcy, dcz, pcx, pcy, pcz, blend, ss);
}
void launch_g2p(hipStream_t st, Grid g, long n, Particles p, const double* dcx, const double* dcy, const double* dcz, const double* pcx,
                const double* pcy, const double* pcz, double blend, StepState* ss)
{
    if (n > 0) hipLaunchKernelGGL(k_g2p, dim3(nblk(n)), dim3(256), 0, st, g, n, p, dcx, dcy, dcz, pcx, pcy, pcz, blend, ss);
}
void launch_advect(hipStream_t st, Grid g, long n, Particles p, const uint8_t* flags, double max_dt, double dx, StepState* ss)
{
    if (n > 0) hipLaunchKernelGGL(k_advect, dim3(nblk(n)), dim3(256), 0, st, g, n, p, flags, max_dt, dx, ss);
    hipLaunchKernelGGL(k_publish_dt, dim3(1), dim3(1), 0, st, max_dt, dx, ss, (const int*)nullptr, 0);
}
void launch_advect_bin(hipStream_t st, Grid g, long n, Particles p, const uint8_t* flags, double max_dt, double dx, StepState* ss, int* key,
                       int* slot, int* cell_count, int* part)
{
    unsigned nb = nblk(n);
    if (nb > 1024) nb = 1024;
    hipLaunchKernelGGL(k_advect_bin, dim3(nb), dim3(256), 0, st, g, n, p, flags, max_dt, dx, ss, key, slot, cell_count, part);
    hipLaunchKernelGGL(k_publish_dt, dim3(1), dim3(256), 0, st, max_dt, dx, ss, (const int*)part, (int)nb);
}
void launch_unpack_records(hipStream_t st, long n, const double* rec, Particles p, long off)
{
    if (n > 0) hipLaunchKernelGGL(k_unpack_records, dim3(nblk(n)), dim3(256), 0, st, n, rec, p, off);
}
void launch_pack_records(hipStream_t st, long n, Particles p, long off, double* rec)
{
    if (n > 0) hipLaunchKernelGGL(k_pack_records, dim3(nblk(n)), dim3(256), 0, st, n, p, off, rec);
}
void launch_unpack_ids(hipStream_t st, long n, const double* pos, const double* vel, const uint32_t* ids, Particles p)
{
    if (n > 0) hipLaunchKernelGGL(k_unpack_ids, dim3(nblk(n)), dim3(256), 0, st, n, pos, vel, ids, p);
}
void launch_pack_ids(hipStream_t st, long n, Particles p, long off, double* pos, double* vel, uint32_t* ids)
{
    if (n > 0) hipLaunchKernelGGL(k_pack_ids, dim3(nblk(n)), dim3(256), 0, st, n, p, off, pos, vel, ids);
}
void launch_pack_particles(hipStream_t st, long n, Particles p, double* pos_aos, double* vel_aos)
{
    if (n > 0) hipLaunchKernelGGL(k_pack, dim3(nblk(n)), dim3(256), 0, st, n, p, pos_aos, vel_aos);
}
void launch_unpack_particles(hipStream_t st, long n, const double* pos_aos, const double* vel_aos, Particles p)
{
    if (n > 0) hipLaunchKernelGGL(k_unpack, dim3(nblk(n)), dim3(256), 0, st, n, pos_aos, vel_aos, p);
}

}
```

fluid-simulation_amd/csrc/sim.h:

```cpp
#pragma once
#include "common.h"
#include "../../include/fluid_hip.h"

#include <cmath>
#include <cstdio>
#include <cstdlib>
#include <cstring>
#include <string>
#include <utility>
#include <vector>

int fluid_fail(int code, const std::string& msg);
#define HIPCHK(expr)                                                                                              \
    do {                                                                                                          \
        hipError_t e_ = (expr);                                                                                   \
        if (e_ != hipSuccess)                                                                                     \
            return fluid_fail(FLUID_ERR_HIP, std::string(#expr) + ": " + hipGetErrorString(e_) + " @" + std::to_string(__LINE__)); \
    } while (0)

using namespace fl;

struct ProfClass {
    long launches = 0, sampled = 0;
    double ms = 0, cells = 0;
    std::vector<hipEvent_t> e0, e1;
    std::vector<double> pc;
};

struct fluid_sim {
    fluid_params_t prm;
    Grid g;
    size_t ncell = 0;
    hipStream_t st = nullptr;
    uint8_t *solid = nullptr, *flags = nullptr;
    float *container = nullptr, *rhs = nullptr, *diver = nullptr, *diver2 = nullptr;
    double *u = nullptr, *v = nullptr, *w = nullptr, *ub = nullptr, *vb = nullptr, *wb = nullptr;
    double *dcx = nullptr, *dcy = nullptr, *dcz = nullptr, *pressure = nullptr;
    double* p_guess = nullptr;
    bool warm = true, have_guess = false;
    double* p_guess2 = nullptr;
    long guess_step = -1, guess2_step = -1;
    int guess_pass = -1, guess2_pass = -1;
    long step_counter = 0;
    bool extrapolate = true;
    double* p_q = nullptr;
    long q_step = -1;
    void start_guess(const double*& g1, const double*& g2, double& ca, double& cb) const
    {
        g1 = p_guess, g2 = nullptr, ca = 1.0, cb = 0.0;
        const int k = stats.outer_passes;
        const bool same_step = p_guess2 && k >= 2 && guess_step == step_counter && guess2_step == step_counter && guess_pass == k - 1 && guess2_pass == k - 2;
        const double f = 1.0 - prm.update_frac;
        if (extrapolate && same_step) {
            g2 = p_guess2, ca = 1.0 + f, cb = -f;
        } else if (extrapolate && p_q && q_step >= 0 && step_counter - q_step <= 4 && k == 1 && guess_step == step_counter && guess_pass == 0) {
            g2 = p_q, ca = f, cb = 1.0;
        }
    }
    bool make_q() const { return warm && p_q && stats.outer_passes == 1 && guess_step == step_counter && guess_pass == 1 && guess2_step == step_counter && guess2_pass == 0; }
    void rotate_guess()
    {
        std::swap(p_guess, p_guess2);
        guess2_step = guess_step, guess2_pass = guess_pass;
        guess_step = step_counter, guess_pass = stats.outer_passes;
    }
    int *indices = nullptr, *scan_sums = nullptr, *ipart = nullptr;
    void *R = nullptr, *S[2] = {nullptr, nullptr}, *Q = nullptr, *X = nullptr, *Zmg = nullptr;
    double *pcx = nullptr, *pcy = nullptr, *pcz = nullptr;
    uint8_t* cntL = nullptr;
    LBox L{};
    size_t lmax = 0;
    double *part_bb = nullptr, *part_rr = nullptr, *part_rz[2] = {nullptr, nullptr}, *part_pq = nullptr, *part_err = nullptr;
    PcgState* ps = nullptr;
    PcgState* h_ps = nullptr;
    hipEvent_t ev_poll[2] = {nullptr, nullptr};
    long np = 0, cap = 0;
    Particles pa{}, pb{};
    int *key = nullptr, *slot = nullptr, *order = nullptr, *order2 = nullptr, *cell_count = nullptr, *cell_start = nullptr;
    uint32_t* spid = nullptr;
    double *stage_pos = nullptr, *stage_vel = nullptr;
    double* pw = nullptr;
    double* p2g_part = nullptr;
    size_t p2g_part_cap = 0;
    int2* p2g_crowd = nullptr;
    size_t p2g_crowd_cap = 0;
    int* p2g_items = nullptr;
    size_t p2g_items_cap = 0;
    int max_cell = 0;
    uint8_t* tl_flags = nullptr;
    int *tl_mg = nullptr, *tl_sq = nullptr;
    size_t tl_cap = 0;
    int n_tl_mg = 0, n_tl_sq = 0;
    int *row_flags = nullptr, *row_pos = nullptr, *row_list = nullptr;
    size_t row_cap = 0;
    int n_rows = 0;
    bool rows_on = true;
    bool drops_on = true;
    bool row_sweeps = true;
    int* drop_ctr = nullptr;
    int* drop_n = nullptr;
    int* drop_cells = nullptr;
    int n_drop = 0;
    int drop_last = -1;
    int drop_min = 4000;
    int drop_skipped = 0;
    bool lists_hint = false;
    bool lists_on = false;
    int lists_force = -1;
    int p2g_force = 0;
    long p2g_ref_cells = 0;
    long last_num_active = 0;
    StepState* ss = nullptr;
    StepState* h_ss = nullptr;
    Box Pb{0, 0, 0, -1, -1, -1}, Rb{0, 0, 0, -1, -1, -1}, Sb{0, 0, 0, -1, -1, -1};
    Box dirty{0, 0, 0, -1, -1, -1};
    int flag_x0 = 0, flag_x1 = -1;
    bool flags_valid = false;
    bool sorted = false, have_p2g = false, have_flags = false;
    long n_out = 0;
    bool sort_hint = false;
    bool advect_bin = true;
    bool binned = false;
    int bin_x0 = 0, bin_x1 = -1;
    int bin_min[3] = {0, 0, 0}, bin_max[3] = {-1, -1, -1}, bin_n_out = 0, bin_max_cell = 0;
    bool solve_tail = true;
    bool tail_ran = false;
    double dt = 0.1;
    fluid_step_stats_t stats{};
    static constexpr int MG_MAXL = 8;
    int mg_nl = 0, mg_tail = 0;
    long mg_last_iters_k[3] = {0, 0, 0};
    int pass_class() const { return stats.outer_passes < 2 ? stats.outer_passes : 2; }
    int mg_csweeps = 3;
    MLevel mgl[MG_MAXL];
    uint8_t *mg_typ[MG_MAXL] = {}, *mg_cnt[MG_MAXL] = {};
    int gal_mode = 1;
    int gal_it[2] = {-1, -1};
    int gal_since_probe = 0;
    bool gal_eligible = false;
    bool gal = false;
    int gal_lc = 0;
    double gal_dt = 0;
    double gal_wc = 1.8;
    int gal_sweeps = 3;
    char* gal_slab = nullptr;
    size_t gal_slab_cap = 0;
    float* gal_c[MG_MAXL][4] = {};
    uint8_t* gal_cnt[MG_MAXL] = {};
    uint8_t* gal_tfl[MG_MAXL] = {};
    char *mg_u[MG_MAXL] = {}, *mg_v[MG_MAXL] = {}, *mg_f[MG_MAXL] = {}, *mg_r[MG_MAXL] = {};
    double mg_wc[4] = {1.25, 1.1, 1.0, 1.0};
    bool mg_fp32 = true;
    double* mg_part = nullptr;
    char* mg_slab = nullptr;
    size_t mg_slab_cap = 0;
    bool dist = false;
    struct DistState* ds = nullptr;
    long p_off = 0;
    int* d_small = nullptr;
    int* h_small = nullptr;
    struct SrcSlot {
        bool on = false;
        fluid_source_t src{};
        Box box{};
        int* buf = nullptr;
    };
    SrcSlot src[FLUID_MAX_SOURCES];
    Box sink[FLUID_MAX_SINKS] = {};
    bool sink_on[FLUID_MAX_SINKS] = {};
    int* src_sums = nullptr;
    long n_steps = 0;
    bool vel_ok = false;
    long src_emit_last = 0, src_rm_last = 0, src_emit_total = 0, src_rm_total = 0;
    struct OutState* out = nullptr;
    int out_every = 0;
    int prof_every = 0;
    ProfClass prof[FLUID_PROF_COUNT];
};

namespace fl {
inline bool box_empty(const Box& b) { return b.x1 < b.x0 || b.y1 < b.y0 || b.z1 < b.z0; }
Box clip_dilate(const Box& b, int d, const Grid& g);
template <typename T>
inline hipError_t dalloc(T** p, size_t n)
{
    hipError_t e = hipMalloc((void**)p, n * sizeof(T));
    if (e == hipSuccess) e = hipMemset(*p, 0, n * sizeof(T));
    return e;
}
inline size_t solver_elem(const fluid_sim* s) { return s->prm.precision == FLUID_PRECISION_FP32 ? 4 : 8; }
inline bool use_mg(const fluid_sim* s) { return s->prm.preconditioner == FLUID_PRECOND_MG && s->prm.precision == FLUID_PRECISION_FP64; }

int prof_begin(fluid_sim* s, int k, double cells);
void prof_end(fluid_sim* s, int k, int tok);
int alloc_particles(fluid_sim* s, long n);
int grow_particles(fluid_sim* s, long need);
int read_ss(fluid_sim* s);
int sort_pass(fluid_sim* s, int ax0, int ax1, int* h_tail = nullptr);
int clear_dirty(fluid_sim* s);
int run_p2g(fluid_sim* s, const Box& box);
template <typename T>
Coef<T> make_coef(const fluid_sim* s);
MgCoef<double> mg_coef(const fluid_sim* s, int level);
hipError_t zero_search(fluid_sim* s, size_t lb);
int phase_flags(fluid_sim* s);
int phase_pressure_pass(fluid_sim* s, double* error);
int pic_fields(fluid_sim* s);
int fluid_create_window(const fluid_params_t* p, const Grid& g, fluid_sim_t** out);

int sources_apply(fluid_sim* s);
void sources_free(fluid_sim* s);

void output_free(fluid_sim* s);
int output_auto_check(fluid_sim* s);
int output_auto(fluid_sim* s);
void output_move(fluid_sim* from, fluid_sim* to);

int dist_step(fluid_sim* s, fluid_step_stats_t* stats);
void dist_destroy(fluid_sim* s);
int dist_download_field(fluid_sim* s, int field, void* dst, size_t bytes, bool* handled);
void dist_keep_solid(fluid_sim* s, const uint8_t* solid_global);
}
```

Baseline: 157.2.

## Launch binned sort speculatively before host readback and overlap MG setup with state copy

After binned advection, the scan/scatter/rank/reorder kernels are now queued before the host waits on the step-state readback. A device-side go flag, computed in the dt-publish kernel from the bbox check, makes those kernels exit early when the speculation misses. The next phase_sort then skips relaunching them. The flags phase likewise starts the search-buffer zeroing and multigrid setup before synchronizing on the async state copy. Both changes cut host-device round-trip stalls, at the cost of more complex state handling and wasted launches when a guess fails.

Result: no change. 157.4 (median of 2 runs) (+0.1%).

```diff
diff --git a/fluid-simulation_amd/csrc/common.h b/fluid-simulation_amd/csrc/common.h
--- a/fluid-simulation_amd/csrc/common.h
+++ b/fluid-simulation_amd/csrc/common.h
@@ -87,6 +87,7 @@
     int n_rows, n_l1_old;
     int n_tl_int, n_tl_bnd;
     int n_l1_gal, n_drop_fail;
+    int sort_go;
     unsigned long long max_speed_bits;
     double dt;
     double err_num;
@@ -201,10 +202,13 @@
 
 void launch_bin_count(hipStream_t st, Grid g, long n, Particles p, int* key, int* slot, int* cell_count, int* part, StepState* ss);
 void launch_bin_scatter(hipStream_t st, long n, const int* key, const int* slot, const int* cell_start, const uint32_t* pid, int* order,
-                         uint32_t* spid);
+                         uint32_t* spid, const int* go = nullptr);
 void launch_bin_rank(hipStream_t st, long n_pos, long pos0, const int* key, const int* cell_start, const int* order, const uint32_t* spid,
                      int* order2);
-void launch_reorder(hipStream_t st, long n, const int* order, Particles src, Particles dst, double* w = nullptr, long wstride = 0);
+void launch_bin_rank(hipStream_t st, long n_pos, long pos0, const int* key, const int* cell_start, const int* order, const uint32_t* spid,
+                     int* order2, const int* go);
+void launch_reorder(hipStream_t st, long n, const int* order, Particles src, Particles dst, double* w = nullptr, long wstride = 0,
+                    const int* go = nullptr);
 void launch_weights(hipStream_t st, long n, Particles p, double* w, long stride);
 void launch_axpby_box(hipStream_t st, Grid g, Box box, double a, const double* x, double b, const double* y, double* out, const PcgState* gate = nullptr);
 long p2g_max_items(Box box);
@@ -221,7 +225,7 @@
                 const double* pcy, const double* pcz, double blend, StepState* ss);
 void launch_advect(hipStream_t st, Grid g, long n, Particles p, const uint8_t* flags, double max_dt, double dx, StepState* ss);
 void launch_advect_bin(hipStream_t st, Grid g, long n, Particles p, const uint8_t* flags, double max_dt, double dx, StepState* ss, int* key,
-                       int* slot, int* cell_count, int* part);
+                       int* slot, int* cell_count, int* part, int go_lo = 0, int go_hi = -1);
 void launch_pack_particles(hipStream_t st, long n, Particles p, double* pos_aos, double* vel_aos);
 void launch_unpack_records(hipStream_t st, long n, const double* rec, Particles p, long off);
 void launch_pack_records(hipStream_t st, long n, Particles p, long off, double* rec);
diff --git a/fluid-simulation_amd/csrc/fluid_api.hip b/fluid-simulation_amd/csrc/fluid_api.hip
--- a/fluid-simulation_amd/csrc/fluid_api.hip
+++ b/fluid-simulation_amd/csrc/fluid_api.hip
@@ -74,7 +74,7 @@
     s->order2 = nullptr; s->spid = nullptr; hipFree(s->pw);
     s->pw = nullptr;
     s->key = s->slot = s->order = nullptr;
-    s->binned = false;
+    s->drop_binned();
     s->stage_pos = s->stage_vel = nullptr;
     s->cap = 0;
 }
@@ -83,6 +83,7 @@
 {
     if (n <= s->cap) return FLUID_OK;
     n = (n + 1) & ~1L;
+    if (s->st) HIPCHK(hipStreamSynchronize(s->st));
     free_particles(s);
     for (Particles* p : {&s->pa, &s->pb}) {
         HIPCHK(dalloc(&p->px, n)); HIPCHK(dalloc(&p->py, n)); HIPCHK(dalloc(&p->pz, n));
@@ -227,6 +228,8 @@
     if (const char* e = getenv("FLUID_DROPLETS_MIN")) s->drop_min = atoi(e);
     if (const char* e = getenv("FLUID_ADVECT_BIN")) s->advect_bin = atoi(e) != 0;
     if (const char* e = getenv("FLUID_SOLVE_TAIL")) s->solve_tail = atoi(e) != 0;
+    if (const char* e = getenv("FLUID_SORT_AHEAD")) s->sort_ahead = atoi(e) != 0;
+    if (const char* e = getenv("FLUID_SETUP_AHEAD")) s->setup_ahead = atoi(e) != 0;
     *out = nullptr;
     auto bail = [&](int rc) { fluid_destroy(s); return rc; };
 #define A(expr) do { hipError_t e_ = (expr); if (e_ != hipSuccess) return bail(fail(FLUID_ERR_HIP, std::string(#expr) + ": " + hipGetErrorString(e_))); } while (0)
@@ -333,7 +336,7 @@
     s->sorted = s->have_p2g = s->have_flags = false;
     s->have_guess = false;
     s->sort_hint = false;
-    s->binned = false;
+    s->drop_binned();
     s->vel_ok = false;
     return FLUID_OK;
 }
@@ -434,46 +437,60 @@
     return read_ss(s);
 }
 
-static int sort_binned(fluid_sim* s)
+struct SortPlan {
+    int ax0, ax1;
+    bool guess, binned;
+};
+static SortPlan sort_plan(const fluid_sim* s)
+{
+    SortPlan p{0, s->g.nx - 1, false, false};
+    p.guess = s->sort_hint && !box_empty(s->Pb);
+    if (p.guess) {
+        p.ax0 = std::max(0, s->Pb.x0 - 3);
+        p.ax1 = std::min(s->g.nx - 1, s->Pb.x1 + 3);
+    }
+    p.binned = s->binned && p.guess && p.ax0 == s->bin_x0 && p.ax1 == s->bin_x1 && s->np > 0;
+    return p;
+}
+static bool sort_missed(const fluid_sim* s, const SortPlan& p, const int* bmin, const int* bmax)
+{
+    return p.guess && bmax[0] >= 0 && (bmin[0] < std::min(p.ax0 + 2, s->Pb.x0) || bmax[0] > std::max(p.ax1 - 2, s->Pb.x1));
+}
+static int sort_binned_launch(fluid_sim* s, const int* go = nullptr)
 {
     const Grid g = s->g;
     const long ncell = (long)s->ncell, n2 = g.sx();
     const long c0 = (long)s->bin_x0 * n2, c1 = (long)(s->bin_x1 + 1) * n2;
-    launch_zero_step_state(s->st, s->ss, g.N);
     launch_exclusive_scan(s->st, s->cell_count + c0, s->cell_start + c0, c1 - c0, s->scan_sums, s->cell_start + c1);
     launch_sort_tail(s->st, s->cell_count, s->cell_start, c1, ncell);
-    launch_bin_scatter(s->st, s->np, s->key, s->slot, s->cell_start, s->pa.shifted(s->p_off).pid, s->order, s->spid);
-    launch_bin_rank(s->st, s->np, 0, s->key, s->cell_start, s->order, s->spid, s->order2);
-    HIPCHK(hipGetLastError());
-    StepState& h = *s->h_ss;
-    for (int a = 0; a < 3; ++a) h.bbox_min[a] = s->bin_min[a], h.bbox_max[a] = s->bin_max[a];
-    h.n_out = s->bin_n_out;
-    h.max_cell = s->bin_max_cell;
+    launch_bin_scatter(s->st, s->np, s->key, s->slot, s->cell_start, s->pa.shifted(s->p_off).pid, s->order, s->spid, go);
+    launch_bin_rank(s->st, s->np, 0, s->key, s->cell_start, s->order, s->spid, s->order2, go);
+    launch_reorder(s->st, s->np, s->order2, s->pa.shifted(s->p_off), s->pb, s->pw, s->cap, go);
+    HIPCHK(hipGetLastError());
     return FLUID_OK;
 }
 
 static int phase_sort(fluid_sim* s)
 {
     const Grid g = s->g;
-    int tok = prof_begin(s, FLUID_PROF_SORT, (double)s->np);
-    int ax0 = 0, ax1 = g.nx - 1;
-    const bool guess = s->sort_hint && !box_empty(s->Pb);
-    if (guess) {
-        ax0 = std::max(0, s->Pb.x0 - 3);
-        ax1 = std::min(g.nx - 1, s->Pb.x1 + 3);
-    }
-    const bool binned = s->binned && guess && ax0 == s->bin_x0 && ax1 == s->bin_x1 && s->np > 0;
-    s->binned = false;
-    const auto missed = [&](const int* bmin, const int* bmax) {
-        return guess && bmax[0] >= 0 && (bmin[0] < std::min(ax0 + 2, s->Pb.x0) || bmax[0] > std::max(ax1 - 2, s->Pb.x1));
-    };
+    const SortPlan pl = sort_plan(s);
+    const bool binned = pl.binned && !sort_missed(s, pl, s->bin_min, s->bin_max);
+    const bool ahead = s->presorted && binned;
+    const int tok = ahead ? -1 : prof_begin(s, FLUID_PROF_SORT, (double)s->np);
+    s->drop_binned();
     int rc;
-    if (binned && !missed(s->bin_min, s->bin_max)) {
-        if ((rc = sort_binned(s))) return rc;
+    if (binned) {
+        launch_zero_step_state(s->st, s->ss, g.N);
+        if (!ahead && (rc = sort_binned_launch(s))) return rc;
+        HIPCHK(hipGetLastError());
+        StepState& h = *s->h_ss;
+        for (int a = 0; a < 3; ++a) h.bbox_min[a] = s->bin_min[a], h.bbox_max[a] = s->bin_max[a];
+        h.n_out = s->bin_n_out;
+        h.max_cell = s->bin_max_cell;
     } else {
-        rc = binned ? FLUID_OK : sort_pass(s, ax0, ax1);
+        rc = pl.binned ? FLUID_OK : sort_pass(s, pl.ax0, pl.ax1);
         if (rc) return rc;
-        if (binned || missed(s->h_ss->bbox_min, s->h_ss->bbox_max)) {
+        if (pl.binned || sort_missed(s, pl, s->h_ss->bbox_min, s->h_ss->bbox_max)) {
             if ((rc = sort_pass(s, 0, g.nx - 1))) return rc;
         }
     }
@@ -492,8 +509,10 @@
     } else {
         s->Rb = s->Sb = s->Pb;
     }
-    launch_reorder(s->st, s->np, s->order2, s->pa.shifted(s->p_off), s->pb, s->pw, s->cap);
-    HIPCHK(hipGetLastError());
+    if (!binned) {
+        launch_reorder(s->st, s->np, s->order2, s->pa.shifted(s->p_off), s->pb, s->pw, s->cap);
+        HIPCHK(hipGetLastError());
+    }
     std::swap(s->pa, s->pb);
     s->p_off = 0;
     prof_end(s, FLUID_PROF_SORT, tok);
@@ -942,10 +961,12 @@
     s->flag_x1 = none ? -1 : s->Sb.x1;
     s->flags_valid = true;
     HIPCHK(hipGetLastError());
-    bool built = false, drops = false;
+    bool built = false, drops = false, setup_done = false;
     s->n_drop = 0;
+    size_t lb = 0;
     if (!box_empty(s->Rb)) {
         s->L = make_lbox(s->Rb);
+        lb = (s->L.cells() + 2 * (size_t)s->L.Lz) * solver_elem(s);
         launch_cnt_local(s->st, s->g, s->L, s->flags, s->cntL);
         if (use_mg(s) && (s->lists_force >= 0 ? s->lists_force == 1 : s->lists_hint)) {
             const MLevel m0 = mg_level0(s->L);
@@ -990,10 +1011,20 @@
                 launch_row_list(s->st, s->L, s->cntL, s->row_flags, s->row_pos, s->row_list, s->scan_sums, &s->ss->n_rows);
             }
             built = true;
+        } else if (s->setup_ahead && use_mg(s) && !s->dist) {
+            HIPCHK(hipGetLastError());
+            HIPCHK(hipMemcpyAsync(s->h_ss, s->ss, sizeof(StepState), hipMemcpyDeviceToHost, s->st));
+            HIPCHK(hipEventRecord(s->ev_poll[0], s->st));
+            s->lists_on = false;
+            HIPCHK(zero_search(s, lb));
+            int rc2 = mg_setup(s);
+            if (rc2) return rc2;
+            HIPCHK(hipEventSynchronize(s->ev_poll[0]));
+            setup_done = true;
         }
         HIPCHK(hipGetLastError());
     }
-    int rc = read_ss(s);
+    int rc = setup_done ? FLUID_OK : read_ss(s);
     if (rc) return rc;
     s->stats.num_active = s->h_ss->num_active;
     s->last_num_active = s->stats.num_active;
@@ -1008,12 +1039,13 @@
         if (s->n_drop > 0) s->stats.paths |= FLUID_PATH_DROPLETS;
         s->lists_on = built && s->n_tl_mg > 0 && s->n_tl_sq > 0 && (s->lists_force == 1 || airy);
         if (s->lists_on) s->stats.paths |= FLUID_PATH_TILE_LISTS;
-        const size_t lb = (s->L.cells() + 2 * (size_t)s->L.Lz) * solver_elem(s);
-        HIPCHK(zero_search(s, lb));
-        HIPCHK(hipGetLastError());
-        if (use_mg(s)) {
-            int rc2 = mg_setup(s);
-            if (rc2) return rc2;
+        if (!setup_done) {
+            HIPCHK(zero_search(s, lb));
+            HIPCHK(hipGetLastError());
+            if (use_mg(s)) {
+                int rc2 = mg_setup(s);
+                if (rc2) return rc2;
+            }
         }
     }
     s->have_flags = true;
@@ -1156,7 +1188,7 @@
     return FLUID_OK;
 }
 
-static int phase_flip_advect(fluid_sim* s)
+static int phase_flip_advect(fluid_sim* s, bool in_step = false)
 {
     if (!s->have_p2g) return fail(FLUID_ERR_STATE, "flip_advect before p2g");
     HIPCHK(hipSetDevice(s->prm.device));
@@ -1174,7 +1206,7 @@
     }
     prof_end(s, FLUID_PROF_G2P, tok);
     const bool bin = s->advect_bin && !s->dist && s->np > 0 && s->sorted && s->sort_hint && !box_empty(s->Pb);
-    s->binned = false;
+    s->drop_binned();
     if (bin) {
         const Grid g = s->g;
         s->bin_x0 = std::max(0, s->Pb.x0 - 3);
@@ -1182,19 +1214,32 @@
         const long n2 = g.sx(), c0 = (long)s->bin_x0 * n2, c1 = (long)(s->bin_x1 + 1) * n2;
         HIPCHK(hipMemsetAsync(s->cell_count + c0, 0, (c1 - c0) * sizeof(int), s->st));
         HIPCHK(hipMemsetAsync(s->cell_count + s->ncell, 0, 4 * sizeof(int), s->st));
-        launch_advect_bin(s->st, g, s->np, s->pa.shifted(s->p_off), s->flags, s->prm.max_dt, s->prm.dx, s->ss, s->key, s->slot, s->cell_count, s->ipart);
+        launch_advect_bin(s->st, g, s->np, s->pa.shifted(s->p_off), s->flags, s->prm.max_dt, s->prm.dx, s->ss, s->key, s->slot, s->cell_count, s->ipart,
+                          std::min(s->bin_x0 + 2, s->Pb.x0), std::max(s->bin_x1 - 2, s->Pb.x1));
     } else {
         launch_advect(s->st, s->g, s->np, s->pa.shifted(s->p_off), s->flags, s->prm.max_dt, s->prm.dx, s->ss);
     }
     HIPCHK(hipGetLastError());
-    int rc = read_ss(s);
-    if (rc) return rc;
+    const bool ahead = bin && in_step && s->sort_ahead && !sources_active(s);
+    int rc;
+    if (ahead) {
+        HIPCHK(hipMemcpyAsync(s->h_ss, s->ss, sizeof(StepState), hipMemcpyDeviceToHost, s->st));
+        HIPCHK(hipEventRecord(s->ev_poll[0], s->st));
+        const int tok = prof_begin(s, FLUID_PROF_SORT, (double)s->np);
+        rc = sort_binned_launch(s, &s->ss->sort_go);
+        prof_end(s, FLUID_PROF_SORT, tok);
+        if (rc) return rc;
+        HIPCHK(hipEventSynchronize(s->ev_poll[0]));
+    } else if ((rc = read_ss(s))) {
+        return rc;
+    }
     if (bin) {
         const StepState& h = *s->h_ss;
         for (int a = 0; a < 3; ++a) s->bin_min[a] = h.bbox_min[a], s->bin_max[a] = h.bbox_max[a];
         s->bin_n_out = h.n_out;
         s->bin_max_cell = h.max_cell;
         s->binned = true;
+        s->presorted = ahead && h.sort_go != 0;
     }
     s->dt = s->h_ss->dt;
     double ms;
@@ -1299,7 +1344,7 @@
     if (n_parked) *n_parked = s->h_small[0];
     s->sorted = s->have_p2g = s->have_flags = false;
     s->sort_hint = false;
-    s->binned = false;
+    s->drop_binned();
     return FLUID_OK;
 }
 
@@ -1324,7 +1369,7 @@
         if ((rc = phase_pressure_pass(s, &error))) return rc;
         if (s->prm.max_outer_passes > 0 && s->stats.outer_passes >= s->prm.max_outer_passes) break;
     } while (error > s->prm.outer_tol);
-    if ((rc = phase_flip_advect(s))) return rc;
+    if ((rc = phase_flip_advect(s, true))) return rc;
     if ((rc = sources_apply(s))) return rc;
     if ((rc = output_auto(s))) return rc;
     s->n_steps++;
diff --git a/fluid-simulation_amd/csrc/fluid_sources.hip b/fluid-simulation_amd/csrc/fluid_sources.hip
--- a/fluid-simulation_amd/csrc/fluid_sources.hip
+++ b/fluid-simulation_amd/csrc/fluid_sources.hip
@@ -109,14 +109,19 @@
     return FLUID_OK;
 }
 
-int fl::sources_apply(fluid_sim* s)
-{
-    s->src_emit_last = s->src_rm_last = 0;
+bool fl::sources_active(const fluid_sim* s)
+{
     bool any = false;
     for (int i = 0; i < FLUID_MAX_SINKS; ++i) any = any || s->sink_on[i];
     for (const auto& q : s->src) any = any || q.on;
-    if (!any) return FLUID_OK;
-    s->binned = false;
+    return any;
+}
+
+int fl::sources_apply(fluid_sim* s)
+{
+    s->src_emit_last = s->src_rm_last = 0;
+    if (!sources_active(s)) return FLUID_OK;
+    s->drop_binned();
     const long t = s->n_steps;
     long removed = 0, emitted = 0;
     int rc = apply_sinks(s, &removed);
@@ -160,7 +165,7 @@
     s->np += (long)n;
     s->sorted = s->have_p2g = s->have_flags = false;
     s->sort_hint = false;
-    s->binned = false;
+    s->drop_binned();
     return FLUID_OK;
 }
 
diff --git a/fluid-simulation_amd/csrc/kernels_particles.hip b/fluid-simulation_amd/csrc/kernels_particles.hip
--- a/fluid-simulation_amd/csrc/kernels_particles.hip
+++ b/fluid-simulation_amd/csrc/kernels_particles.hip
@@ -134,8 +134,9 @@
 
 __global__ __launch_bounds__(256) void k_bin_scatter(long n, const int* __restrict__ key, const int* __restrict__ slot,
                                                      const int* __restrict__ cell_start, const uint32_t* __restrict__ pid,
-                                                     int* __restrict__ order, uint32_t* __restrict__ spid)
-{
+                                                     int* __restrict__ order, uint32_t* __restrict__ spid, const int* __restrict__ go)
+{
+    if (go && !*go) return;
     long i = (long)blockIdx.x * 256 + threadIdx.x;
     if (i >= n) return;
     const int d = cell_start[key[i]] + slot[i];
@@ -145,8 +146,10 @@
 
 constexpr int RANK_CH = 2048;
 __global__ __launch_bounds__(256) void k_bin_rank(long n_pos, long pos0, const int* __restrict__ key, const int* __restrict__ cell_start,
-                                                  const int* __restrict__ order, const uint32_t* __restrict__ spid, int* __restrict__ order2)
-{
+                                                  const int* __restrict__ order, const uint32_t* __restrict__ spid, int* __restrict__ order2,
+                                                  const int* __restrict__ go)
+{
+    if (go && !*go) return;
     __shared__ uint32_t sid[RANK_CH];
     __shared__ int sAB[2];
     const long j = pos0 + (long)blockIdx.x * 256 + threadIdx.x;
@@ -189,8 +192,9 @@
 }
 
 __global__ __launch_bounds__(256) void k_reorder(long n, const int* __restrict__ order, Particles s, Particles d, double* __restrict__ w,
-                                                 long wstride)
-{
+                                                 long wstride, const int* __restrict__ go)
+{
+    if (go && !*go) return;
     long j = (long)blockIdx.x * 256 + threadIdx.x;
     if (j >= n) return;
     int i = order[j];
@@ -935,11 +939,15 @@
     bin_block_partials(acc, sm, part);
 }
 
-__global__ __launch_bounds__(256) void k_publish_dt(double max_dt, double dx, StepState* ss, const int* __restrict__ part, int nb)
+__global__ __launch_bounds__(256) void k_publish_dt(double max_dt, double dx, StepState* ss, const int* __restrict__ part, int nb, int go_lo,
+                                                    int go_hi)
 {
     __shared__ int sm[4][8];
     if (nb > 0) bin_reduce(part, nb, ss, sm);
-    if (threadIdx.x == 0) ss->dt = advect_timestep(max_dt, dx, ss);
+    if (threadIdx.x == 0) {
+        ss->dt = advect_timestep(max_dt, dx, ss);
+        ss->sort_go = nb > 0 && (ss->bbox_max[0] < 0 || (ss->bbox_min[0] >= go_lo && ss->bbox_max[0] <= go_hi));
+    }
 }
 
 __global__ __launch_bounds__(256) void k_unpack_records(long n, const double* __restrict__ rec, Particles p, long off)
@@ -1009,18 +1017,23 @@
     hipLaunchKernelGGL(k_bin_bbox, dim3(1), dim3(256), 0, st, (const int*)part, (int)nb, ss);
 }
 void launch_bin_scatter(hipStream_t st, long n, const int* key, const int* slot, const int* cell_start, const uint32_t* pid, int* order,
-                         uint32_t* spid)
-{
-    if (n > 0) hipLaunchKernelGGL(k_bin_scatter, dim3(nblk(n)), dim3(256), 0, st, n, key, slot, cell_start, pid, order, spid);
+                         uint32_t* spid, const int* go)
+{
+    if (n > 0) hipLaunchKernelGGL(k_bin_scatter, dim3(nblk(n)), dim3(256), 0, st, n, key, slot, cell_start, pid, order, spid, go);
+}
+void launch_bin_rank(hipStream_t st, long n_pos, long pos0, const int* key, const int* cell_start, const int* order, const uint32_t* spid,
+                     int* order2, const int* go)
+{
+    if (n_pos > 0) hipLaunchKernelGGL(k_bin_rank, dim3(nblk(n_pos)), dim3(256), 0, st, n_pos, pos0, key, cell_start, order, spid, order2, go);
 }
 void launch_bin_rank(hipStream_t st, long n_pos, long pos0, const int* key, const int* cell_start, const int* order, const uint32_t* spid,
                      int* order2)
 {
-    if (n_pos > 0) hipLaunchKernelGGL(k_bin_rank, dim3(nblk(n_pos)), dim3(256), 0, st, n_pos, pos0, key, cell_start, order, spid, order2);
-}
-void launch_reorder(hipStream_t st, long n, const int* order, Particles src, Particles dst, double* w, long wstride)
-{
-    if (n > 0) hipLaunchKernelGGL(k_reorder, dim3(nblk(n)), dim3(256), 0, st, n, order, src, dst, w, wstride);
+    launch_bin_rank(st, n_pos, pos0, key, cell_start, order, spid, order2, nullptr);
+}
+void launch_reorder(hipStream_t st, long n, const int* order, Particles src, Particles dst, double* w, long wstride, const int* go)
+{
+    if (n > 0) hipLaunchKernelGGL(k_reorder, dim3(nblk(n)), dim3(256), 0, st, n, order, src, dst, w, wstride, go);
 }
 void launch_weights(hipStream_t st, long n, Particles p, double* w, long stride)
 {
@@ -1097,15 +1110,15 @@
 void launch_advect(hipStream_t st, Grid g, long n, Particles p, const uint8_t* flags, double max_dt, double dx, StepState* ss)
 {
     if (n > 0) hipLaunchKernelGGL(k_advect, dim3(nblk(n)), dim3(256), 0, st, g, n, p, flags, max_dt, dx, ss);
-    hipLaunchKernelGGL(k_publish_dt, dim3(1), dim3(1), 0, st, max_dt, dx, ss, (const int*)nullptr, 0);
+    hipLaunchKernelGGL(k_publish_dt, dim3(1), dim3(1), 0, st, max_dt, dx, ss, (const int*)nullptr, 0, 0, -1);
 }
 void launch_advect_bin(hipStream_t st, Grid g, long n, Particles p, const uint8_t* flags, double max_dt, double dx, StepState* ss, int* key,
-                       int* slot, int* cell_count, int* part)
+                       int* slot, int* cell_count, int* part, int go_lo, int go_hi)
 {
     unsigned nb = nblk(n);
     if (nb > 1024) nb = 1024;
     hipLaunchKernelGGL(k_advect_bin, dim3(nb), dim3(256), 0, st, g, n, p, flags, max_dt, dx, ss, key, slot, cell_count, part);
-    hipLaunchKernelGGL(k_publish_dt, dim3(1), dim3(256), 0, st, max_dt, dx, ss, (const int*)part, (int)nb);
+    hipLaunchKernelGGL(k_publish_dt, dim3(1), dim3(256), 0, st, max_dt, dx, ss, (const int*)part, (int)nb, go_lo, go_hi);
 }
 void launch_unpack_records(hipStream_t st, long n, const double* rec, Particles p, long off)
 {
diff --git a/fluid-simulation_amd/csrc/sim.h b/fluid-simulation_amd/csrc/sim.h
--- a/fluid-simulation_amd/csrc/sim.h
+++ b/fluid-simulation_amd/csrc/sim.h
@@ -123,6 +123,10 @@
     bool binned = false;
     int bin_x0 = 0, bin_x1 = -1;
     int bin_min[3] = {0, 0, 0}, bin_max[3] = {-1, -1, -1}, bin_n_out = 0, bin_max_cell = 0;
+    bool sort_ahead = true;
+    bool presorted = false;
+    void drop_binned() { binned = presorted = false; }
+    bool setup_ahead = true;
     bool solve_tail = true;
     bool tail_ran = false;
     double dt = 0.1;
@@ -208,6 +212,7 @@
 int pic_fields(fluid_sim* s);
 int fluid_create_window(const fluid_params_t* p, const Grid& g, fluid_sim_t** out);
 
+bool sources_active(const fluid_sim* s);
 int sources_apply(fluid_sim* s);
 void sources_free(fluid_sim* s);
 
```
